# zqqqqz2000/MixGRPO

Hardware: AMD Instinct MI355X
Metric: GRPO train-step images/sec, FLUX.1-dev 1024^2 (higher is better)
Workload: dtype bf16

## Files before the change

### include/mixgrpo_hip.h

```cpp
#ifndef MIXGRPO_HIP_H
#define MIXGRPO_HIP_H
#include <stdint.h>
#ifdef __cplusplus
extern "C" {
#endif

int mgx_version(void);
const char* mgx_last_error(void);

typedef struct {
  float sigma_x0;
  float c_x;
  float c_v;
  float dt_mean;
  float sd_noise;
  float dt_det;
  float den;
  float log_sd;
  float log_c;
} mgx_flow_coeffs;

long mgx_logp_workspace_elems(int B, long n);

int mgx_flow_step_fwd(const float* x, const uint16_t* v, const uint16_t* noise, const float* prev_in,
// ... 7 lines not shown
  float ds_r;
  float s_r;
  float ds;
  float ds_b;
  float s_b;
  float one_m_s;
  float s_sq;
  float half_eta2;
  float sd;
  float den;
} mgx_dance_coeffs;

int mgx_dance_step_fwd(const float* x, const uint16_t* v, const float* noise, const float* prev_in,
                       float* prev_out, float* x0_out, float* logp, double* ws, int B, long n,
                       const mgx_dance_coeffs* k , int sde, void* stream);
int mgx_dance_step_bwd(const float* x, const uint16_t* v, const float* prev, const float* g_logp, uint16_t* dv,
                       int B, long n, const mgx_dance_coeffs* k , int sde, void* stream);

typedef struct {
  int order;
  int sde;
  float sigma_x0;
  float inv_r0;
  float inv_r1;
  float c_r;
  float inv_r01;
  float cm[4];
  float cx[4];
  float sd_noise;
  float den;
  float log_sd;
  float log_c;
} mgx_dpm_coeffs;

int mgx_dpm_step_fwd(const float* sample, const uint16_t* v, const float* m1, const float* m2, const float* noise,
                     float* x_out, float* x0_out, float* logp, double* ws, int B, long n,
                     const mgx_dpm_coeffs* k , void* stream);

int mgx_dpm_step_bwd(const float* sample, const uint16_t* v, const float* x_t, const float* g_logp, uint16_t* dv, int B,
                     long n, const mgx_dpm_coeffs* k , float sigma_b, void* stream);

int mgx_x0_pred(const float* sample, const uint16_t* v, float* x0_out, long total, float sigma_x0, void* stream);

int mgx_pack_latents(const void* in, void* out, int B, int C, int H, int W, int elem_size, void* stream);
int mgx_unpack_latents(const void* in, void* out, int B, int C, int H, int W, int elem_size, void* stream);

int mgx_group_advantage(const float* rewards, float* out, int n, int G, int trim, float weight, int accumulate,
                        void* stream);
int mgx_global_advantage(const float* rewards, const float* gathered, float* out, int n, int n_all, void* stream);

int mgx_grpo_loss(const float* new_logp, const float* old_logp, const float* adv, int B, float clip_range,
                  float adv_clip_max, float kl_coeff, float denom, float* loss, float* policy, float* kl,
                  float* clip_frac, float* g_logp, void* stream);

enum { MGX_EPI_BIAS = 0, MGX_EPI_BIAS_GELU = 1, MGX_EPI_BIAS_GATE_RES = 2, MGX_EPI_F32_ACC = 3, MGX_EPI_DGELU = 4 };

int mgx_gemm_bf16(const uint16_t* A, const uint16_t* W, const uint16_t* bias, void* C, const uint16_t* gate,
                  uint16_t* aux, long ldaux, int M, int N, int K, long lda, long a_rpb, long a_bstride, long ldw, long ldc,
                  long c_rpb, long c_bstride, long gate_ld, int epilogue, float beta, void* stream);
long mgx_gemm_sk_workspace_elems(void);
int mgx_gemm_bf16_sk(const uint16_t* A, const uint16_t* W, const uint16_t* bias, void* C, const uint16_t* gate,
                     uint16_t* aux, long ldaux, int M, int N, int K, long lda, long a_rpb, long a_bstride, long ldw, long ldc,
                     long c_rpb, long c_bstride, long gate_ld, int epilogue, float beta, float* sk_workspace,
                     long sk_workspace_elems, void* stream);
int mgx_linear_qk_norm_rope(const uint16_t* X, const uint16_t* Wqk, const uint16_t* bias, const float* wq, const float* wk,
                            const float* cos, const float* sin, const float* cos_sin_pairs ,
                            uint16_t* Q, uint16_t* K, int B, int H, int S, int rows_per_batch, int s0, int Kdim, long ldx,
                            long ldw, float q_scale, void* stream);

int mgx_linear_bf16_t(const uint16_t* X, const uint16_t* W, const uint16_t* bias, uint16_t* Ct, int tokens, int F, int K,
                      long ldx, long ldw, long ld_ct, long tok_rpb, long ct_bstride, float* sk_workspace,
                      long sk_workspace_elems, void* stream);

int mgx_gemm_plan(int M, int N, int K, int stream_k, int* out, int cap);
int mgx_gemm_plan_units(int M, int N, int K, int stream_k, int fixup, int index, int* out, int cap);

long mgx_transpose_partial_elems(int M, int N);
int mgx_transpose_bf16(const uint16_t* in, uint16_t* out, float* colsum_partial, float* colsum_out, float colsum_beta,
                       int M, int N, long ld_in, long in_rpb, long in_bstride, long ld_out, void* stream);

int mgx_ln_modulate_fwd(const uint16_t* x, long ldx, long x_rpb, long x_bstride, const uint16_t* shift,
                        const uint16_t* scale, long mod_ld, uint16_t* y, long ldy, float* stats, long M, int D,
                        void* stream);
long mgx_ln_modulate_bwd_workspace(long M, long rpb, int D);
int mgx_ln_modulate_bwd(const uint16_t* dy, long lddy, const uint16_t* x, long ldx, long x_rpb, long x_bstride,
                        const uint16_t* scale, long mod_ld, uint16_t* dx, long lddx, long dx_rpb, long dx_bstride,
                        int accumulate, uint16_t* dshift, uint16_t* dscale, float* ws, long M, int D, void* stream);

int mgx_qk_norm_rope_fwd(const uint16_t* qkv, long ld, const float* wq, const float* wk, const float* cos,
                         const float* sin, uint16_t* Q, uint16_t* K, uint16_t* Vt, uint16_t* V, uint16_t* Qt,
                         uint16_t* Kt, int B, int H, int S, int Sp, int rows_per_batch, int s0, void* stream);
int mgx_qk_norm_rope_fwd_qs(const uint16_t* qkv, long ld, const float* wq, const float* wk, const float* cos,
                            const float* sin, uint16_t* Q, uint16_t* K, uint16_t* Vt, uint16_t* V, uint16_t* Qt,
                            uint16_t* Kt, int B, int H, int S, int Sp, int rows_per_batch, int s0, float q_scale,
                            void* stream);
long mgx_qk_norm_rope_bwd_workspace(int B, int H, int rows_per_batch);
int mgx_qk_norm_rope_bwd(const uint16_t* qkv, long ld, const float* wq, const float* wk, const float* cos,
                         const float* sin, const uint16_t* dQ, const uint16_t* dK, const uint16_t* dV, uint16_t* dqkv,
                         long ld_dqkv , float* gwq, float* gwk, float* ws, int B,
                         int H, int S, int Sp, int rows_per_batch, int s0, void* stream);

int mgx_qk_norm_rope_bwd_qs(const uint16_t* qkv, long ld, const float* wq, const float* wk, const float* cos,
                            const float* sin, const uint16_t* dQ, const uint16_t* dK, const uint16_t* dV, uint16_t* dqkv,
                            long ld_dqkv, float* gwq, float* gwk, float* ws, int B, int H, int S, int Sp,
                            int rows_per_batch, int s0, float q_scale, void* stream);

int mgx_attn_fwd(const uint16_t* Q, const uint16_t* K, const uint16_t* Vt, uint16_t* O, float* lse, int B, int H, int S,
                 int Sp, long ldo, long o_bstride, float scale, void* stream);

int mgx_attn_fwd_log2(const uint16_t* Q2, const uint16_t* K, const uint16_t* Vt, uint16_t* O, float* lse, int B, int H,
                      int S, int Sp, long ldo, long o_bstride, void* stream);

int mgx_attn_fwd_path(int B, int H, int S, int Sp, long ldo, long o_bstride);
int mgx_attn_bwd_path(int B, int H, int S, int Sp, long ldo, long o_bstride);

int mgx_attn_fwd_log2_kv(const uint16_t* Q2, const uint16_t* K, const uint16_t* Vt, uint16_t* O, float* lse, int B, int H,
                         int Sa, int kv_len, long ldo, long o_bstride, void* stream);
int mgx_attn_fwd_kv_path(int B, int H, int Sa, int kv_len, long ldo, long o_bstride);

int mgx_attn_fp8_quantize(const uint16_t* Q, const uint16_t* K, const uint16_t* Vt, uint8_t* Q8, uint8_t* K8,
                          uint8_t* V8t, float* amax, int B, int H, int S, int Sp, void* stream);
int mgx_attn_fwd_fp8(const uint8_t* Q8, const uint8_t* K8, const uint8_t* V8t, const float* amax, uint16_t* O,
                     float* lse, int B, int H, int S, int Sp, long ldo, long o_bstride, float scale, void* stream);

int mgx_attn_bwd(const uint16_t* Q, const uint16_t* K, const uint16_t* V, const uint16_t* Qt, const uint16_t* Kt,
                 const uint16_t* O, const uint16_t* dO, const float* lse, float* delta, uint16_t* dOt, uint16_t* dQ,
                 uint16_t* dK, uint16_t* dV, int B, int H, int S, int Sp, long ldo, long o_bstride, float scale,
                 void* stream);

long mgx_attn_bwd_fp8_workspace(int B, int H, int S, int Sp);
int mgx_attn_bwd_fp8(const uint16_t* Q, const uint16_t* K, const uint16_t* V, const uint16_t* Qt, const uint16_t* Kt,
                     const uint16_t* O, const uint16_t* dO, const float* lse, float* delta, uint16_t* dOt, uint16_t* dQ,
                     uint16_t* dK, uint16_t* dV, uint8_t* ws, float* amax, int B, int H, int S, int Sp, long ldo,
                     long o_bstride, float scale, long ws_bytes, void* stream);

int mgx_attn_bwd_kv(const uint16_t* Q, const uint16_t* K, const uint16_t* V, const uint16_t* Qt, const uint16_t* Kt,
                    const uint16_t* O, const uint16_t* dO, const float* lse, float* delta, uint16_t* dOt, uint16_t* dQ,
                    uint16_t* dK, uint16_t* dV, int B, int H, int Sa, int kv_len, long ldo, long o_bstride, float scale,
                    void* stream);
int mgx_attn_bwd_kv_path(int B, int H, int Sa, int kv_len, long ldo, long o_bstride);

int mgx_attn_kv_operands(int stream, int kv_len, int block, int* out, int cap);

int mgx_skinny_linear(const uint16_t* x, long ldx, const uint16_t* W, long ldw, const uint16_t* bias, uint16_t* out,
                      long ldo, int Bn, int N, int K, void* stream);
int mgx_skinny_wgrad(const uint16_t* dout, long ldd, const uint16_t* x, long ldx, float* dW, long ldw, float* dbias,
                     int Bn, int N, int K, void* stream);
long mgx_skinny_dgrad_workspace(int Bn, int K);
int mgx_skinny_dgrad(const uint16_t* dout, long ldd, const uint16_t* W, long ldw, uint16_t* dx, long lddx, float* ws,
                     int Bn, int N, int K, int accumulate, void* stream);
int mgx_ew_bf16(const uint16_t* a, const uint16_t* b, uint16_t* y, long n, int op, void* stream);
int mgx_sincos_embed(const float* t, uint16_t* out, int Bn, void* stream);
int mgx_cast_f32_bf16(const float* x, uint16_t* y, long n, void* stream);
int mgx_cast_bf16_f32(const uint16_t* x, float* y, long n, float scale, void* stream);
int mgx_transpose_gelu_bf16(const uint16_t* in, uint16_t* out, int M, int N, long ld_in, long ld_out, void* stream);
int mgx_gelu_bf16(const uint16_t* x, long ldx, uint16_t* y, long ldy, long M, int N, void* stream);
long mgx_gate_bwd_workspace(long batches, long rows_per_batch, int D);
int mgx_gate_bwd(const uint16_t* dout, long ldd, long d_bstride, const uint16_t* y, long ldy, const uint16_t* gate,
                 long gate_ld, uint16_t* dy, long lddy, uint16_t* dgate, float* ws, int batches, long rows_per_batch,
                 int D, void* stream);

long mgx_sqnorm_workspace(void);
int mgx_sqnorm_f32(const float* g, long n, double* ws, float* out, float beta, void* stream);
int mgx_adamw_step(float* w, uint16_t* w16, const float* g, float* m, float* v, long n, double lr, double beta1,
                   double beta2, double eps, double weight_decay, int step, const float* gnorm_sq, float max_norm,
                   float grad_scale, void* stream);
int mgx_scale_f32(float* x, long n, float s, void* stream);


int mgx_conv3x3_nhwc(const uint16_t* x, const uint16_t* Wt, const uint16_t* bias, uint16_t* out, long ld_out,
                     const uint16_t* ones, int H, int W, int C, int Cout, int residual, void* stream);
long mgx_group_norm_workspace(long M, int C, int G);
int mgx_group_norm_nhwc(const uint16_t* x, long ld, const uint16_t* gamma, const uint16_t* beta, uint16_t* out, long out_row,
                        long out_px, float* ws, int H, int W, int C, int G, float eps, int silu, void* stream);
int mgx_upsample2x_pad_nhwc(const uint16_t* x, uint16_t* out, int H, int W, int C, void* stream);
int mgx_latents_to_pad_nhwc(const float* z, uint16_t* out, int Cin, int H, int W, int C, void* stream);
int mgx_nhwc_to_image(const uint16_t* x, long ld, uint16_t* img, int Cout, int H, int W, void* stream);
int mgx_softmax_rows_f32(const float* S, long lds, uint16_t* P, long ldp, int M, int n, float scale, void* stream);

int mgx_lora_proj(const uint16_t* in, const uint16_t* P, uint16_t* out, long M, int Kin, int r, long ld_in, long in_rpb,
                  long in_bstride, float scale, void* stream);
long mgx_lora_wgrad_workspace(long M, int Kin, int r);
int mgx_lora_wgrad(const uint16_t* small, const uint16_t* big, float* G, float* workspace, long workspace_elems, long M, int Kin,
                   int r, long ld_big, long big_rpb, long big_bstride, float beta, void* stream);
int mgx_lora_merge(const float* W0, const float* Bt, const float* A, uint16_t* W16, int N, int K, int r, float s, void* stream);

#ifdef __cplusplus
}
#endif
#endif
```

### mixgrpo_amd/_lib.py

```python
import ctypes as C
import os

import torch

_HERE = os.path.dirname(os.path.abspath(__file__))
LIB_PATH = os.path.join(_HERE, "csrc", "libmixgrpo_hip.so")


class MgxError(RuntimeError):
    pass


class FlowCoeffs(C.Structure):
    _fields_ = [(n, C.c_float) for n in ("sigma_x0", "c_x", "c_v", "dt_mean", "sd_noise", "dt_det", "den", "log_sd",
                                         "log_c")]


class DanceCoeffs(C.Structure):
    _fields_ = [(n, C.c_float) for n in ("ds_r", "s_r", "ds", "ds_b", "s_b", "one_m_s", "s_sq", "half_eta2", "sd", "den")]


class DpmCoeffs(C.Structure):
    _fields_ = [("order", C.c_int), ("sde", C.c_int), ("sigma_x0", C.c_float), ("inv_r0", C.c_float),
                ("inv_r1", C.c_float), ("c_r", C.c_float), ("inv_r01", C.c_float), ("cm", C.c_float * 4),
                ("cx", C.c_float * 4), ("sd_noise", C.c_float), ("den", C.c_float), ("log_sd", C.c_float),
                ("log_c", C.c_float)]


_P = C.c_void_p
_I = C.c_int
_L = C.c_long
_F = C.c_float
_D = C.c_double

SIGNATURES = {
    "mgx_version": (_I, []),
    "mgx_last_error": (C.c_char_p, []),
    "mgx_logp_workspace_elems": (_L, [_I, _L]),
    "mgx_flow_step_fwd": (_I, [_P] * 9 + [_I, _L, C.POINTER(FlowCoeffs), _I, _P]),
    "mgx_flow_step_bwd": (_I, [_P] * 5 + [_I, _L, C.POINTER(FlowCoeffs), _P]),
    "mgx_dance_step_fwd": (_I, [_P] * 8 + [_I, _L, C.POINTER(DanceCoeffs), _I, _P]),
    "mgx_dance_step_bwd": (_I, [_P] * 5 + [_I, _L, C.POINTER(DanceCoeffs), _I, _P]),
    "mgx_dpm_step_fwd": (_I, [_P] * 9 + [_I, _L, C.POINTER(DpmCoeffs), _P]),
    "mgx_dpm_step_bwd": (_I, [_P] * 5 + [_I, _L, C.POINTER(DpmCoeffs), _F, _P]),
    "mgx_x0_pred": (_I, [_P, _P, _P, _L, _F, _P]),
    "mgx_pack_latents": (_I, [_P, _P, _I, _I, _I, _I, _I, _P]),
    "mgx_unpack_latents": (_I, [_P, _P, _I, _I, _I, _I, _I, _P]),
    "mgx_group_advantage": (_I, [_P, _P, _I, _I, _I, _F, _I, _P]),
    "mgx_global_advantage": (_I, [_P, _P, _P, _I, _I, _P]),
    "mgx_grpo_loss": (_I, [_P, _P, _P, _I, _F, _F, _F, _F, _P, _P, _P, _P, _P, _P]),
    "mgx_gemm_bf16": (_I, [_P] * 6 + [_L, _I, _I, _I] + [_L] * 8 + [_I, _F, _P]),
    "mgx_gemm_sk_workspace_elems": (_L, []),
    "mgx_gemm_bf16_sk": (_I, [_P] * 6 + [_L, _I, _I, _I] + [_L] * 8 + [_I, _F, _P, _L, _P]),
    "mgx_linear_bf16_t": (_I, [_P] * 4 + [_I] * 3 + [_L] * 5 + [_P, _L, _P]),
    "mgx_linear_qk_norm_rope": (_I, [_P] * 10 + [_I] * 6 + [_L, _L, _F, _P]),
    "mgx_gemm_plan": (_I, [_I] * 4 + [C.POINTER(_I), _I]),
    "mgx_gemm_plan_units": (_I, [_I] * 6 + [C.POINTER(_I), _I]),
    "mgx_transpose_partial_elems": (_L, [_I, _I]),
    "mgx_transpose_bf16": (_I, [_P, _P, _P, _P, _F, _I, _I, _L, _L, _L, _L, _P]),
    "mgx_ln_modulate_fwd": (_I, [_P, _L, _L, _L, _P, _P, _L, _P, _L, _P, _L, _I, _P]),
    "mgx_ln_modulate_bwd_workspace": (_L, [_L, _L, _I]),
    "mgx_ln_modulate_bwd": (_I, [_P, _L, _P, _L, _L, _L, _P, _L, _P, _L, _L, _L, _I, _P, _P, _P, _L, _I, _P]),
    "mgx_qk_norm_rope_fwd": (_I, [_P, _L] + [_P] * 10 + [_I] * 6 + [_P]),
    "mgx_qk_norm_rope_fwd_qs": (_I, [_P, _L] + [_P] * 10 + [_I] * 6 + [_F, _P]),
    "mgx_qk_norm_rope_bwd_workspace": (_L, [_I, _I, _I]),
    "mgx_qk_norm_rope_bwd": (_I, [_P, _L] + [_P] * 8 + [_L] + [_P] * 3 + [_I] * 6 + [_P]),
    "mgx_qk_norm_rope_bwd_qs": (_I, [_P, _L] + [_P] * 8 + [_L] + [_P] * 3 + [_I] * 6 + [_F, _P]),
    "mgx_attn_fwd": (_I, [_P] * 5 + [_I] * 4 + [_L, _L, _F, _P]),
    "mgx_attn_fwd_log2": (_I, [_P] * 5 + [_I] * 4 + [_L, _L, _P]),
    "mgx_attn_fwd_path": (_I, [_I] * 4 + [_L, _L]),
    "mgx_attn_fwd_log2_kv": (_I, [_P] * 5 + [_I] * 4 + [_L, _L, _P]),
    "mgx_attn_fwd_kv_path": (_I, [_I] * 4 + [_L, _L]),
    "mgx_attn_bwd_path": (_I, [_I] * 4 + [_L, _L]),
    "mgx_attn_fp8_quantize": (_I, [_P] * 7 + [_I] * 4 + [_P]),
    "mgx_attn_fwd_fp8": (_I, [_P] * 6 + [_I] * 4 + [_L, _L, _F, _P]),
    "mgx_attn_bwd": (_I, [_P] * 13 + [_I] * 4 + [_L, _L, _F, _P]),
    "mgx_attn_bwd_fp8_workspace": (_L, [_I] * 4),
    "mgx_attn_bwd_fp8": (_I, [_P] * 15 + [_I] * 4 + [_L, _L, _F, _L, _P]),
    "mgx_attn_bwd_kv": (_I, [_P] * 13 + [_I] * 4 + [_L, _L, _F, _P]),
    "mgx_attn_bwd_kv_path": (_I, [_I] * 4 + [_L, _L]),
    "mgx_attn_kv_operands": (_I, [_I] * 3 + [C.POINTER(_I), _I]),
    "mgx_skinny_linear": (_I, [_P, _L, _P, _L, _P, _P, _L, _I, _I, _I, _P]),
    "mgx_skinny_wgrad": (_I, [_P, _L, _P, _L, _P, _L, _P, _I, _I, _I, _P]),
    "mgx_skinny_dgrad_workspace": (_L, [_I, _I]),
    "mgx_conv3x3_nhwc": (_I, [_P, _P, _P, _P, _L, _P, _I, _I, _I, _I, _I, _P]),
    "mgx_group_norm_workspace": (_L, [_L, _I, _I]),
    "mgx_group_norm_nhwc": (_I, [_P, _L, _P, _P, _P, _L, _L, _P, _I, _I, _I, _I, _F, _I, _P]),
    "mgx_upsample2x_pad_nhwc": (_I, [_P, _P, _I, _I, _I, _P]),
    "mgx_latents_to_pad_nhwc": (_I, [_P, _P, _I, _I, _I, _I, _P]),
    "mgx_nhwc_to_image": (_I, [_P, _L, _P, _I, _I, _I, _P]),
    "mgx_softmax_rows_f32": (_I, [_P, _L, _P, _L, _I, _I, _F, _P]),
    "mgx_skinny_dgrad": (_I, [_P, _L, _P, _L, _P, _L, _P, _I, _I, _I, _I, _P]),
    "mgx_ew_bf16": (_I, [_P, _P, _P, _L, _I, _P]),
    "mgx_sincos_embed": (_I, [_P, _P, _I, _P]),
    "mgx_cast_f32_bf16": (_I, [_P, _P, _L, _P]),
    "mgx_cast_bf16_f32": (_I, [_P, _P, _L, _F, _P]),
    "mgx_gelu_bf16": (_I, [_P, _L, _P, _L, _L, _I, _P]),
    "mgx_transpose_gelu_bf16": (_I, [_P, _P, _I, _I, _L, _L, _P]),
    "mgx_gate_bwd_workspace": (_L, [_L, _L, _I]),
    "mgx_gate_bwd": (_I, [_P, _L, _L, _P, _L, _P, _L, _P, _L, _P, _P, _I, _L, _I, _P]),
    "mgx_sqnorm_workspace": (_L, []),
    "mgx_sqnorm_f32": (_I, [_P, _L, _P, _P, _F, _P]),
    "mgx_adamw_step": (_I, [_P, _P, _P, _P, _P, _L, _D, _D, _D, _D, _D, _I, _P, _F, _F, _P]),
    "mgx_scale_f32": (_I, [_P, _L, _F, _P]),
    "mgx_lora_proj": (_I, [_P, _P, _P, _L, _I, _I, _L, _L, _L, _F, _P]),
    "mgx_lora_wgrad_workspace": (_L, [_L, _I, _I]),
    "mgx_lora_wgrad": (_I, [_P, _P, _P, _P, _L, _L, _I, _I, _L, _L, _L, _F, _P]),
    "mgx_lora_merge": (_I, [_P, _P, _P, _P, _I, _I, _I, _F, _P]),
}

_lib = None


def lib():
    global _lib
    if _lib is None:
        if not os.path.exists(LIB_PATH):
            raise MgxError(f"{LIB_PATH} is missing: run `python -m mixgrpo_amd.build` (hipcc, gfx950). "
                           "There is no CPU fallback for the product path.")
        h = C.CDLL(LIB_PATH)
        h.mgx_version.restype = _I
        v = h.mgx_version()
        if v < 0:
            raise MgxError(f"{LIB_PATH} is a DIAGNOSTIC build (mgx_version() = {v}, -DMGX_DIAGNOSTIC_BUILD): its timing-only "
                           "switches compute wrong results.  Rebuild with `python -m mixgrpo_amd.build --force`.")
        for name, (res, args) in SIGNATURES.items():
            fn = getattr(h, name)
            fn.restype = res
            fn.argtypes = args
        _lib = h
    return _lib


def check(code):
    if code != 0:
        raise MgxError(f"libmixgrpo_hip error {code}: {lib().mgx_last_error().decode()}")


def ptr(t):
    if t is None:
        return None
    if not t.is_cuda:
        raise MgxError("mixgrpo_amd HIP ops need device tensors (got a CPU tensor); there is no CPU path")
    if not t.is_contiguous():
        raise MgxError("mixgrpo_amd HIP ops need contiguous tensors")
    return t.data_ptr()


def stream():
    return torch.cuda.current_stream().cuda_stream


_ws_cache = {}


def logp_workspace(B, n, device):
    need = lib().mgx_logp_workspace_elems(B, n)
    key = (device, torch.cuda.current_stream().cuda_stream)
    w = _ws_cache.get(key)
    if w is None or w.numel() < need:
        w = torch.empty(max(need, 4096), dtype=torch.float64, device=device)
        _ws_cache[key] = w
    return w
```

### mixgrpo_amd/csrc/gemm.hip

```cpp
#include "../../include/mixgrpo_hip.h"
#include "common.h"
#include "gemm_plan.h"

#include <cmath>
#include <cstdlib>

namespace {

constexpr int BM = 128, BN = 128, BK = gemm_plan::BK;
constexpr int NT = 256;

struct RowMap {
  long ld;
  long rpb;
  long bstride;
};

__device__ __forceinline__ long row_off(const RowMap& r, long m) {
  const uint32_t rpb = (uint32_t)r.rpb;
  const uint32_t b = (uint32_t)m / rpb;
  return (long)b * r.bstride + (long)((uint32_t)m - b * rpb) * r.ld;
}

enum Epi { EPI_BIAS = 0, EPI_BIAS_GELU = 1, EPI_BIAS_GATE_RES = 2, EPI_F32_ACC = 3, EPI_BIAS_MULAUX = 4,
// ... 242 lines not shown
    if (m < M && n < N) v = in[row_off(im, m) + n];
    tile[r][tx] = v;
  }
  __syncthreads();
  for (int r = ty; r < 64; r += 4) {
    const int n = n0 + r;
    const long m = m0 + tx;
    if (n < N && m < ldo) out[(long)n * ldo + m] = (m < M) ? tile[tx][r] : (bf16_raw)0;
  }
  if (part && m0 < M) {
    if (ty == 0) {
      float s = 0.f;
      for (int r = 0; r < 64; ++r) s += bf2f(tile[r][tx]);
      if (n0 + tx < N) part[(long)blockIdx.y * N + n0 + tx] = s;
    }
  }
}

__device__ __forceinline__ uint32_t lo16(uint32_t a, uint32_t b) { return __builtin_amdgcn_perm(b, a, 0x05040100); }
__device__ __forceinline__ uint32_t hi16(uint32_t a, uint32_t b) { return __builtin_amdgcn_perm(b, a, 0x07060302); }
template <bool GELU>
__global__ void __launch_bounds__(256) transpose8_kernel(const bf16_raw* __restrict__ in, bf16_raw* __restrict__ out,
                                                         float* __restrict__ part, int M, int N, RowMap im, long ldo) {
  __shared__ float cs[16][129];
  const int tx = (threadIdx.x & 7) | (((threadIdx.x >> 6) & 1) << 3), ty = ((threadIdx.x >> 3) & 7) | ((threadIdx.x >> 7) << 3);
  const int n0 = blockIdx.x * 128 + tx * 8;
  const long m0 = (long)blockIdx.y * 128 + ty * 8;
  uint32_t r[8][4];
  float csum[8];
#pragma unroll
  for (int j = 0; j < 8; ++j) csum[j] = 0.f;
  const bool ncol_ok = n0 < N;
#pragma unroll
  for (int i = 0; i < 8; ++i) {
    const long m = m0 + i;
    uint4 v = make_uint4(0, 0, 0, 0);
    if (ncol_ok && m < M) v = *reinterpret_cast<const uint4*>(in + row_off(im, m) + n0);
    if (GELU && ncol_ok && m < M) {
      auto gl = [](uint32_t u) {
        return (uint32_t)f2bf(gelu_tanh_f(bf2f(u & 0xffff))) | ((uint32_t)f2bf(gelu_tanh_f(bf2f(u >> 16))) << 16);
      };
      v.x = gl(v.x); v.y = gl(v.y); v.z = gl(v.z); v.w = gl(v.w);
    }
    r[i][0] = v.x; r[i][1] = v.y; r[i][2] = v.z; r[i][3] = v.w;
    if (part) {
      csum[0] += bf2f(v.x & 0xffff); csum[1] += bf2f(v.x >> 16); csum[2] += bf2f(v.y & 0xffff); csum[3] += bf2f(v.y >> 16);
      csum[4] += bf2f(v.z & 0xffff); csum[5] += bf2f(v.z >> 16); csum[6] += bf2f(v.w & 0xffff); csum[7] += bf2f(v.w >> 16);
    }
  }
  if (ncol_ok && m0 < ldo) {
#pragma unroll
    for (int c2 = 0; c2 < 4; ++c2) {
      uint4 e, o;
      e.x = lo16(r[0][c2], r[1][c2]); e.y = lo16(r[2][c2], r[3][c2]); e.z = lo16(r[4][c2], r[5][c2]); e.w = lo16(r[6][c2], r[7][c2]);
      o.x = hi16(r[0][c2], r[1][c2]); o.y = hi16(r[2][c2], r[3][c2]); o.z = hi16(r[4][c2], r[5][c2]); o.w = hi16(r[6][c2], r[7][c2]);
      *reinterpret_cast<uint4*>(out + (long)(n0 + 2 * c2) * ldo + m0) = e;
      *reinterpret_cast<uint4*>(out + (long)(n0 + 2 * c2 + 1) * ldo + m0) = o;
    }
  }
  if (part) {
#pragma unroll
    for (int j = 0; j < 8; ++j) cs[ty][tx * 8 + j] = csum[j];
    __syncthreads();
    if (threadIdx.x < 128) {
      float t = 0.f;
#pragma unroll
      for (int k = 0; k < 16; ++k) t += cs[k][threadIdx.x];
      const int n = blockIdx.x * 128 + threadIdx.x;
      if (n < N && (long)blockIdx.y * 128 < M) part[(long)blockIdx.y * N + n] = t;
    }
  }
}

__global__ void __launch_bounds__(256) colsum_finish_kernel(const float* __restrict__ part, float* __restrict__ out, int nblk,
                                                            int N, float beta) {
  __shared__ float red[4][64];
  const int cx = threadIdx.x & 63, ky = threadIdx.x >> 6;
  const int n = blockIdx.x * 64 + cx;
  float s = 0.f;
  if (n < N)
    for (int b = ky; b < nblk; b += 4) s += part[(long)b * N + n];
  red[ky][cx] = s;
  __syncthreads();
  if (ky == 0 && n < N) out[n] = beta * out[n] + ((red[0][cx] + red[1][cx]) + (red[2][cx] + red[3][cx]));
}

__device__ __forceinline__ int wperm(int p) { return (p >> 5) * 32 + ((p & 15) >> 2) * 8 + ((p >> 4) & 1) * 4 + (p & 3); }
__device__ __forceinline__ int lane_feat(int fq, int t) { return (t >> 1) * 32 + fq * 8 + (t & 1) * 4; }

__device__ __forceinline__ void unpack8(const uint4& u, float* v) {
  v[0] = bf2f(u.x & 0xffff); v[1] = bf2f(u.x >> 16); v[2] = bf2f(u.y & 0xffff); v[3] = bf2f(u.y >> 16);
  v[4] = bf2f(u.z & 0xffff); v[5] = bf2f(u.z >> 16); v[6] = bf2f(u.w & 0xffff); v[7] = bf2f(u.w >> 16);
}
__device__ __forceinline__ uint4 pack8(const float* v) {
  uint4 o;
  o.x = (uint32_t)f2bf(v[0]) | ((uint32_t)f2bf(v[1]) << 16);
  o.y = (uint32_t)f2bf(v[2]) | ((uint32_t)f2bf(v[3]) << 16);
  o.z = (uint32_t)f2bf(v[4]) | ((uint32_t)f2bf(v[5]) << 16);
  o.w = (uint32_t)f2bf(v[6]) | ((uint32_t)f2bf(v[7]) << 16);
  return o;
}

__device__ __forceinline__ float vmul1(float a, float b) { float r; asm("v_mul_f32 %0, %1, %2" : "=v"(r) : "v"(a), "v"(b)); return r; }
__device__ __forceinline__ float vsub1(float a, float b) { float r; asm("v_sub_f32 %0, %1, %2" : "=v"(r) : "v"(a), "v"(b)); return r; }
__device__ __forceinline__ float vadd1(float a, float b) { float r; asm("v_add_f32 %0, %1, %2" : "=v"(r) : "v"(a), "v"(b)); return r; }

template <bool PAIRED>
__device__ __forceinline__ void qknorm_epilogue(const GemmArgs& g, f32x4 (&acc)[4][8], int wid, int lane, long m0, long n0,
                                                char* red) {
#pragma clang fp contract(off)
  constexpr int MT = 8;
  const int fr = lane & 15, fq = lane >> 4;
  const int wu = __builtin_amdgcn_readfirstlane(wid);
  const long nu = n0 + (wu & 3) * 64;
  long mu = m0 + (wu >> 2) * 128;
  const bool inside = mu < g.M;
  if (!inside) mu = g.M - 128;
  const int sec = nu >= g.qn_dmodel ? 1 : 0;
  const int hcol = (int)(nu - (long)sec * g.qn_dmodel);
  const int head = hcol >> 7, hb = hcol & 64;
  const uint32_t bu = (uint32_t)mu / (uint32_t)g.c.rpb;
  const int t0 = (int)((uint32_t)mu - bu * (uint32_t)g.c.rpb);
  const int f0 = lane_feat(fq, 0), f1 = lane_feat(fq, 2);
  uint4 bias0 = make_uint4(0, 0, 0, 0), bias1 = bias0;
  if (g.bias) {
    bias0 = *reinterpret_cast<const uint4*>(g.bias + nu + f0);
    bias1 = *reinterpret_cast<const uint4*>(g.bias + nu + f1);
  }
  const float* cbase = g.qn_cos + (long)(g.qn_s0 + t0 + fr) * 128 + hb;
  const float* sbase = g.qn_sin + (long)(g.qn_s0 + t0 + fr) * 128 + hb;
  constexpr int AHEAD = PAIRED ? 2 : 1, NSLOT = AHEAD + 1;
  float4 cs[NSLOT][PAIRED ? 4 : 8];
  const float* pbase = g.qn_cs2 + (long)(g.qn_s0 + t0 + fr) * 128 + hb;
  auto load_cs = [&](int slot, int j, uint32_t dep) {
    const long o = (long)(j * 16 + dep) * 128;
    if constexpr (PAIRED) {
      cs[slot][0] = *reinterpret_cast<const float4*>(pbase + o + f0);
      cs[slot][1] = *reinterpret_cast<const float4*>(pbase + o + f0 + 4);
      cs[slot][2] = *reinterpret_cast<const float4*>(pbase + o + f1);
      cs[slot][3] = *reinterpret_cast<const float4*>(pbase + o + f1 + 4);
      return;
    }
    cs[slot][0] = *reinterpret_cast<const float4*>(cbase + o + f0);
    cs[slot][1] = *reinterpret_cast<const float4*>(cbase + o + f0 + 4);
    cs[slot][2] = *reinterpret_cast<const float4*>(cbase + o + f1);
    cs[slot][3] = *reinterpret_cast<const float4*>(cbase + o + f1 + 4);
    cs[slot][4] = *reinterpret_cast<const float4*>(sbase + o + f0);
    cs[slot][5] = *reinterpret_cast<const float4*>(sbase + o + f0 + 4);
    cs[slot][6] = *reinterpret_cast<const float4*>(sbase + o + f1);
    cs[slot][7] = *reinterpret_cast<const float4*>(sbase + o + f1 + 4);
  };
  uint4 y[MT][2];
  {
    float bias[16];
    unpack8(bias0, bias);
    unpack8(bias1, bias + 8);
#pragma unroll
    for (int j = 0; j < MT; ++j) {
      float v[16];
#pragma unroll
      for (int t = 0; t < 4; ++t)
#pragma unroll
        for (int r = 0; r < 4; ++r) v[t * 4 + r] = acc[t][j][r] + bias[t * 4 + r];
      y[j][0] = pack8(v);
      y[j][1] = pack8(v + 8);
      __builtin_amdgcn_sched_barrier(0);
    }
// ... 837 lines not shown
```

### mixgrpo_amd/csrc/norm.hip

```cpp
#include "../../include/mixgrpo_hip.h"
#include "common.h"

namespace {

struct RowMap {
  long ld, rpb, bstride;
};
__device__ __forceinline__ long row_off(const RowMap& r, long m) {
  const long b = m / r.rpb;
  return b * r.bstride + (m - b * r.rpb) * r.ld;
}

constexpr int LN_MAXV = 8;

__device__ __forceinline__ void unpack8(const uint4& u, float* f) {
  f[0] = bf2f(u.x & 0xffff); f[1] = bf2f(u.x >> 16); f[2] = bf2f(u.y & 0xffff); f[3] = bf2f(u.y >> 16);
  f[4] = bf2f(u.z & 0xffff); f[5] = bf2f(u.z >> 16); f[6] = bf2f(u.w & 0xffff); f[7] = bf2f(u.w >> 16);
}
__device__ __forceinline__ uint4 pack8(const float* f) {
  uint4 u;
  u.x = (uint32_t)f2bf(f[0]) | ((uint32_t)f2bf(f[1]) << 16);
  u.y = (uint32_t)f2bf(f[2]) | ((uint32_t)f2bf(f[3]) << 16);
  u.z = (uint32_t)f2bf(f[4]) | ((uint32_t)f2bf(f[5]) << 16);
  u.w = (uint32_t)f2bf(f[6]) | ((uint32_t)f2bf(f[7]) << 16);
  return u;
}

template <int NV>
__global__ void __launch_bounds__(256) ln_mod_fwd_kernel(const bf16_raw* __restrict__ x, RowMap xm,
                                                         const bf16_raw* __restrict__ shift,
                                                         const bf16_raw* __restrict__ scale, long mod_ld,
                                                         bf16_raw* __restrict__ y, long ldy, float* __restrict__ stats,
                                                         long M) {
  const long m = (long)blockIdx.x * 4 + (threadIdx.x >> 6);
  if (m >= M) return;
  const int lane = threadIdx.x & 63;
  const long b = m / xm.rpb;
  const bf16_raw* xr = x + row_off(xm, m);
  float v[NV][8];
  float s = 0.f;
#pragma unroll
  for (int i = 0; i < NV; ++i) {
    unpack8(*reinterpret_cast<const uint4*>(xr + (i * 64 + lane) * 8), v[i]);
#pragma unroll
    for (int j = 0; j < 8; ++j) s += v[i][j];
  }
  const float D = (float)(NV * 512);
  const float mean = wave_sum(s) / D;
  float q = 0.f;
#pragma unroll
  for (int i = 0; i < NV; ++i)
#pragma unroll
    for (int j = 0; j < 8; ++j) {
      const float d = v[i][j] - mean;
      q += d * d;
    }
  const float rstd = rsqrtf(wave_sum(q) / D + 1e-6f);
  if (stats && lane == 0) {
    stats[2 * m] = mean;
    stats[2 * m + 1] = rstd;
  }
  const bf16_raw* sh = shift + b * mod_ld;
  const bf16_raw* sc = scale + b * mod_ld;
#pragma unroll
  for (int i = 0; i < NV; ++i) {
    const int c = (i * 64 + lane) * 8;
    float fs[8], fc[8], o[8];
    unpack8(*reinterpret_cast<const uint4*>(sh + c), fs);
    unpack8(*reinterpret_cast<const uint4*>(sc + c), fc);
#pragma unroll
    for (int j = 0; j < 8; ++j) o[j] = (v[i][j] - mean) * rstd * rbf(1.0f + fc[j]) + fs[j];
    *reinterpret_cast<uint4*>(y + m * ldy + c) = pack8(o);
  }
}

constexpr int LN_BWD_ROWS = 32;
template <int NV>
__global__ void __launch_bounds__(256) ln_mod_bwd_kernel(const bf16_raw* __restrict__ dy, long lddy,
                                                         const bf16_raw* __restrict__ x, RowMap xm,
                                                         const bf16_raw* __restrict__ scale, long mod_ld,
                                                         bf16_raw* __restrict__ dx, RowMap dxm, int accumulate,
                                                         float* __restrict__ part, long M, int blocks_per_batch) {
  extern __shared__ float red[];
  const int D = NV * 512;
  const int lane = threadIdx.x & 63, w = threadIdx.x >> 6;
  const long b = blockIdx.x / blocks_per_batch;
  const long r0 = (long)(blockIdx.x % blocks_per_batch) * LN_BWD_ROWS;
  const bf16_raw* sc = scale + b * mod_ld;
  float a_sh[NV][8], a_sc[NV][8];
#pragma unroll
  for (int i = 0; i < NV; ++i)
#pragma unroll
    for (int j = 0; j < 8; ++j) a_sh[i][j] = a_sc[i][j] = 0.f;

  auto row_ok = [&](int rr) { return rr < LN_BWD_ROWS && r0 + rr < xm.rpb && b * xm.rpb + r0 + rr < M; };
  uint4 nx[NV], ng[NV], nold[NV];
  auto fetch = [&](int rr) {
    const long m = b * xm.rpb + r0 + rr;
    const bf16_raw* xr = x + row_off(xm, m);
    const bf16_raw* dxr = dx + row_off(dxm, m);
#pragma unroll
    for (int i = 0; i < NV; ++i) {
      nx[i] = *reinterpret_cast<const uint4*>(xr + (i * 64 + lane) * 8);
      ng[i] = *reinterpret_cast<const uint4*>(dy + m * lddy + (i * 64 + lane) * 8);
      nold[i] = accumulate ? *reinterpret_cast<const uint4*>(dxr + (i * 64 + lane) * 8) : make_uint4(0, 0, 0, 0);
    }
  };
  if (row_ok(w)) fetch(w);
  for (int rr = w; row_ok(rr); rr += 4) {
    const long m = b * xm.rpb + r0 + rr;
    bf16_raw* dxr = dx + row_off(dxm, m);
    float v[NV][8], g[NV][8];
    uint4 oldp[NV];
    float s = 0.f;
#pragma unroll
    for (int i = 0; i < NV; ++i) {
      unpack8(nx[i], v[i]);
      unpack8(ng[i], g[i]);
      oldp[i] = nold[i];
#pragma unroll
      for (int j = 0; j < 8; ++j) s += v[i][j];
    }
    if (row_ok(rr + 4)) fetch(rr + 4);
    const float Df = (float)D;
    const float mean = wave_sum(s) / Df;
    float q = 0.f;
#pragma unroll
    for (int i = 0; i < NV; ++i)
#pragma unroll
      for (int j = 0; j < 8; ++j) {
        const float d = v[i][j] - mean;
        q += d * d;
      }
    const float rstd = rsqrtf(wave_sum(q) / Df + 1e-6f);
    float c1 = 0.f, c2 = 0.f;
#pragma unroll
    for (int i = 0; i < NV; ++i) {
      float fc[8];
      unpack8(*reinterpret_cast<const uint4*>(sc + (i * 64 + lane) * 8), fc);
#pragma unroll
      for (int j = 0; j < 8; ++j) {
        const float xh = (v[i][j] - mean) * rstd;
        const float gx = g[i][j] * rbf(1.0f + fc[j]);
        a_sh[i][j] += g[i][j];
        a_sc[i][j] += g[i][j] * xh;
        c1 += gx;
        c2 += gx * xh;
        v[i][j] = xh;
        g[i][j] = gx;
      }
    }
    c1 = wave_sum(c1) / Df;
    c2 = wave_sum(c2) / Df;
#pragma unroll
    for (int i = 0; i < NV; ++i) {
// ... 176 lines not shown
  long ldo;
  float* part;
  int H, S, Sp, rows_per_batch, s0;
  float q_scale;
};

__global__ void __launch_bounds__(256) qk_norm_rope_bwd_kernel(QkBwdArgs a) {
  __shared__ float red[4][2][128];
  const int lane = threadIdx.x & 63, w = threadIdx.x >> 6;
  const int hh = blockIdx.y, b = blockIdx.z;
  const int t0 = blockIdx.x * 64;
  const int HD = 128;
  const long dmodel = (long)a.H * HD;
  const float wq0 = a.wq[2 * lane], wq1 = a.wq[2 * lane + 1];
  const float wk0 = a.wk[2 * lane], wk1 = a.wk[2 * lane + 1];
  float gq0 = 0.f, gq1 = 0.f, gk0 = 0.f, gk1 = 0.f;
  constexpr int U = 4;
  for (int i0 = 0; i0 < 16; i0 += U) {
    uint32_t ux[U][2], ug[U][2], uv[U];
    float2 cc[U], ss[U];
    bool ok[U];
#pragma unroll
    for (int u = 0; u < U; ++u) {
      const int t = t0 + w * 16 + i0 + u;
      ok[u] = t < a.rows_per_batch;
      const int tc = ok[u] ? t : a.rows_per_batch - 1;
      const long row = (long)b * a.rows_per_batch + tc;
      const int s = a.s0 + tc;
      const bf16_raw* base = a.qkv + row * a.ld + hh * HD + 2 * lane;
      const long o = (((long)b * a.H + hh) * a.S + s) * HD + 2 * lane;
      ux[u][0] = *reinterpret_cast<const uint32_t*>(base);
      ux[u][1] = *reinterpret_cast<const uint32_t*>(base + dmodel);
      ug[u][0] = *reinterpret_cast<const uint32_t*>(a.dQ + o);
      ug[u][1] = *reinterpret_cast<const uint32_t*>(a.dK + o);
      uv[u] = *reinterpret_cast<const uint32_t*>(a.dV + o);
      cc[u] = *reinterpret_cast<const float2*>(a.cos + (long)s * HD + 2 * lane);
      ss[u] = *reinterpret_cast<const float2*>(a.sin + (long)s * HD + 2 * lane);
    }
#pragma unroll
    for (int u = 0; u < U; ++u) {
      if (!ok[u]) continue;
      const int t = t0 + w * 16 + i0 + u;
      const long row = (long)b * a.rows_per_batch + t;
      bf16_raw* obase = a.dqkv + row * a.ldo + hh * HD + 2 * lane;
      const float c0 = cc[u].x, c1 = cc[u].y, s0 = ss[u].x, s1 = ss[u].y;
#pragma unroll
      for (int which = 0; which < 2; ++which) {
        const float w0 = which ? wk0 : wq0, w1 = which ? wk1 : wq1;
        const float x0 = bf2f(ux[u][which] & 0xffff), x1 = bf2f(ux[u][which] >> 16);
        const float gs = which ? 1.f : a.q_scale;
        const float go0 = bf2f(ug[u][which] & 0xffff) * gs, go1 = bf2f(ug[u][which] >> 16) * gs;
        const float gy0 = go0 * c0 + go1 * s1;
        const float gy1 = -go0 * s0 + go1 * c1;
        const float r = rsqrtf(head_sum(x0 * x0 + x1 * x1) / 128.f + 1e-6f);
        if (which) { gk0 += gy0 * x0 * r; gk1 += gy1 * x1 * r; } else { gq0 += gy0 * x0 * r; gq1 += gy1 * x1 * r; }
        const float gz0 = gy0 * w0, gz1 = gy1 * w1;
        const float dot = wave_sum(gz0 * x0 + gz1 * x1) / 128.f;
        const float dx0 = r * gz0 - x0 * r * r * r * dot;
        const float dx1 = r * gz1 - x1 * r * r * r * dot;
        *reinterpret_cast<uint32_t*>(obase + which * dmodel) = (uint32_t)f2bf(dx0) | ((uint32_t)f2bf(dx1) << 16);
      }
      *reinterpret_cast<uint32_t*>(obase + 2 * dmodel) = uv[u];
    }
  }
  red[w][0][2 * lane] = gq0; red[w][0][2 * lane + 1] = gq1;
  red[w][1][2 * lane] = gk0; red[w][1][2 * lane + 1] = gk1;
  __syncthreads();
  const long blk = ((long)blockIdx.z * gridDim.y + blockIdx.y) * gridDim.x + blockIdx.x;
  {
    const int which = threadIdx.x >> 7, c = threadIdx.x & 127;
    a.part[(blk * 2 + which) * 128 + c] = red[0][which][c] + red[1][which][c] + red[2][which][c] + red[3][which][c];
  }
}

constexpr int QK_FIN_G = 128;
__global__ void __launch_bounds__(256) qk_bwd_partial_kernel(const float* __restrict__ part, float* __restrict__ mid,
                                                             long nblocks) {
  float s = 0.f;
  for (long k = blockIdx.x; k < nblocks; k += QK_FIN_G) s += part[k * 256 + threadIdx.x];
  mid[(long)blockIdx.x * 256 + threadIdx.x] = s;
}

__global__ void __launch_bounds__(256) qk_bwd_finish_kernel(const float* __restrict__ part, float* __restrict__ gq,
                                                            float* __restrict__ gk, long nblocks) {
  __shared__ float red[16][17];
  const int which = blockIdx.x >> 3, c0 = (blockIdx.x & 7) * 16;
  const int cx = threadIdx.x & 15, ry = threadIdx.x >> 4;
  float s = 0.f;
  for (long k = ry; k < nblocks; k += 16) s += part[(k * 2 + which) * 128 + c0 + cx];
  red[ry][cx] = s;
  __syncthreads();
  if (ry == 0) {
    float t = 0.f;
#pragma unroll
    for (int i = 0; i < 16; ++i) t += red[i][cx];
    float* dst = which ? gk : gq;
    dst[c0 + cx] += t;
  }
}

}

extern "C" int mgx_ln_modulate_fwd(const uint16_t* x, long ldx, long x_rpb, long x_bstride, const uint16_t* shift,
                                   const uint16_t* scale, long mod_ld, uint16_t* y, long ldy, float* stats, long M, int D,
                                   void* stream) {
  MGX_REQUIRE(x && shift && scale && y && M > 0, "bad argument");
  MGX_REQUIRE(D % 512 == 0 && D <= 4096, "feature size must be a multiple of 512 up to 4096");
  MGX_REQUIRE(ldx % 8 == 0 && ldy % 8 == 0 && mod_ld % 8 == 0 && x_bstride % 8 == 0, "16-byte row alignment");
  hipStream_t st = (hipStream_t)stream;
  const RowMap xm{ldx, x_rpb, x_bstride};
  const int grid = cdiv(M, 4);
  switch (D / 512) {
#define CASE(nv) case nv: ln_mod_fwd_kernel<nv><<<grid, 256, 0, st>>>(x, xm, shift, scale, mod_ld, y, ldy, stats, M); break;
    CASE(1) CASE(2) CASE(3) CASE(4) CASE(5) CASE(6) CASE(7) CASE(8)
#undef CASE
  }
  MGX_CHECK_LAUNCH();
  return MGX_OK;
}

extern "C" long mgx_ln_modulate_bwd_workspace(long M, long rpb, int D) {
  const long batches = (M + rpb - 1) / rpb;
  const long bpb = ((rpb < M ? rpb : M) + LN_BWD_ROWS - 1) / LN_BWD_ROWS;
  return batches * bpb * 2 * D;
}

extern "C" int mgx_ln_modulate_bwd(const uint16_t* dy, long lddy, const uint16_t* x, long ldx, long x_rpb, long x_bstride,
                                   const uint16_t* scale, long mod_ld, uint16_t* dx, long lddx, long dx_rpb,
                                   long dx_bstride, int accumulate, uint16_t* dshift, uint16_t* dscale, float* ws, long M,
                                   int D, void* stream) {
  MGX_REQUIRE(dy && x && scale && dx && dshift && dscale && ws && M > 0, "bad argument");
  MGX_REQUIRE(D % 512 == 0 && D <= 4096, "feature size must be a multiple of 512 up to 4096");
  MGX_REQUIRE(x_rpb == dx_rpb, "x and dx must be batched alike");
  hipStream_t st = (hipStream_t)stream;
  const long rpb = x_rpb < M ? x_rpb : M;
  const int batches = cdiv(M, rpb);
  const int bpb = cdiv(rpb, LN_BWD_ROWS);
  const RowMap xm{ldx, rpb, x_bstride}, dxm{lddx, rpb, dx_bstride};
  const size_t lds = (size_t)2 * D * sizeof(float);
  switch (D / 512) {
#define CASE(nv)                                                                                                  \
  case nv:                                                                                                        \
    ln_mod_bwd_kernel<nv><<<batches * bpb, 256, lds, st>>>(dy, lddy, x, xm, scale, mod_ld, dx, dxm, accumulate, ws, M, bpb); \
    break;
    CASE(1) CASE(2) CASE(3) CASE(4) CASE(5) CASE(6) CASE(7) CASE(8)
#undef CASE
  }
  ln_mod_bwd_finish_kernel<<<dim3(cdiv(D, 64), batches), 256, 0, st>>>(ws, dshift, dscale, mod_ld, D, bpb);
  MGX_CHECK_LAUNCH();
  return MGX_OK;
}

extern "C" int mgx_qk_norm_rope_fwd_qs(const uint16_t* qkv, long ld, const float* wq, const float* wk, const float* cos,
                                       const float* sin, uint16_t* Q, uint16_t* K, uint16_t* Vt, uint16_t* V, uint16_t* Qt,
                                       uint16_t* Kt, int B, int H, int S, int Sp, int rows_per_batch, int s0, float q_scale,
                                       void* stream) {
  MGX_REQUIRE(qkv && wq && wk && cos && sin && Q && K, "null argument");
  MGX_REQUIRE((V != nullptr) == (Qt != nullptr) && (V != nullptr) == (Kt != nullptr), "V, Qt, Kt come together");
  MGX_REQUIRE(Vt || !V, "Vt may only be left out (V^T written by mgx_linear_bf16_t) without the backward's extra layouts");
  MGX_REQUIRE(B > 0 && H > 0 && rows_per_batch > 0 && s0 >= 0 && s0 + rows_per_batch <= S && Sp >= S, "bad sizes");
  MGX_REQUIRE(ld == 3L * H * 128, "qkv rows must be [q | k | v] of H*128 each");
  MGX_REQUIRE(q_scale > 0.f, "q_scale must be positive");
  QkArgs a{qkv, ld, wq, wk, cos, sin, Q, K, Vt, V, Qt, Kt, H, S, Sp, rows_per_batch, s0, q_scale};
  dim3 grid(cdiv(rows_per_batch, 64), H, B);
  if (V) qk_norm_rope_fwd_kernel<true><<<grid, 256, 0, (hipStream_t)stream>>>(a);
  else qk_norm_rope_fwd_kernel<false><<<grid, 256, 0, (hipStream_t)stream>>>(a);
  MGX_CHECK_LAUNCH();
  return MGX_OK;
}

extern "C" int mgx_qk_norm_rope_fwd(const uint16_t* qkv, long ld, const float* wq, const float* wk, const float* cos,
                                    const float* sin, uint16_t* Q, uint16_t* K, uint16_t* Vt, uint16_t* V, uint16_t* Qt,
                                    uint16_t* Kt, int B, int H, int S, int Sp, int rows_per_batch, int s0, void* stream) {
  return mgx_qk_norm_rope_fwd_qs(qkv, ld, wq, wk, cos, sin, Q, K, Vt, V, Qt, Kt, B, H, S, Sp, rows_per_batch, s0, 1.0f, stream);
}

extern "C" long mgx_qk_norm_rope_bwd_workspace(int B, int H, int rows_per_batch) {
  return ((long)cdiv(rows_per_batch, 64) * H * B + QK_FIN_G) * 2 * 128;
}

extern "C" int mgx_qk_norm_rope_bwd_qs(const uint16_t* qkv, long ld, const float* wq, const float* wk, const float* cos,
                                       const float* sin, const uint16_t* dQ, const uint16_t* dK, const uint16_t* dV,
                                       uint16_t* dqkv, long ld_dqkv, float* gwq, float* gwk, float* ws, int B, int H, int S,
                                       int Sp, int rows_per_batch, int s0, float q_scale, void* stream) {
  MGX_REQUIRE(qkv && wq && wk && cos && sin && dQ && dK && dV && dqkv && gwq && gwk && ws, "null argument");
  MGX_REQUIRE(ld == 3L * H * 128, "qkv rows must be [q | k | v] of H*128 each");
  MGX_REQUIRE(ld_dqkv >= ld && ld_dqkv % 2 == 0, "dqkv rows must hold [dq | dk | dv] and keep 4-byte alignment");
  hipStream_t st = (hipStream_t)stream;
  QkBwdArgs a{qkv, ld, wq, wk, cos, sin, dQ, dK, dV, dqkv, ld_dqkv, ws, H, S, Sp, rows_per_batch, s0, q_scale};
  dim3 grid(cdiv(rows_per_batch, 64), H, B);
  qk_norm_rope_bwd_kernel<<<grid, 256, 0, st>>>(a);
  const long nblocks = (long)grid.x * grid.y * grid.z;
  float* mid = ws + nblocks * 256;
  qk_bwd_partial_kernel<<<QK_FIN_G, 256, 0, st>>>(ws, mid, nblocks);
  qk_bwd_finish_kernel<<<16, 256, 0, st>>>(mid, gwq, gwk, QK_FIN_G);
  MGX_CHECK_LAUNCH();
  return MGX_OK;
}

extern "C" int mgx_qk_norm_rope_bwd(const uint16_t* qkv, long ld, const float* wq, const float* wk, const float* cos,
                                    const float* sin, const uint16_t* dQ, const uint16_t* dK, const uint16_t* dV,
                                    uint16_t* dqkv, long ld_dqkv, float* gwq, float* gwk, float* ws, int B, int H, int S,
                                    int Sp, int rows_per_batch, int s0, void* stream) {
  return mgx_qk_norm_rope_bwd_qs(qkv, ld, wq, wk, cos, sin, dQ, dK, dV, dqkv, ld_dqkv, gwq, gwk, ws, B, H, S, Sp, rows_per_batch,
                                 s0, 1.0f, stream);
}
```

### mixgrpo_amd/csrc/small.hip

```cpp
#include "../../include/mixgrpo_hip.h"
#include "common.h"

namespace {

__global__ void __launch_bounds__(256) skinny_linear_kernel(const bf16_raw* __restrict__ x, long ldx,
                                                            const bf16_raw* __restrict__ W, long ldw,
                                                            const bf16_raw* __restrict__ bias,
                                                            bf16_raw* __restrict__ out, long ldo, int Bn, int N, int K) {
  __shared__ f32x4 red[3][64];
  const int lane = threadIdx.x & 63, w = threadIdx.x >> 6;
  const int n0 = blockIdx.x * 16;
  const int fr = lane & 15, fq = lane >> 4;
  int nrow = n0 + fr;
  if (nrow >= N) nrow = N - 1;
  int brow = fr < Bn ? fr : Bn - 1;
  const int kchunk = ((K / 32 + 3) / 4) * 32;
  const int kbeg = min(w * kchunk, K), kend = min(kbeg + kchunk, K);
  const bf16_raw* wp = W + (long)nrow * ldw + fq * 8;
  const bf16_raw* xp = x + (long)brow * ldx + fq * 8;
  f32x4 acc = {0.f, 0.f, 0.f, 0.f};
  int k = kbeg;
  for (; k + 128 <= kend; k += 128) {
    s16x8 a0 = *reinterpret_cast<const s16x8*>(wp + k), a1 = *reinterpret_cast<const s16x8*>(wp + k + 32);
    s16x8 a2 = *reinterpret_cast<const s16x8*>(wp + k + 64), a3 = *reinterpret_cast<const s16x8*>(wp + k + 96);
    s16x8 b0 = *reinterpret_cast<const s16x8*>(xp + k), b1 = *reinterpret_cast<const s16x8*>(xp + k + 32);
    s16x8 b2 = *reinterpret_cast<const s16x8*>(xp + k + 64), b3 = *reinterpret_cast<const s16x8*>(xp + k + 96);
    acc = __builtin_amdgcn_mfma_f32_16x16x32_bf16(a0, b0, acc, 0, 0, 0);
    acc = __builtin_amdgcn_mfma_f32_16x16x32_bf16(a1, b1, acc, 0, 0, 0);
    acc = __builtin_amdgcn_mfma_f32_16x16x32_bf16(a2, b2, acc, 0, 0, 0);
    acc = __builtin_amdgcn_mfma_f32_16x16x32_bf16(a3, b3, acc, 0, 0, 0);
  }
  for (; k < kend; k += 32) {
    s16x8 a0 = *reinterpret_cast<const s16x8*>(wp + k);
    s16x8 b0 = *reinterpret_cast<const s16x8*>(xp + k);
    acc = __builtin_amdgcn_mfma_f32_16x16x32_bf16(a0, b0, acc, 0, 0, 0);
  }
  if (w > 0) red[w - 1][lane] = acc;
  __syncthreads();
  if (w > 0) return;
#pragma unroll
  for (int i = 0; i < 3; ++i) {
    const f32x4 o = red[i][lane];
    acc[0] += o[0]; acc[1] += o[1]; acc[2] += o[2]; acc[3] += o[3];
  }
  if (fr < Bn) {
#pragma unroll
    for (int r = 0; r < 4; ++r) {
      const int n = n0 + 4 * fq + r;
      if (n < N) {
        float v = acc[r];
        if (bias) v += bf2f(bias[n]);
        out[(long)fr * ldo + n] = f2bf(v);
      }
    }
  }
}

__global__ void __launch_bounds__(256) skinny_wgrad_kernel(const bf16_raw* __restrict__ dout, long ldd,
                                                           const bf16_raw* __restrict__ x, long ldx,
                                                           float* __restrict__ dW, long ldw, float* __restrict__ dbias,
                                                           int Bn, int N, int K) {
  const int n = blockIdx.y;
  float dn[16];
  float sb = 0.f;
#pragma unroll
  for (int b = 0; b < 16; ++b) {
    dn[b] = b < Bn ? bf2f(dout[(long)b * ldd + n]) : 0.f;
    sb += dn[b];
  }
  if (dbias && blockIdx.x == 0 && threadIdx.x == 0) dbias[n] += sb;
  for (int k = (blockIdx.x * 256 + threadIdx.x) * 4; k < K; k += gridDim.x * 256 * 4) {
    float4 g = *reinterpret_cast<float4*>(dW + (long)n * ldw + k);
    for (int b = 0; b < Bn; ++b) {
      const uint2 u = *reinterpret_cast<const uint2*>(x + (long)b * ldx + k);
      g.x += dn[b] * bf2f(u.x & 0xffff); g.y += dn[b] * bf2f(u.x >> 16);
      g.z += dn[b] * bf2f(u.y & 0xffff); g.w += dn[b] * bf2f(u.y >> 16);
    }
    *reinterpret_cast<float4*>(dW + (long)n * ldw + k) = g;
  }
}

constexpr int SD_G = 128;
__global__ void __launch_bounds__(256) skinny_dgrad_kernel(const bf16_raw* __restrict__ dout, long ldd,
                                                           const bf16_raw* __restrict__ W, long ldw, float* __restrict__ part,
                                                           int Bn, int N, int K) {
  extern __shared__ float dsh[];
  const int g = blockIdx.y;
  const int nrows = (N - g + SD_G - 1) / SD_G;
  for (int id = threadIdx.x; id < nrows * 8; id += 256) {
    const int i = id >> 3, b = id & 7;
    dsh[id] = b < Bn ? bf2f(dout[(long)b * ldd + g + (long)i * SD_G]) : 0.f;
  }
  __syncthreads();
  const int c = (blockIdx.x * 256 + threadIdx.x) * 8;
  if (c >= K) return;
  float acc[8][8];
#pragma unroll
  for (int b = 0; b < 8; ++b)
#pragma unroll
    for (int e = 0; e < 8; ++e) acc[b][e] = 0.f;
  const bf16_raw* wp = W + (long)g * ldw + c;
  const long step = (long)SD_G * ldw;
  int i = 0;
  for (; i + 4 <= nrows; i += 4) {
    uint4 u[4];
#pragma unroll
    for (int q = 0; q < 4; ++q) u[q] = *reinterpret_cast<const uint4*>(wp + (i + q) * step);
#pragma unroll
    for (int q = 0; q < 4; ++q) {
      float wv[8];
      wv[0] = bf2f(u[q].x & 0xffff); wv[1] = bf2f(u[q].x >> 16); wv[2] = bf2f(u[q].y & 0xffff); wv[3] = bf2f(u[q].y >> 16);
      wv[4] = bf2f(u[q].z & 0xffff); wv[5] = bf2f(u[q].z >> 16); wv[6] = bf2f(u[q].w & 0xffff); wv[7] = bf2f(u[q].w >> 16);
      const float4 d0 = *reinterpret_cast<const float4*>(dsh + (i + q) * 8), d1 = *reinterpret_cast<const float4*>(dsh + (i + q) * 8 + 4);
      const float dv[8] = {d0.x, d0.y, d0.z, d0.w, d1.x, d1.y, d1.z, d1.w};
#pragma unroll
      for (int b = 0; b < 8; ++b)
#pragma unroll
        for (int e = 0; e < 8; ++e) acc[b][e] += dv[b] * wv[e];
    }
  }
  for (; i < nrows; ++i) {
    const uint4 u = *reinterpret_cast<const uint4*>(wp + i * step);
    float wv[8];
    wv[0] = bf2f(u.x & 0xffff); wv[1] = bf2f(u.x >> 16); wv[2] = bf2f(u.y & 0xffff); wv[3] = bf2f(u.y >> 16);
    wv[4] = bf2f(u.z & 0xffff); wv[5] = bf2f(u.z >> 16); wv[6] = bf2f(u.w & 0xffff); wv[7] = bf2f(u.w >> 16);
#pragma unroll
    for (int b = 0; b < 8; ++b)
#pragma unroll
      for (int e = 0; e < 8; ++e) acc[b][e] += dsh[i * 8 + b] * wv[e];
  }
  for (int b = 0; b < Bn; ++b) {
    float* pp = part + ((long)g * Bn + b) * K + c;
    *reinterpret_cast<float4*>(pp) = make_float4(acc[b][0], acc[b][1], acc[b][2], acc[b][3]);
    *reinterpret_cast<float4*>(pp + 4) = make_float4(acc[b][4], acc[b][5], acc[b][6], acc[b][7]);
  }
}

__global__ void __launch_bounds__(256) skinny_dgrad_finish_kernel(const float* __restrict__ part, bf16_raw* __restrict__ dx,
                                                                  long lddx, int Bn, int K, int accumulate) {
  const long id = (long)blockIdx.x * 256 + threadIdx.x;
  if (id >= (long)Bn * K) return;
  const int b = (int)(id / K), k = (int)(id - (long)b * K);
  float s = 0.f;
  for (int g = 0; g < SD_G; ++g) s += part[((long)g * Bn + b) * K + k];
  bf16_raw* o = dx + (long)b * lddx + k;
  const float r = rbf(s);
  *o = f2bf(accumulate ? bf2f(*o) + r : r);
}

__device__ __forceinline__ float silu_f(float x) { return x / (1.0f + expf(-x)); }

__global__ void ew_kernel(const bf16_raw* __restrict__ a, const bf16_raw* __restrict__ b, bf16_raw* __restrict__ y,
                          long n, int op) {
  for (long i = (long)blockIdx.x * blockDim.x + threadIdx.x; i < n; i += (long)gridDim.x * blockDim.x) {
    const float fa = bf2f(a[i]);
// ... 11 lines not shown
__global__ void sincos_embed_kernel(const float* __restrict__ t, bf16_raw* __restrict__ out, int Bn) {
  const int b = blockIdx.x, k = threadIdx.x;
  if (b >= Bn) return;
  const float f = expf(-logf(10000.0f) * (float)k / 128.0f);
  const float ang = t[b] * f;
  out[(long)b * 256 + k] = f2bf(cosf(ang));
  out[(long)b * 256 + 128 + k] = f2bf(sinf(ang));
}

__global__ void cast_f32_bf16_kernel(const float* __restrict__ x, bf16_raw* __restrict__ y, long n) {
  for (long i = ((long)blockIdx.x * blockDim.x + threadIdx.x) * 4; i < n; i += (long)gridDim.x * blockDim.x * 4) {
    const float4 v = *reinterpret_cast<const float4*>(x + i);
    uint2 o;
    o.x = (uint32_t)f2bf(v.x) | ((uint32_t)f2bf(v.y) << 16);
    o.y = (uint32_t)f2bf(v.z) | ((uint32_t)f2bf(v.w) << 16);
    *reinterpret_cast<uint2*>(y + i) = o;
  }
}

__global__ void cast_bf16_f32_kernel(const bf16_raw* __restrict__ x, float* __restrict__ y, long n, float scale) {
  for (long i = ((long)blockIdx.x * blockDim.x + threadIdx.x) * 8; i < n; i += (long)gridDim.x * blockDim.x * 8) {
    const uint4 u = *reinterpret_cast<const uint4*>(x + i);
    float4 a, b;
    a.x = bf2f(u.x & 0xffff) * scale; a.y = bf2f(u.x >> 16) * scale; a.z = bf2f(u.y & 0xffff) * scale; a.w = bf2f(u.y >> 16) * scale;
    b.x = bf2f(u.z & 0xffff) * scale; b.y = bf2f(u.z >> 16) * scale; b.z = bf2f(u.w & 0xffff) * scale; b.w = bf2f(u.w >> 16) * scale;
    *reinterpret_cast<float4*>(y + i) = a;
    *reinterpret_cast<float4*>(y + i + 4) = b;
  }
}

constexpr int GR_ROWS = 64;
__global__ void __launch_bounds__(256) gate_bwd_kernel(const bf16_raw* __restrict__ dout, long ldd, long d_rpb,
                                                       long d_bstride, const bf16_raw* __restrict__ y, long ldy,
                                                       const bf16_raw* __restrict__ gate, long gate_ld,
                                                       bf16_raw* __restrict__ dy, long lddy, float* __restrict__ part,
                                                       long rows_per_batch, int D, int blocks_per_batch) {
  const long b = blockIdx.y / blocks_per_batch;
  const long r0 = (long)(blockIdx.y % blocks_per_batch) * GR_ROWS;
  const int c = (blockIdx.x * 256 + threadIdx.x) * 2;
  if (c >= D) return;
  const uint32_t gu = *reinterpret_cast<const uint32_t*>(gate + b * gate_ld + c);
  const float g0 = bf2f(gu & 0xffff), g1 = bf2f(gu >> 16);
  float a0 = 0.f, a1 = 0.f;
  const long rend = min(r0 + (long)GR_ROWS, rows_per_batch);
  for (long r = r0; r < rend; ++r) {
    const long m = b * rows_per_batch + r;
    const uint32_t du = *reinterpret_cast<const uint32_t*>(dout + b * d_bstride + r * ldd + c);
    const uint32_t yu = *reinterpret_cast<const uint32_t*>(y + m * ldy + c);
    const float d0 = bf2f(du & 0xffff), d1 = bf2f(du >> 16);
    a0 += d0 * bf2f(yu & 0xffff);
    a1 += d1 * bf2f(yu >> 16);
    *reinterpret_cast<uint32_t*>(dy + m * lddy + c) = (uint32_t)f2bf(g0 * d0) | ((uint32_t)f2bf(g1 * d1) << 16);
  }
  part[(long)blockIdx.y * D + c] = a0;
  part[(long)blockIdx.y * D + c + 1] = a1;
}

__global__ void __launch_bounds__(256) gate_bwd_finish_kernel(const float* __restrict__ part, bf16_raw* __restrict__ dgate,
                                                              long gate_ld, int D, int blocks_per_batch) {
  __shared__ float red[4][64];
  const int b = blockIdx.y;
  const int cx = threadIdx.x & 63, ky = threadIdx.x >> 6;
  const int c = blockIdx.x * 64 + cx;
  float s = 0.f;
  if (c < D)
    for (int k = ky; k < blocks_per_batch; k += 4) s += part[((long)b * blocks_per_batch + k) * D + c];
  red[ky][cx] = s;
  __syncthreads();
  if (ky == 0 && c < D) dgate[(long)b * gate_ld + c] = f2bf((red[0][cx] + red[1][cx]) + (red[2][cx] + red[3][cx]));
}

}

extern "C" int mgx_skinny_linear(const uint16_t* x, long ldx, const uint16_t* W, long ldw, const uint16_t* bias,
                                 uint16_t* out, long ldo, int Bn, int N, int K, void* stream) {
  MGX_REQUIRE(x && W && out, "null operand");
  MGX_REQUIRE(Bn >= 1 && Bn <= 16, "skinny linear handles 1..16 rows");
  MGX_REQUIRE(K % 32 == 0 && ldx % 8 == 0 && ldw % 8 == 0, "K must be a multiple of 32 with 16-byte aligned rows");
  skinny_linear_kernel<<<cdiv(N, 16), 256, 0, (hipStream_t)stream>>>(x, ldx, W, ldw, bias, out, ldo, Bn, N, K);
  MGX_CHECK_LAUNCH();
  return MGX_OK;
}

extern "C" int mgx_skinny_wgrad(const uint16_t* dout, long ldd, const uint16_t* x, long ldx, float* dW, long ldw,
                                float* dbias, int Bn, int N, int K, void* stream) {
  MGX_REQUIRE(dout && x && dW, "null operand");
  MGX_REQUIRE(Bn >= 1 && Bn <= 16, "skinny wgrad handles 1..16 rows");
  MGX_REQUIRE(K % 4 == 0 && ldx % 4 == 0 && ldw % 4 == 0, "K must be a multiple of 4");
  int gx = cdiv(K, 1024);
  skinny_wgrad_kernel<<<dim3(gx, N), 256, 0, (hipStream_t)stream>>>(dout, ldd, x, ldx, dW, ldw, dbias, Bn, N, K);
  MGX_CHECK_LAUNCH();
  return MGX_OK;
}

extern "C" long mgx_skinny_dgrad_workspace(int Bn, int K) { return (long)SD_G * (Bn < 8 ? Bn : 8) * K; }

extern "C" int mgx_skinny_dgrad(const uint16_t* dout, long ldd, const uint16_t* W, long ldw, uint16_t* dx, long lddx,
                                float* ws, int Bn, int N, int K, int accumulate, void* stream) {
  MGX_REQUIRE(dout && W && dx && ws, "null operand");
  MGX_REQUIRE(Bn >= 1 && Bn <= 8, "skinny dgrad handles 1..8 rows per call");
  MGX_REQUIRE(N >= SD_G && K % 8 == 0 && ldw % 8 == 0 && ((uintptr_t)W % 16 == 0), "weight rows must be 16-byte addressable");
  hipStream_t st = (hipStream_t)stream;
  const size_t lds = (size_t)cdiv(N, SD_G) * 8 * sizeof(float);
  MGX_REQUIRE(lds <= 65536, "too many weight rows");
  skinny_dgrad_kernel<<<dim3(cdiv(K, 2048), SD_G), 256, lds, st>>>(dout, ldd, W, ldw, ws, Bn, N, K);
  skinny_dgrad_finish_kernel<<<cdiv((long)Bn * K, 256), 256, 0, st>>>(ws, dx, lddx, Bn, K, accumulate);
  MGX_CHECK_LAUNCH();
  return MGX_OK;
}

extern "C" int mgx_ew_bf16(const uint16_t* a, const uint16_t* b, uint16_t* y, long n, int op, void* stream) {
  MGX_REQUIRE(a && y && n > 0 && op >= 0 && op <= 3, "bad argument");
  MGX_REQUIRE(op == 0 || op == 3 || b, "binary op needs b");
  int nb = cdiv(n, 256);
  if (nb > 2048) nb = 2048;
  ew_kernel<<<nb, 256, 0, (hipStream_t)stream>>>(a, b, y, n, op);
  MGX_CHECK_LAUNCH();
  return MGX_OK;
}

extern "C" int mgx_sincos_embed(const float* t, uint16_t* out, int Bn, void* stream) {
  MGX_REQUIRE(t && out && Bn > 0, "bad argument");
  sincos_embed_kernel<<<Bn, 128, 0, (hipStream_t)stream>>>(t, out, Bn);
  MGX_CHECK_LAUNCH();
  return MGX_OK;
}

extern "C" int mgx_cast_f32_bf16(const float* x, uint16_t* y, long n, void* stream) {
  MGX_REQUIRE(x && y && n > 0 && n % 4 == 0, "bad argument");
  int nb = cdiv(n, 1024);
  if (nb > 4096) nb = 4096;
  cast_f32_bf16_kernel<<<nb, 256, 0, (hipStream_t)stream>>>(x, y, n);
  MGX_CHECK_LAUNCH();
  return MGX_OK;
}

extern "C" int mgx_cast_bf16_f32(const uint16_t* x, float* y, long n, float scale, void* stream) {
  MGX_REQUIRE(x && y && n > 0 && n % 8 == 0, "bad argument");
  MGX_REQUIRE(((uintptr_t)x % 16 == 0) && ((uintptr_t)y % 16 == 0), "operands must be 16-byte aligned");
  int nb = cdiv(n, 2048);
  if (nb > 4096) nb = 4096;
  cast_bf16_f32_kernel<<<nb, 256, 0, (hipStream_t)stream>>>(x, y, n, scale);
  MGX_CHECK_LAUNCH();
  return MGX_OK;
}

extern "C" long mgx_gate_bwd_workspace(long batches, long rows_per_batch, int D) {
  return batches * ((rows_per_batch + GR_ROWS - 1) / GR_ROWS) * D;
}

extern "C" int mgx_gate_bwd(const uint16_t* dout, long ldd, long d_bstride, const uint16_t* y, long ldy,
                            const uint16_t* gate, long gate_ld, uint16_t* dy, long lddy, uint16_t* dgate, float* ws,
                            int batches, long rows_per_batch, int D, void* stream) {
  MGX_REQUIRE(dout && y && gate && dy && dgate && ws, "null operand");
  MGX_REQUIRE(D % 2 == 0 && batches > 0 && rows_per_batch > 0, "bad sizes");
  const int bpb = cdiv(rows_per_batch, GR_ROWS);
  hipStream_t st = (hipStream_t)stream;
  gate_bwd_kernel<<<dim3(cdiv(D, 512), batches * bpb), 256, 0, st>>>(dout, ldd, rows_per_batch, d_bstride, y, ldy, gate,
                                                                      gate_ld, dy, lddy, ws, rows_per_batch, D, bpb);
  gate_bwd_finish_kernel<<<dim3(cdiv(D, 64), batches), 256, 0, st>>>(ws, dgate, gate_ld, D, bpb);
  MGX_CHECK_LAUNCH();
  return MGX_OK;
}
```

### mixgrpo_amd/flux.py

```python
import json
import math
import os
from dataclasses import asdict, dataclass
from typing import Dict, List, Tuple

import torch

from . import ops
from ._lib import MgxError
from .ops import BF16, F32, Rows, EPI_BIAS, EPI_BIAS_GELU, EPI_BIAS_GATE_RES


@dataclass
class FluxConfig:
    patch_size: int = 1
    in_channels: int = 64
    num_layers: int = 19
    num_single_layers: int = 38
    attention_head_dim: int = 128
    num_attention_heads: int = 24
    joint_attention_dim: int = 4096
    pooled_projection_dim: int = 768
    guidance_embeds: bool = True
    axes_dims_rope: Tuple[int, int, int] = (16, 56, 56)

    @property
    def dim(self):
        return self.attention_head_dim * self.num_attention_heads

    def to_dict(self):
        d = asdict(self)
        d["axes_dims_rope"] = list(self.axes_dims_rope)
        d["_class_name"] = "FluxTransformer2DModel"
        return d


def param_layout(cfg: FluxConfig) -> List[Tuple[str, Tuple[int, ...]]]:
    d, hd = cfg.dim, cfg.attention_head_dim
    out = []

    def lin(name, o, i):
        out.append((name + ".weight", (o, i)))
        out.append((name + ".bias", (o,)))

    def qkv(prefix, names):
        for n in names:
            out.append((f"{prefix}.{n}.weight", (d, d)))
        for n in names:
            out.append((f"{prefix}.{n}.bias", (d,)))

    lin("x_embedder", d, cfg.in_channels)
    lin("context_embedder", d, cfg.joint_attention_dim)
    embs = ["timestep_embedder"] + (["guidance_embedder"] if cfg.guidance_embeds else []) + ["text_embedder"]
    for e in embs:
        lin(f"time_text_embed.{e}.linear_1", d, cfg.pooled_projection_dim if e == "text_embedder" else 256)
        lin(f"time_text_embed.{e}.linear_2", d, d)
    for i in range(cfg.num_layers):
        p = f"transformer_blocks.{i}"
        lin(f"{p}.norm1.linear", 6 * d, d)
        lin(f"{p}.norm1_context.linear", 6 * d, d)
        qkv(f"{p}.attn", ("to_q", "to_k", "to_v"))
        qkv(f"{p}.attn", ("add_q_proj", "add_k_proj", "add_v_proj"))
        lin(f"{p}.attn.to_out.0", d, d)
        lin(f"{p}.attn.to_add_out", d, d)
        for n in ("norm_q", "norm_k", "norm_added_q", "norm_added_k"):
            out.append((f"{p}.attn.{n}.weight", (hd,)))
        for ff in ("ff", "ff_context"):
            lin(f"{p}.{ff}.net.0.proj", 4 * d, d)
            lin(f"{p}.{ff}.net.2", d, 4 * d)
    for i in range(cfg.num_single_layers):
        p = f"single_transformer_blocks.{i}"
        lin(f"{p}.norm.linear", 3 * d, d)
        for n in ("attn.to_q", "attn.to_k", "attn.to_v"):
            out.append((f"{p}.{n}.weight", (d, d)))
        out.append((f"{p}.proj_mlp.weight", (4 * d, d)))
        for n in ("attn.to_q", "attn.to_k", "attn.to_v"):
            out.append((f"{p}.{n}.bias", (d,)))
        out.append((f"{p}.proj_mlp.bias", (4 * d,)))
        lin(f"{p}.proj_out", d, 5 * d)
        for n in ("norm_q", "norm_k"):
            out.append((f"{p}.attn.{n}.weight", (hd,)))
    lin("norm_out.linear", 2 * d, d)
    lin("proj_out", cfg.patch_size * cfg.patch_size * cfg.in_channels, d)
    return out


class ParamStore:

    ALIGN = 64

    def __init__(self, cfg: FluxConfig, device):
        self.cfg = cfg
        self.device = torch.device(device)
        self.index: Dict[str, Tuple[int, Tuple[int, ...]]] = {}
        off = 0
        for name, shape in param_layout(cfg):
            self.index[name] = (off, shape)
            n = 1
            for s in shape:
                n *= s
            off += (n + self.ALIGN - 1) // self.ALIGN * self.ALIGN
        self.numel = off
        self.w32 = torch.zeros(off, dtype=F32, device=self.device)
        self.w16 = torch.zeros(off, dtype=BF16, device=self.device)
        self.g32 = None

    def view(self, buf, name):
        off, shape = self.index[name]
        n = 1
        for s in shape:
            n *= s
        return buf[off:off + n].view(shape)

    def fused(self, buf, first, rows_total):
        off, shape = self.index[first]
        if len(shape) == 1:
            return buf[off:off + rows_total]
        return buf[off:off + rows_total * shape[1]].view(rows_total, shape[1])

    def block_ranges(self):
        names = list(self.index)
        key = lambda n: ".".join(n.split(".")[:2]) if n.startswith(("transformer_blocks.", "single_transformer_blocks.")) \
            else ("head" if self.index[n][0] < self.index["norm_out.linear.weight"][0] else "tail")
        out, cur, lo = {}, None, 0
        for n in names:
            k = key(n)
            if k != cur:
                if cur is not None:
                    out[cur] = (lo, self.index[n][0])
                cur, lo = k, self.index[n][0]
        out[cur] = (lo, self.numel)
        return out

    def sync_bf16(self):
        self.w16.copy_(self.w32)

    def ensure_grad(self):
        if self.g32 is None:
            self.g32 = torch.zeros(self.numel, dtype=F32, device=self.device)
        return self.g32

    def init_synthetic(self, seed=0, std=0.02, bias_std=0.0):
        g = torch.Generator(device=self.device).manual_seed(seed)
        for name, (off, shape) in self.index.items():
            v = self.view(self.w32, name)
            if name.endswith(".bias"):
                if bias_std > 0:
                    v.normal_(0.0, bias_std, generator=g)
                else:
                    v.zero_()
            elif len(shape) == 1:
                v.fill_(1.0)
                if bias_std > 0:
                    v.add_(torch.randn(shape, generator=g, device=self.device) * bias_std)
            else:
                v.normal_(0.0, std, generator=g)
        self.sync_bf16()


def rope_tables(ids, axes_dims, theta=10000.0):
    cos, sin = [], []
    pos = ids.float()
    for a, dim in enumerate(axes_dims):
        fr = 1.0 / (theta ** (torch.arange(0, dim, 2, dtype=torch.float64, device=ids.device) / dim))
        ang = torch.outer(pos[:, a].double(), fr)
        cos.append(ang.cos().repeat_interleave(2, dim=1).float())
        sin.append(ang.sin().repeat_interleave(2, dim=1).float())
    return torch.cat(cos, -1).contiguous(), torch.cat(sin, -1).contiguous()


class _Work:

    kv_len = None

    def __init__(self, cfg, B, L, N, device):
        d, H, hd = cfg.dim, cfg.num_attention_heads, cfg.attention_head_dim
        S = L + N
        self.B, self.L, self.N, self.S = B, L, N, S
        self.Sp = (S + 63) // 64 * 64
        e = lambda *shape, dtype=BF16: torch.empty(*shape, dtype=dtype, device=device)
        self.X = e(B, S, d)
        self.nrm = e(B * S, d)
        self.qkv = e(B * S, 3 * d)
        self.Q = e(B, H, S, hd)
        self.K = e(B, H, S, hd)
        self.Vt = torch.zeros(B, H, hd, self.Sp, dtype=BF16, device=device)
        self.O = e(B, S, d)
        self.hid = e(B * S, 4 * d)
# ... 90 lines not shown
        lo = LoraStore(self.cfg, self.store.device, rank, rank if alpha is None else alpha, target_modules)
        lo.init_adapters(seed)
        self._attach_lora(lo)
        return self

    def _attach_lora(self, lo):
        self.lora = lo
        self.lora_param = torch.nn.Parameter(lo.w32, requires_grad=True)
        self.flat_param.requires_grad_(False)
        self.flat_param.grad = None
        self.store.g32 = None
        self.config.update(lora_rank=lo.rank, lora_alpha=lo.alpha, lora_target_modules=list(lo.target_modules))
        lo.merge(self.store)

    def merge_lora(self):
        self.lora.merge(self.store)

    def unload_lora(self):
        if self.lora is None:
            return self
        self.lora.unmerge(self.store)
        self.lora = None
        del self.lora_param
        for k in ("lora_rank", "lora_alpha", "lora_target_modules"):
            self.config.pop(k, None)
        self.flat_param.requires_grad_(True)
        return self

    def lora_state_dict(self):
        if self.lora is None:
            raise MgxError("lora_state_dict: no adapters attached")
        return self.lora.state_dict()

    def save_lora(self, save_dir, step=0):
        from safetensors.torch import save_file

        from .lora import WEIGHTS_NAME, write_lora_config
        os.makedirs(save_dir, exist_ok=True)
        sd = {k: v.detach().cpu().contiguous() for k, v in self.lora_state_dict().items()}
        tmp = os.path.join(save_dir, WEIGHTS_NAME + ".tmp")
        save_file(sd, tmp)
        os.replace(tmp, os.path.join(save_dir, WEIGHTS_NAME))
        write_lora_config(save_dir, self.lora.config(step))

    def load_lora(self, load_dir):
        from safetensors.torch import load_file

        from .lora import WEIGHTS_NAME, LoraStore, read_lora_config
        rank, alpha, targets, _ = read_lora_config(load_dir)
        self.unload_lora()
        lo = LoraStore(self.cfg, self.store.device, rank, alpha, targets)
        lo.load_state_dict(load_file(os.path.join(load_dir, WEIGHTS_NAME)))
        self._attach_lora(lo)
        return self

    def state_dict(self, *args, **kwargs):
        return {k: self.store.view(self.store.w32, k) for k in self.store.index}

    def load_state_dict(self, sd, strict=True):
        missing = [k for k in self.store.index if k not in sd]
        unexpected = [k for k in sd if k not in self.store.index]
        if strict and (missing or unexpected):
            raise RuntimeError(f"load_state_dict: missing {missing[:5]} unexpected {unexpected[:5]}")
        with torch.no_grad():
            for k, v in sd.items():
                if k in self.store.index:
                    self.store.view(self.store.w32, k).copy_(v.to(F32))
        self.store.sync_bf16()
        if self.lora is not None:
            self.lora.merge(self.store)
        return missing, unexpected

    def init_synthetic(self, seed=0, std=0.02, bias_std=0.0):
        self.store.init_synthetic(seed, std, bias_std)
        return self

    def W(self, name):
        return self.store.view(self.store.w16, name)

    def W32(self, name):
        return self.store.view(self.store.w32, name)

    def clip_grad_norm_(self, max_norm):
        g = self.trainable_store.ensure_grad()
        nsq = torch.zeros(1, dtype=F32, device=g.device)
        ops.sqnorm(g, nsq)
        total = nsq.sqrt()
        coef = torch.clamp(max_norm / (total + 1e-6), max=1.0)
        g.mul_(coef)
        return total.squeeze(0)

    def grow_ff_keep(self, reserve_gib=None):
        from . import flux_backward as FB
        if not FB.KEEP_ACTS or (FB.KEEP_FF != "auto" and FB.KEEP_QKV != "auto"):
            return self.ff_blocks_kept()
        reserve = (FB.KEEP_FF_RESERVE_GIB if reserve_gib is None else reserve_gib) * 2.0 ** 30
        for base in self._work.values():
            tr = base.train
            if tr is None or tr.keep is None:
                continue
            free, _total = torch.cuda.mem_get_info(self.store.device)
            tr.grow_auto(int(free - reserve))
        return self.ff_blocks_kept()

    def ff_blocks_kept(self):
        return sum(b.train.ff_kept() for b in self._work.values() if b.train is not None and b.train.keep is not None)

    def qkv_blocks_kept(self):
        return sum(b.train.qkv_kept() for b in self._work.values() if b.train is not None and b.train.keep is not None)

    def _workspace(self, B, L, N, kv_len=None):
        key = (L, N)
        base = self._work.get(key)
        if base is None or base.B < B:
            if base is not None:
                self._work.pop(key)
                del base
            elif len(self._work) >= 2:
                self._work.pop(next(iter(self._work)))
            torch.cuda.empty_cache()
            base = _Work(self.cfg, B, L, N, self.store.device)
            self._work[key] = base
        return base.view(B, kv_len)

    def _attn(self, w, O, lse, ldo, o_bstride):
        H = self.cfg.num_attention_heads
        scale = self.attn_scale()
        if self.attention_dtype == "fp8":
            q8, k8, v8t, amax = w.fp8_operands()
            ops.attn_fp8_quantize(w.Q, w.K, w.Vt, q8, k8, v8t, amax, w.B, H, w.S, w.Sp)
            ops.attn_fwd_fp8(q8, k8, v8t, amax, O, lse, w.B, H, w.S, w.Sp, ldo, o_bstride, scale)
        elif ops.Q_PRESCALE and w.kv_len is not None:
            if not ops.attn_fwd_log2_kv(w.Q, w.K, w.Vt, O, lse, w.B, H, w.S, w.kv_len, ldo, o_bstride):
                raise MgxError(f"mgx_attn_fwd_log2_kv refused B {w.B} H {H} Sa {w.S} kv_len {w.kv_len} after its path query took it")
        elif ops.Q_PRESCALE:
            ops.attn_fwd_log2(w.Q, w.K, w.Vt, O, lse, w.B, H, w.S, w.Sp, ldo, o_bstride)
        else:
            ops.attn_fwd(w.Q, w.K, w.Vt, O, lse, w.B, H, w.S, w.Sp, ldo, o_bstride, scale)

    def _qkv_nograd(self, nrm, first, qkv, w, rows, s0, wq, wk, cos, sin):
        d, H = self.cfg.dim, self.cfg.num_attention_heads
        Wf = self.store.fused(self.store.w16, f"{first}.weight", 3 * d)
        bf = self.store.fused(self.store.w16, f"{first}.bias", 3 * d)
        tokens = nrm.numel() // d
        B = tokens // rows
        vt = ops.LINEAR_VT and ops.linear_t(nrm, Wf[2 * d:], bf[2 * d:], w.Vt.view(-1)[s0:], tokens, d, d, w.Sp, rows, d * w.Sp)
        if vt and ops.LINEAR_QKNORM and H * 128 == d and ops.linear_qk_norm_rope(
                nrm, Wf[:2 * d], bf[:2 * d], wq, wk, cos, sin, w.Q, w.K, B, H, w.S, rows, s0, d, q_scale=self.q_scale(),
                pairs=self._rope_pairs(cos, sin)):
            return
        if vt:
            ops.gemm(Rows.of(nrm), Wf[:2 * d], bf[:2 * d], Rows(qkv, tokens, 3 * d), 2 * d, d)
        else:
            ops.gemm(Rows.of(nrm), Wf, bf, Rows.of(qkv), 3 * d, d)
        ops.qk_norm_rope(qkv, wq, wk, cos, sin, w.Q, w.K, None if vt else w.Vt, B, H, w.S, w.Sp, rows, s0, q_scale=self.q_scale())

    def q_scale(self):
        return ops.LOG2E / math.sqrt(self.cfg.attention_head_dim) if ops.Q_PRESCALE else 1.0

    def attn_scale(self):
        return ops.LN2 if ops.Q_PRESCALE else 1.0 / math.sqrt(self.cfg.attention_head_dim)

    def _rope(self, txt_ids, img_ids):
        key = (id(txt_ids), txt_ids._version, tuple(txt_ids.shape), id(img_ids), img_ids._version, tuple(img_ids.shape))
        hit = self._rope_cache.get("k")
        if hit is not None and hit[0] == key:
            return hit[1], hit[2]
        ids = torch.cat([txt_ids.float(), img_ids.float()], dim=0)
        cos, sin = rope_tables(ids, self.cfg.axes_dims_rope)
        self._rope_cache["k"] = (key, cos, sin, txt_ids, img_ids)
        return cos, sin

    def _rope_pairs(self, cos, sin):
        if not ops.ROPE_PAIR_TABLE:
            return None
        hit = self._rope_cache.get("pairs")
        if hit is None or hit[0] is not cos:
            hit = (cos, ops.rope_pair_table(cos, sin))
            self._rope_cache["pairs"] = hit
        return hit[1]

    def _temb(self, B, timestep, guidance, pooled, keep=None):
        d = self.cfg.dim
        dev = self.store.device
        t = (timestep.to(BF16) * 1000).float().contiguous()
        gd = guidance.to(dev)
        gd = (gd.to(BF16) * 1000).float()
        gd = gd.expand(B).contiguous() if gd.numel() == 1 else gd.contiguous()

        def mlp(name, x, K):
            h1 = torch.empty(B, d, dtype=BF16, device=dev)
            ops.skinny_linear(x, self.W(f"time_text_embed.{name}.linear_1.weight"),
                              self.W(f"time_text_embed.{name}.linear_1.bias"), h1, d, K)
            a1 = torch.empty_like(h1)
            ops.ew(h1, None, a1, 0)
            h2 = torch.empty_like(h1)
            ops.skinny_linear(a1, self.W(f"time_text_embed.{name}.linear_2.weight"),
                              self.W(f"time_text_embed.{name}.linear_2.bias"), h2, d, d)
            if keep is not None:
                keep[name] = (x, h1, a1)
            return h2

        te = torch.empty(B, 256, dtype=BF16, device=dev)
        ops.sincos_embed(t, te)
        temb = mlp("timestep_embedder", te, 256)
        if self.cfg.guidance_embeds:
            ge = torch.empty(B, 256, dtype=BF16, device=dev)
            ops.sincos_embed(gd, ge)
            gemb = mlp("guidance_embedder", ge, 256)
            t2 = torch.empty_like(temb)
            ops.ew(temb, gemb, t2, 2)
            temb = t2
        pe = mlp("text_embedder", pooled.to(BF16).contiguous(), self.cfg.pooled_projection_dim)
        t3 = torch.empty_like(temb)
        ops.ew(temb, pe, t3, 2)
        st = torch.empty_like(t3)
        ops.ew(t3, None, st, 0)
        return t3, st

    def _stream_rows(self, t, w, which, width):
        if which == "txt":
            return Rows(t, w.B * w.L, width, w.L, w.S * width)
        return Rows(t[0, w.L:], w.B * w.N, width, w.N, w.S * width)

    def _streams(self, w):
        streams = (("txt", "norm1_context", ("add_q_proj", "add_k_proj", "add_v_proj"), "norm_added_q", "norm_added_k",
                    "to_add_out", "ff_context", w.L, 0),
                   ("img", "norm1", ("to_q", "to_k", "to_v"), "norm_q", "norm_k", "to_out.0", "ff", w.N, w.L))
        return streams, {"txt": slice(0, w.B * w.L), "img": slice(w.B * w.L, w.B * w.S)}

    def _double_block(self, i, w, st, cos, sin, pl, mods_in=None):
        cfg, d, H = self.cfg, self.cfg.dim, self.cfg.num_attention_heads
        p = f"transformer_blocks.{i}"
        B = w.B
        dev = self.store.device
        mods = {}
        streams, sl = self._streams(w)
        W16, fused = self.W, self.store.fused
        if pl.restore is not None:
            w.X.copy_(pl.restore)
        for name, norm, qkvn, nq, nk, outn, ffn, rows, s0 in streams:
            if mods_in is not None:
                m = mods_in[name]
            else:
                m = torch.empty(B, 6 * d, dtype=BF16, device=dev)
                ops.skinny_linear(st, W16(f"{p}.{norm}.linear.weight"), W16(f"{p}.{norm}.linear.bias"), m, 6 * d, d)
            mods[name] = m
            ops.ln_modulate(self._stream_rows(pl.x_in, w, name, d), m[:, 0:d], m[:, d:2 * d], 6 * d, pl.nrm1[sl[name]], d)
        if pl.fused_qkv:
            for name, _, qkvn, nq, nk, _, _, rows, s0 in streams:
                self._qkv_nograd(pl.nrm1[sl[name]], f"{p}.attn.{qkvn[0]}", pl.qkv[sl[name]], w, rows, s0,
                                 self.W32(f"{p}.attn.{nq}.weight"), self.W32(f"{p}.attn.{nk}.weight"), cos, sin)
        else:
            for name, _, qkvn, *_ in (streams if pl.run_qkv else ()):
                ops.gemm(Rows.of(pl.nrm1[sl[name]]), fused(self.store.w16, f"{p}.attn.{qkvn[0]}.weight", 3 * d),
                         fused(self.store.w16, f"{p}.attn.{qkvn[0]}.bias", 3 * d), Rows.of(pl.qkv[sl[name]]), 3 * d, d)
            for name, norm, qkvn, nq, nk, outn, ffn, rows, s0 in streams:
                ops.qk_norm_rope(pl.qkv[sl[name]], self.W32(f"{p}.attn.{nq}.weight"), self.W32(f"{p}.attn.{nk}.weight"), cos, sin,
                                 w.Q, w.K, w.Vt, B, H, w.S, w.Sp, rows, s0, V=pl.V, Qt=pl.Qt, Kt=pl.Kt, q_scale=self.q_scale())
        if pl.run_attn:
            self._attn(w, pl.O, pl.lse, d, w.S * d)
        part = lambda t, name: None if t is None else t[sl[name]]
        if pl.run_out:
            for name, _, _, _, _, outn, *_ in streams:
                ops.gemm(self._stream_rows(pl.O, w, name, d), W16(f"{p}.attn.{outn}.weight"), W16(f"{p}.attn.{outn}.bias"),
                         self._stream_rows(w.X, w, name, d), d, d, EPI_BIAS_GATE_RES, gate=mods[name][:, 2 * d:3 * d],
                         gate_ld=6 * d, aux=part(pl.y_attn, name))
            if pl.x_mid is not None:
                pl.x_mid.copy_(w.X)
        x_mid = w.X if pl.run_out else pl.x_mid
        for name in ("txt", "img"):
            m = mods[name]
            ops.ln_modulate(self._stream_rows(x_mid, w, name, d), m[:, 3 * d:4 * d], m[:, 4 * d:5 * d], 6 * d, pl.nrm2[sl[name]], d)
        for name, _, _, _, _, _, ffn, *_ in (streams if pl.run_ff else ()):
            ops.gemm(Rows.of(pl.nrm2[sl[name]]), W16(f"{p}.{ffn}.net.0.proj.weight"), W16(f"{p}.{ffn}.net.0.proj.bias"),
                     Rows.of(w.hid[sl[name]]), 4 * d, d, EPI_BIAS_GELU, aux=part(pl.hid_pre, name))
        for name, _, _, _, _, _, ffn, *_ in (streams if pl.run_out else ()):
            ops.gemm(Rows.of(w.hid[sl[name]]), W16(f"{p}.{ffn}.net.2.weight"), W16(f"{p}.{ffn}.net.2.bias"),
                     self._stream_rows(w.X, w, name, d), d, 4 * d, EPI_BIAS_GATE_RES, gate=mods[name][:, 5 * d:6 * d],
                     gate_ld=6 * d, aux=part(pl.y_ff, name))
        return mods

    def _single_block(self, i, w, st, cos, sin, pl, mod_in=None):
        cfg, d, H = self.cfg, self.cfg.dim, self.cfg.num_attention_heads
        p = f"single_transformer_blocks.{i}"
        B, S = w.B, w.S
        M = B * S
        if pl.restore is not None:
            w.X.copy_(pl.restore)
        if mod_in is not None:
            m = mod_in
        else:
            m = torch.empty(B, 3 * d, dtype=BF16, device=self.store.device)
            ops.skinny_linear(st, self.W(f"{p}.norm.linear.weight"), self.W(f"{p}.norm.linear.bias"), m, 3 * d, d)
        Xa = Rows(pl.x_in, M, d, S, S * d)
        ops.ln_modulate(Xa, m[:, 0:d], m[:, d:2 * d], 3 * d, pl.nrm1, d)
        wq, wk = self.W32(f"{p}.attn.norm_q.weight"), self.W32(f"{p}.attn.norm_k.weight")
        if pl.fused_qkv:
            self._qkv_nograd(pl.nrm1, f"{p}.attn.to_q", pl.qkv, w, S, 0, wq, wk, cos, sin)
        elif pl.run_qkv:
            ops.gemm(Rows.of(pl.nrm1), self.store.fused(self.store.w16, f"{p}.attn.to_q.weight", 3 * d),
                     self.store.fused(self.store.w16, f"{p}.attn.to_q.bias", 3 * d), Rows.of(pl.qkv), 3 * d, d)
        cat2 = w.cat.view(M, 5 * d)
        if pl.run_ff:
            ops.gemm(Rows.of(pl.nrm1), self.W(f"{p}.proj_mlp.weight"), self.W(f"{p}.proj_mlp.bias"),
                     Rows(cat2[0, d:], M, 5 * d), 4 * d, d, EPI_BIAS_GELU, aux=pl.hid_pre)
        if not pl.fused_qkv:
            ops.qk_norm_rope(pl.qkv, wq, wk, cos, sin, w.Q, w.K, w.Vt, B, H, S, w.Sp, S, 0, V=pl.V, Qt=pl.Qt, Kt=pl.Kt,
                             q_scale=self.q_scale())
        if pl.run_attn:
            self._attn(w, pl.O, pl.lse, pl.ldo, S * pl.ldo)
            if pl.O_keep is not None:
                pl.O_keep.copy_(w.cat[:, :, :d])
        elif not pl.lean:
            w.cat[:, :, :d].copy_(pl.O_keep)
        if pl.run_out:
            ops.gemm(Rows.of(cat2), self.W(f"{p}.proj_out.weight"), self.W(f"{p}.proj_out.bias"), Xa, d, 5 * d,
                     EPI_BIAS_GATE_RES, gate=m[:, 2 * d:3 * d], gate_ld=3 * d, aux=pl.y_attn)
        return m

    def _embed(self, w, hidden_states, encoder_hidden_states):
        d = self.cfg.dim
        B, N, L = w.B, w.N, w.L
        hs = hidden_states.detach()
        if hs.dtype == BF16:
            w.in16.copy_(hs.reshape(B * N, -1))
        else:
            ops.cast_bf16(hs.to(F32).contiguous().view(-1), w.in16.view(-1))
        ops.gemm(Rows.of(w.in16), self.W("x_embedder.weight"), self.W("x_embedder.bias"),
                 self._stream_rows(w.X, w, "img", d), d, self.cfg.in_channels)
        ehs = encoder_hidden_states.detach().to(BF16).contiguous()
        ops.gemm(Rows.of(ehs.view(B * L, -1)), self.W("context_embedder.weight"), self.W("context_embedder.bias"),
                 self._stream_rows(w.X, w, "txt", d), d, self.cfg.joint_attention_dim)
        return ehs

    def _head(self, w, st):
        d = self.cfg.dim
        B, N = w.B, w.N
        e = torch.empty(B, 2 * d, dtype=BF16, device=self.store.device)
        ops.skinny_linear(st, self.W("norm_out.linear.weight"), self.W("norm_out.linear.bias"), e, 2 * d, d)
        nrm = w.nrm[:B * N]
        ops.ln_modulate(self._stream_rows(w.X, w, "img", d), e[:, d:2 * d], e[:, 0:d], 2 * d, nrm, d)
        cout = self.cfg.patch_size * self.cfg.patch_size * self.cfg.in_channels
        out = torch.empty(B, N, cout, dtype=BF16, device=self.store.device)
        ops.gemm(Rows.of(nrm), self.W("proj_out.weight"), self.W("proj_out.bias"), Rows.of(out.view(B * N, cout)), cout, d)
        return out, e

    def forward(self, hidden_states, encoder_hidden_states, timestep, guidance, txt_ids, pooled_projections, img_ids,
                joint_attention_kwargs=None, return_dict=False):
        if torch.is_grad_enabled() and self.training and self.trainable_param.requires_grad:
            from .flux_backward import FluxFunction
            out = FluxFunction.apply(self.trainable_param, self, hidden_states, encoder_hidden_states, timestep, guidance,
                                     txt_ids, pooled_projections, img_ids)
            return (out,)
        with torch.no_grad():
            out = self._forward_nograd(hidden_states, encoder_hidden_states, timestep, guidance, txt_ids,
                                       pooled_projections, img_ids)
        return (out,)

    def _pad_kv_rows(self, B, L, N):
        S = L + N
        if not ops.ATTN_PAD_KV or S % 256 == 0 or not ops.Q_PRESCALE or self.attention_dtype != "bf16":
            return None
        d, H = self.cfg.dim, self.cfg.num_attention_heads
        Sa = (S + 255) // 256 * 256
        if not all(ops.attn_fwd_kv_path(B, H, Sa, S, ld, Sa * ld) == 1 for ld in (d, 5 * d)):
            return None
        return Sa - L

    def _pad_kv_rows_train(self, B, L, N):
        N_pad = self._pad_kv_rows(B, L, N)
        if N_pad is None:
            return None
        d, H = self.cfg.dim, self.cfg.num_attention_heads
        Sa = L + N_pad
        if not all(ops.attn_bwd_kv_path(B, H, Sa, L + N, ld, Sa * ld) == 1 for ld in (d, 5 * d)):
            return None
        return N_pad

# ... 82 lines not shown
```

### mixgrpo_amd/flux_backward.py

```python
import math

import torch

from . import ops
from .ops import BF16, F32, Rows, EPI_BIAS, EPI_BIAS_GATE_RES, EPI_DGELU, EPI_F32_ACC


import os

KEEP_ACTS = os.environ.get("MGX_KEEP_ACTS", "1") != "0"
KEEP_FF = os.environ.get("MGX_KEEP_FF_BLOCKS", "auto")
KEEP_FF_RESERVE_GIB = float(os.environ.get("MGX_KEEP_FF_RESERVE_GIB", "12"))
KEEP_QKV = os.environ.get("MGX_KEEP_QKV_BLOCKS", "auto")


def _pad64(n):
    return (n + 63) // 64 * 64


class _Train:

    def __init__(self, cfg, w, device):
        d, H, hd = cfg.dim, cfg.num_attention_heads, cfg.attention_head_dim
        B, S, Sp = w.B, w.S, w.Sp
        self.B, self.S = B, S
        M = B * S
        e = lambda *shape, dtype=BF16: torch.empty(*shape, dtype=dtype, device=device)
        z = lambda *shape, dtype=BF16: torch.zeros(*shape, dtype=dtype, device=device)
        nblk = cfg.num_layers + cfg.num_single_layers
        self.block_in = e(nblk, B, S, d)
        self.x_final = e(B, S, d)
        self.keep = None
        if KEEP_ACTS:
            self.keep = []
            for b in range(nblk):
                k = dict(O=e(B, S, d), lse=e(B, H, S, dtype=F32), y_attn=e(M, d))
                if b < cfg.num_layers:
                    k.update(y_ff=e(M, d), x_mid=e(B, S, d))
                self.keep.append(k)
            self._ff_shape, self._ff_device = (M, 4 * d), device
            self._qkv_shape = (M, 3 * d)
            if KEEP_FF != "auto":
                self.grow_ff(int(KEEP_FF))
            if KEEP_QKV != "auto":
                self.grow_qkv(int(KEEP_QKV))
        self.save = dict(nrm1=e(M, d), nrm2=e(M, d), y_attn=e(M, d), y_ff=e(M, d), hid_pre=e(M, 4 * d),
                         x_mid=e(B, S, d), V=e(B, H, S, hd), Qt=z(B, H, hd, Sp), Kt=z(B, H, hd, Sp))
        self.dX = e(B, S, d)
        self.dO = e(B, S, 5 * d)
        self.dQ, self.dK, self.dV = e(B, H, S, hd), e(B, H, S, hd), e(B, H, S, hd)
        self.dOt = z(B, H, hd, Sp)
        self.delta = e(B, H, S, dtype=F32)
        self.dy = e(M, d)
        self.dbig = e(M, 7 * d)
        self.dnrm = e(M, d)
        Mp = _pad64(M)
        self.dCt = e(7 * d * Mp)
        self.At = e(5 * d * Mp)
        self.Wt = e(7 * d * max(d, 64) + 5 * d * d)
        self.ones = torch.ones(1, 5 * d, dtype=BF16, device=device)

    def view(self, B):
        return self if B == self.B else _TrainView(self, B)

    def ff_block_bytes(self):
        return self._ff_shape[0] * self._ff_shape[1] * 2

    def ff_kept(self):
        return sum(1 for k in (self.keep or []) if "hid_pre" in k)

    def qkv_block_bytes(self):
        return self._qkv_shape[0] * self._qkv_shape[1] * 2

    def qkv_kept(self):
        return sum(1 for k in (self.keep or []) if "qkv" in k)

    def grow_ff(self, n_total):
        if self.keep is None:
            return 0
        for k in self.keep[:max(0, n_total)]:
            if "hid_pre" not in k:
                k["hid_pre"] = torch.empty(*self._ff_shape, dtype=BF16, device=self._ff_device)
        return self.ff_kept()

    def grow_qkv(self, n_total):
        if self.keep is None:
            return 0
        for k in self.keep[:max(0, n_total)]:
            if "qkv" not in k:
                k["qkv"] = torch.empty(*self._qkv_shape, dtype=BF16, device=self._ff_device)
        return self.qkv_kept()

    def grow_auto(self, budget_bytes):
        if self.keep is None:
            return budget_bytes
        for i, k in enumerate(self.keep):
            for name, auto, size, grow in (("hid_pre", KEEP_FF == "auto", self.ff_block_bytes(), self.grow_ff),
                                           ("qkv", KEEP_QKV == "auto", self.qkv_block_bytes(), self.grow_qkv)):
                if name in k or not auto:
                    continue
                if budget_bytes < size:
                    return budget_bytes
                k[name] = torch.empty(*(self._ff_shape if name == "hid_pre" else self._qkv_shape), dtype=BF16,
                                      device=self._ff_device)
                budget_bytes -= size
        return budget_bytes


class _TrainView:

    def __init__(self, base, B):
        assert B <= base.B
        M = B * base.S
        self.B, self.S = B, base.S
        self.block_in = [base.block_in[i, :B] for i in range(base.block_in.shape[0])]
        self.x_final = base.x_final[:B]
        rows = ("nrm1", "nrm2", "y_attn", "y_ff", "hid_pre")
        self.save = {k: (v[:M] if k in rows else v[:B]) for k, v in base.save.items()}
        self.keep = None
        if base.keep is not None:
            self.keep = [{k: (v[:M] if k in ("y_attn", "y_ff", "hid_pre", "qkv") else v[:B]) for k, v in kb.items()}
                         for kb in base.keep]
        self.dX, self.dO, self.dQ, self.dK, self.dV, self.dOt, self.delta = (
            t[:B] for t in (base.dX, base.dO, base.dQ, base.dK, base.dV, base.dOt, base.delta))
        self.dy, self.dbig, self.dnrm = base.dy[:M], base.dbig[:M], base.dnrm[:M]
        self.dCt, self.At, self.Wt, self.ones = base.dCt, base.At, base.Wt, base.ones


class _BlockPlan:

    def __init__(self, w, double, tr=None, blk=None, recompute=False):
        k = tr.keep[blk] if tr is not None and tr.keep else None
        s = tr.save if recompute else {}
        replay = recompute and k is not None
        has = lambda name: k is not None and name in k
        pick = lambda name, scratch=None: k[name] if has(name) else s.get(name, scratch)
        d = w.X.shape[-1]
        self.fused_qkv = k is None and not recompute
        self.run_qkv = not (replay and has("qkv"))
        self.run_attn = self.run_out = not replay
        self.run_ff = not (replay and has("hid_pre"))
        self.lean = not double and not self.run_ff
        self.restore = tr.block_in[blk] if recompute and not replay else None
        self.x_in = tr.block_in[blk] if replay else w.X
        self.nrm1, self.nrm2 = s.get("nrm1", w.nrm), s.get("nrm2", w.nrm)
        self.qkv = pick("qkv", w.qkv)
        self.V, self.Qt, self.Kt = s.get("V"), s.get("Qt"), s.get("Kt")
        self.lse = pick("lse", w.lse if recompute else None)
        self.y_attn, self.hid_pre = pick("y_attn"), pick("hid_pre")
        if double:
            self.O, self.ldo = pick("O", w.O), d
            self.y_ff, self.x_mid = pick("y_ff"), pick("x_mid")
        else:
            self.O_keep = pick("O")
            self.O, self.ldo = (self.O_keep, d) if self.lean else (w.cat, 5 * d)


def _train_buffers(cfg, w, device):
    base = w.train
    if base is None or base.B < w.B:
        w.train = None
        del base
        torch.cuda.empty_cache()
        base = _Train(cfg, w, device)
        w.train = base
    return base.view(w.B)


class FluxFunction(torch.autograd.Function):
    @staticmethod
    def forward(ctx, flat_param, model, hidden_states, encoder_hidden_states, timestep, guidance, txt_ids,
                pooled_projections, img_ids):
        cfg = model.cfg
        B, N, _ = hidden_states.shape
        L = encoder_hidden_states.shape[1]
        N_pad = model._pad_kv_rows_train(B, L, N)
        kv_len = None
        if N_pad is not None:
            hidden_states, img_ids = model._padded_inputs(hidden_states, img_ids, N_pad)
            kv_len = L + N
        w = model._workspace(B, L, N if N_pad is None else N_pad, kv_len=kv_len)
        tr = _train_buffers(cfg, w, model.store.device)
        ehs = model._embed(w, hidden_states, encoder_hidden_states)
        keep = {}
        temb, st = model._temb(B, timestep.to(model.store.device), guidance, pooled_projections, keep=keep)
        cos, sin = model._rope(txt_ids, img_ids)
        mods = []
        for blk in range(cfg.num_layers + cfg.num_single_layers):
            tr.block_in[blk].copy_(w.X)
            if blk < cfg.num_layers:
                mods.append(model._double_block(blk, w, st, cos, sin, _BlockPlan(w, True, tr, blk)))
            else:
                mods.append(model._single_block(blk - cfg.num_layers, w, st, cos, sin, _BlockPlan(w, False, tr, blk)))
        tr.x_final.copy_(w.X)
        out, e = model._head(w, st)
        model.last_train_route = "plain" if kv_len is None else "padded_kv"
        model.padded_kv_train_calls += int(kv_len is not None)
        w.train.generation = getattr(w.train, "generation", 0) + 1
        ctx.generation = w.train.generation
        ctx.model, ctx.w, ctx.tr = model, w, tr
        ctx.rows = N
        ctx.saved = dict(ehs=ehs, in16=w.in16.clone(), temb=temb, st=st, keep=keep, cos=cos, sin=sin, mods=mods, e=e)
        return out if kv_len is None else out[:, :N].contiguous()

    @staticmethod
    def backward(ctx, dout):
        if getattr(ctx.w.train, "generation", None) != ctx.generation:
            from ._lib import MgxError
            raise MgxError("FluxTransformer2DModel: the activations of this forward pass were overwritten by a later "
                           "grad-enabled forward of the same model (one pending backward per model; call backward() "
                           "before the next training forward)")
        dout = dout.contiguous().to(BF16)
        if ctx.w.kv_len is not None:
            dout, valid = dout.new_zeros(dout.shape[0], ctx.w.N, dout.shape[2]), dout
            dout[:, :ctx.rows] = valid
        _backward(ctx.model, ctx.w, ctx.tr, ctx.saved, dout)
        return (None,) * 9


def _wgrad(model, tr, A, K, dC: Rows, N, wname, bname, rows=None):
    if model.lora is not None:
        return _lora_wgrad(model, A, K, dC, wname, N if rows else None)
    st = model.store
    g = st.ensure_grad()
    parts = A if isinstance(A, list) else [(A, K, False)]
    M = parts[0][0].M
    Mp = _pad64(M)
    dCt = tr.dCt[:N * Mp].view(N, Mp)
    At = tr.At[:K * Mp].view(K, Mp)
    gb = None
    if bname is not None:
        gb = st.fused(g, bname, N) if rows else st.view(g, bname)
    ops.transpose(dC, N, dCt, Mp, colsum_out=gb, colsum_beta=1.0)
    k0 = 0
    for a_rows, width, gelu in parts:
        ops.transpose(a_rows, width, At[k0:k0 + width], Mp, gelu=gelu)
        k0 += width
    assert k0 == K
    gw = st.fused(g, wname, N) if rows else st.view(g, wname)
    ops.gemm(Rows.of(dCt), At, None, Rows(gw, N, K), K, Mp, EPI_F32_ACC, beta=1.0, ldw=Mp)


def _lora_wgrad(model, X, K, dC: Rows, wname, rows_total):
    lo = model.lora
    members = lo.members(wname, rows_total)
    if not members:
        return
    assert isinstance(X, Rows), "adapter targets take their input as one row-batched matrix"
    g = lo.ensure_grad()
    r, M = lo.rank, dC.M
    dev = lo.device
    T = ops.scratch("lora_T", M * r, BF16, dev)
    dT = ops.scratch("lora_dT", M * r, BF16, dev)
    flat = dC.t.reshape(-1)
    for module, col, n in members:
        A16, Bt16 = lo.view(lo.w16, f"{module}.lora_A"), lo.view(lo.w16, f"{module}.lora_Bt")
        dCm = Rows(flat[col:], M, dC.ld, dC.rpb, dC.bstride)
        ops.lora_proj(X, A16, T, K, r, lo.scale)
        ops.lora_proj(dCm, Bt16, dT, n, r, lo.scale)
        ops.lora_wgrad(T, dCm, lo.view(g, f"{module}.lora_Bt"), n, r, beta=1.0)
        ops.lora_wgrad(dT, X, lo.view(g, f"{module}.lora_A"), K, r, beta=1.0)


def _dgrad(model, tr, dC: Rows, N, K, wname, out: Rows, rows=None, epi=EPI_BIAS, aux=None, ldaux=None, row_lo=0,
           row_hi=None, gate=None):
    st = model.store
    W = st.fused(st.w16, wname, N) if rows else st.view(st.w16, wname)
    Wt = tr.Wt[:K * N].view(K, N)
    ops.transpose(Rows.of(W), K, Wt, N)
    row_hi = K if row_hi is None else row_hi
    ops.gemm(dC, Wt[row_lo:row_hi], None, out, row_hi - row_lo, N, epi, aux=aux, ldaux=ldaux, gate=gate, gate_ld=0)


def _attn_bwd(model, w, Q, K, V, Qt, Kt, O, dO, lse, tr, B, H, S, Sp, ldo, o_bstride, scale):
    if ops.ATTN_FP8_BWD and model.attention_dtype == "fp8":
        ws, amax = w.fp8_bwd_workspace()
        ops.attn_bwd_fp8(Q, K, V, Qt, Kt, O, dO, lse, tr.delta, tr.dOt, tr.dQ, tr.dK, tr.dV, ws, amax, B, H, S, Sp, ldo, o_bstride,
                         scale)
        return
    if w.kv_len is None:
        ops.attn_bwd(Q, K, V, Qt, Kt, O, dO, lse, tr.delta, tr.dOt, tr.dQ, tr.dK, tr.dV, B, H, S, Sp, ldo, o_bstride, scale)
    elif not ops.attn_bwd_kv(Q, K, V, Qt, Kt, O, dO, lse, tr.delta, tr.dOt, tr.dQ, tr.dK, tr.dV, B, H, S, w.kv_len, ldo, o_bstride,
                             scale):
        from ._lib import MgxError
        raise MgxError(f"mgx_attn_bwd_kv refused B {B} H {H} Sa {S} kv_len {w.kv_len} after its path query took it")


def _skinny_bwd(model, tr, dmod, x, wname, bname, N, K, dx_acc):
    st = model.store
    if model.lora is None:
        g = st.ensure_grad()
        ops.skinny_wgrad(dmod, x, st.view(g, wname), st.view(g, bname), N, K)
    if dx_acc is not None:
        ops.skinny_dgrad(dmod, st.view(st.w16, wname), dx_acc, N, K)


def _backward(model, w, tr, sv, dout):
    cfg = model.cfg
    d, H = cfg.dim, cfg.num_attention_heads
    B, L, N, S, Sp = w.B, w.L, w.N, w.S, w.Sp
    M = B * S
    dev = model.store.device
    st_, cos, sin = sv["st"], sv["cos"], sv["sin"]
    scale, q_scale = model.attn_scale(), model.q_scale()
    store = model.store
    if model.lora is None:
        g32 = store.ensure_grad()
        gnorm = lambda name: store.view(g32, name)
    else:
        sink = torch.zeros(cfg.attention_head_dim, dtype=F32, device=dev)
        gnorm = lambda name: sink
    dst = torch.zeros(B, d, dtype=BF16, device=dev)

    def srows(t, which, width):
        return model._stream_rows(t, w, which, width)

    cout = cfg.patch_size * cfg.patch_size * cfg.in_channels
    e = sv["e"]
    nrm = tr.save["nrm1"][:B * N]
    ops.ln_modulate(srows(tr.x_final, "img", d), e[:, d:2 * d], e[:, 0:d], 2 * d, nrm, d)
    dC = Rows.of(dout.view(B * N, cout))
    _wgrad(model, tr, Rows.of(nrm), d, dC, cout, "proj_out.weight", "proj_out.bias")
    dn = tr.dnrm[:B * N]
    _dgrad(model, tr, dC, cout, d, "proj_out.weight", Rows.of(dn))
    tr.dX.zero_()
    de = torch.zeros(B, 2 * d, dtype=BF16, device=dev)
    ops.ln_modulate_bwd(dn, srows(tr.x_final, "img", d), e[:, 0:d], 2 * d, srows(tr.dX, "img", d), False,
                        de[:, d:2 * d], de[:, 0:d], d)
    _skinny_bwd(model, tr, de, st_, "norm_out.linear.weight", "norm_out.linear.bias", 2 * d, d, dst)

    grad_ready = getattr(model, "_grad_ready", None) or (lambda prefix: None)
    grad_ready("tail")
    nblk = cfg.num_layers + cfg.num_single_layers
    for i in reversed(range(cfg.num_single_layers)):
        blk = cfg.num_layers + i
        p = f"single_transformer_blocks.{i}"
        m = sv["mods"][blk]
        pl = _BlockPlan(w, False, tr, blk, recompute=True)
        model._single_block(i, w, st_, cos, sin, pl, mod_in=m)
        dmod = torch.empty(B, 3 * d, dtype=BF16, device=dev)
        x_in = Rows(tr.block_in[blk], M, d, S, S * d)
        dXr = Rows(tr.dX, M, d, S, S * d)
        ops.gate_bwd(dXr, pl.y_attn, m[:, 2 * d:3 * d], 3 * d, tr.dy, dmod[:, 2 * d:3 * d], B, S, d)
        dyr = Rows.of(tr.dy)
        a_op = [(Rows.of(pl.O.view(M, d)), d, False), (Rows.of(pl.hid_pre), 4 * d, True)] if pl.lean else Rows.of(pl.O.view(M, 5 * d))
        _wgrad(model, tr, a_op, 5 * d, dyr, d, f"{p}.proj_out.weight", f"{p}.proj_out.bias")
        dO = tr.dO.view(-1)[:M * pl.ldo].view(B, S, pl.ldo)
        dbig = tr.dbig
        stW = store.view(store.w16, f"{p}.proj_out.weight")
        Wt = tr.Wt[:5 * d * d].view(5 * d, d)
        ops.transpose(Rows.of(stW), 5 * d, Wt, d)
        ops.gemm(dyr, Wt[0:d], None, Rows.of(dO.view(M, pl.ldo)), d, d, EPI_BIAS)
        ops.gemm(dyr, Wt[d:5 * d], None, Rows(dbig[0, 3 * d:], M, 7 * d), 4 * d, d, EPI_DGELU, aux=pl.hid_pre, ldaux=4 * d)
        _attn_bwd(model, w, w.Q, w.K, pl.V, pl.Qt, pl.Kt, pl.O, dO, pl.lse, tr, B, H, S, Sp, pl.ldo, S * pl.ldo, scale)
        ops.qk_norm_rope_bwd(pl.qkv, model.W32(f"{p}.attn.norm_q.weight"), model.W32(f"{p}.attn.norm_k.weight"), cos, sin,
                             tr.dQ, tr.dK, tr.dV, dbig, gnorm(f"{p}.attn.norm_q.weight"),
                             gnorm(f"{p}.attn.norm_k.weight"), B, H, S, Sp, S, 0, ld_dqkv=7 * d, q_scale=q_scale)
        dbr = Rows.of(dbig)
        _wgrad(model, tr, Rows.of(pl.nrm1), d, dbr, 7 * d, f"{p}.attn.to_q.weight", f"{p}.attn.to_q.bias", rows=True)
        _dgrad(model, tr, dbr, 7 * d, d, f"{p}.attn.to_q.weight", Rows.of(tr.dnrm), rows=True)
        ops.ln_modulate_bwd(tr.dnrm, x_in, m[:, d:2 * d], 3 * d, dXr, True, dmod[:, 0:d], dmod[:, d:2 * d], d)
        _skinny_bwd(model, tr, dmod, st_, f"{p}.norm.linear.weight", f"{p}.norm.linear.bias", 3 * d, d, dst)
        grad_ready(p)

    streams, sl = model._streams(w)
    dO3 = tr.dO.view(-1)[:B * S * d].view(B, S, d)
    dh_all = tr.dbig.view(-1)[:M * 4 * d].view(M, 4 * d)
    dqkv_all = tr.dbig.view(-1)[:M * 3 * d].view(M, 3 * d)
    for i in reversed(range(cfg.num_layers)):
        p = f"transformer_blocks.{i}"
        mods = sv["mods"][i]
        pl = _BlockPlan(w, True, tr, i, recompute=True)
        model._double_block(i, w, st_, cos, sin, pl, mods_in=mods)
        dmods = {k: torch.empty(B, 6 * d, dtype=BF16, device=dev) for k in ("img", "txt")}
        for name, norm, qkvn, nq, nk, outn, ffn, rows, s0 in streams:
            m, dm = mods[name], dmods[name]
            ops.gate_bwd(srows(tr.dX, name, d), pl.y_ff[sl[name]], m[:, 5 * d:6 * d], 6 * d, tr.dy[sl[name]],
                         dm[:, 5 * d:6 * d], B, rows, d)
            a_op = Rows.of(w.hid[sl[name]]) if pl.run_ff else [(Rows.of(pl.hid_pre[sl[name]]), 4 * d, True)]
            _wgrad(model, tr, a_op, 4 * d, Rows.of(tr.dy[sl[name]]), d, f"{p}.{ffn}.net.2.weight", f"{p}.{ffn}.net.2.bias")
        for name, norm, qkvn, nq, nk, outn, ffn, rows, s0 in streams:
            _dgrad(model, tr, Rows.of(tr.dy[sl[name]]), d, 4 * d, f"{p}.{ffn}.net.2.weight", Rows.of(dh_all[sl[name]]),
                   epi=EPI_DGELU, aux=pl.hid_pre[sl[name]], ldaux=4 * d)
        for name, norm, qkvn, nq, nk, outn, ffn, rows, s0 in streams:
            _wgrad(model, tr, Rows.of(pl.nrm2[sl[name]]), d, Rows.of(dh_all[sl[name]]), 4 * d, f"{p}.{ffn}.net.0.proj.weight",
                   f"{p}.{ffn}.net.0.proj.bias")
        for name, norm, qkvn, nq, nk, outn, ffn, rows, s0 in streams:
            _dgrad(model, tr, Rows.of(dh_all[sl[name]]), 4 * d, d, f"{p}.{ffn}.net.0.proj.weight", Rows.of(tr.dnrm[sl[name]]))
        for name, norm, qkvn, nq, nk, outn, ffn, rows, s0 in streams:
            m, dm = mods[name], dmods[name]
            dXs = srows(tr.dX, name, d)
            ops.ln_modulate_bwd(tr.dnrm[sl[name]], srows(pl.x_mid, name, d), m[:, 4 * d:5 * d], 6 * d, dXs, True,
                                dm[:, 3 * d:4 * d], dm[:, 4 * d:5 * d], d)
            ops.gate_bwd(dXs, pl.y_attn[sl[name]], m[:, 2 * d:3 * d], 6 * d, tr.dy[sl[name]], dm[:, 2 * d:3 * d], B, rows, d)
            _wgrad(model, tr, srows(pl.O, name, d), d, Rows.of(tr.dy[sl[name]]), d, f"{p}.attn.{outn}.weight",
                   f"{p}.attn.{outn}.bias")
        for name, norm, qkvn, nq, nk, outn, ffn, rows, s0 in streams:
            _dgrad(model, tr, Rows.of(tr.dy[sl[name]]), d, d, f"{p}.attn.{outn}.weight", srows(dO3, name, d))
        _attn_bwd(model, w, w.Q, w.K, pl.V, pl.Qt, pl.Kt, pl.O, dO3, pl.lse, tr, B, H, S, Sp, d, S * d, scale)
        for name, norm, qkvn, nq, nk, outn, ffn, rows, s0 in streams:
            ops.qk_norm_rope_bwd(pl.qkv[sl[name]], model.W32(f"{p}.attn.{nq}.weight"), model.W32(f"{p}.attn.{nk}.weight"), cos,
                                 sin, tr.dQ, tr.dK, tr.dV, dqkv_all[sl[name]], gnorm(f"{p}.attn.{nq}.weight"),
                                 gnorm(f"{p}.attn.{nk}.weight"), B, H, S, Sp, rows, s0, q_scale=q_scale)
            _wgrad(model, tr, Rows.of(pl.nrm1[sl[name]]), d, Rows.of(dqkv_all[sl[name]]), 3 * d, f"{p}.attn.{qkvn[0]}.weight",
                   f"{p}.attn.{qkvn[0]}.bias", rows=True)
        for name, norm, qkvn, nq, nk, outn, ffn, rows, s0 in streams:
            _dgrad(model, tr, Rows.of(dqkv_all[sl[name]]), 3 * d, d, f"{p}.attn.{qkvn[0]}.weight", Rows.of(tr.dnrm[sl[name]]),
                   rows=True)
        for name, norm, qkvn, nq, nk, outn, ffn, rows, s0 in streams:
            m, dm = mods[name], dmods[name]
            ops.ln_modulate_bwd(tr.dnrm[sl[name]], srows(tr.block_in[i], name, d), m[:, d:2 * d], 6 * d, srows(tr.dX, name, d),
                                True, dm[:, 0:d], dm[:, d:2 * d], d)
            _skinny_bwd(model, tr, dm, st_, f"{p}.{norm}.linear.weight", f"{p}.{norm}.linear.bias", 6 * d, d, dst)
        grad_ready(p)

    _wgrad(model, tr, Rows.of(sv["in16"]), cfg.in_channels, srows(tr.dX, "img", d), d, "x_embedder.weight",
           "x_embedder.bias")
    _wgrad(model, tr, Rows.of(sv["ehs"].view(B * L, -1)), cfg.joint_attention_dim, srows(tr.dX, "txt", d), d,
           "context_embedder.weight", "context_embedder.bias")

    dtemb = torch.empty(B, d, dtype=BF16, device=dev)
    ops.ew(sv["temb"], dst, dtemb, 1)
    for name, (x, h1, a1) in sv["keep"].items():
        K = x.shape[1]
        da1 = torch.zeros(B, d, dtype=BF16, device=dev)
        _skinny_bwd(model, tr, dtemb, a1, f"time_text_embed.{name}.linear_2.weight",
                    f"time_text_embed.{name}.linear_2.bias", d, d, da1)
        dh1 = torch.empty(B, d, dtype=BF16, device=dev)
        ops.ew(h1, da1, dh1, 1)
        _skinny_bwd(model, tr, dh1, x, f"time_text_embed.{name}.linear_1.weight",
                    f"time_text_embed.{name}.linear_1.bias", d, K, None)
    if model.lora is not None:
        if model.lora_param.grad is None:
            model.lora_param.grad = model.lora.ensure_grad()
    elif model.flat_param.grad is None:
        model.flat_param.grad = g32
```

### mixgrpo_amd/lora.py

```python
import json
import math
import os
from typing import Dict, List, Tuple

import torch

from . import ops
from .ops import BF16, F32

SUPPORTED_TARGETS = ("to_q", "to_k", "to_v", "add_q_proj", "add_k_proj", "add_v_proj", "to_out.0", "to_add_out",
                     "ff.net.0.proj", "ff_context.net.0.proj", "proj_mlp")
DEFAULT_TARGETS = ("to_q", "to_k", "to_v", "add_q_proj", "add_k_proj", "add_v_proj", "to_out.0", "to_add_out")
WEIGHTS_NAME = "pytorch_lora_weights.safetensors"
CONFIG_NAME = "lora_config.json"
KEY_PREFIX = "transformer."


def parse_target_modules(spec):
    if spec is None or spec == "" or spec == ():
        return DEFAULT_TARGETS
    names = [s.strip() for s in spec.split(",")] if isinstance(spec, str) else list(spec)
    names = [n for n in names if n]
    for n in names:
        if n not in SUPPORTED_TARGETS:
            raise ValueError(f"LoRA target module {n!r} is not supported; choose from {', '.join(SUPPORTED_TARGETS)}")
    if not names:
        return DEFAULT_TARGETS
    return tuple(dict.fromkeys(names))


def resolve_targets(layout, target_modules) -> List[Tuple[str, int, int]]:
    targets = parse_target_modules(target_modules)
    out = []
    for name, shape in layout:
        if not name.endswith(".weight") or len(shape) != 2:
            continue
        module = name[:-len(".weight")]
        if any(module == t or module.endswith("." + t) for t in targets):
            out.append((module, shape[0], shape[1]))
    return out


def check_rank(rank):
    if rank not in ops.LORA_RANKS:
        raise ValueError(f"LoRA rank {rank} is not supported; choose from {ops.LORA_RANKS}")


class LoraStore:

    ALIGN = 64

    def __init__(self, cfg, device, rank, alpha, target_modules=None, layout=None, allocate=True):
        from .flux import param_layout
        check_rank(rank)
        self.cfg = cfg
        self.device = torch.device(device)
        self.rank, self.alpha = int(rank), float(alpha)
        self.scale = self.alpha / self.rank
        self.target_modules = parse_target_modules(target_modules)
        self.layout = param_layout(cfg) if layout is None else layout
        self.targets = resolve_targets(self.layout, self.target_modules)
        if not self.targets:
            raise ValueError(f"LoRA target modules {self.target_modules} select no Linear of this model")
        for module, N, K in self.targets:
            if K % 64 or N % 64:
                raise ValueError(f"LoRA target {module}: [{N}, {K}] is not a multiple of 64 in both dimensions")
        self.index: Dict[str, Tuple[int, Tuple[int, ...]]] = {}
        self.by_module = {m: (N, K) for m, N, K in self.targets}
        off = 0
        for module, N, K in self.targets:
            for key, width in ((f"{module}.lora_A", K), (f"{module}.lora_Bt", N)):
                self.index[key] = (off, (self.rank, width))
                off += (self.rank * width + self.ALIGN - 1) // self.ALIGN * self.ALIGN
        self.numel = off
        self.g32 = None
        self._members = {}
        self._order = [n for n, _ in self.layout]
        self._shape = dict(self.layout)
        if allocate:
            self.w32 = torch.zeros(off, dtype=F32, device=self.device)
            self.w16 = torch.zeros(off, dtype=BF16, device=self.device)

    def view(self, buf, name):
        off, shape = self.index[name]
        return buf[off:off + shape[0] * shape[1]].view(shape)

    def sync_bf16(self):
        self.w16.copy_(self.w32)

    def ensure_grad(self):
        if self.g32 is None:
            self.g32 = torch.zeros(self.numel, dtype=F32, device=self.device)
        return self.g32

    def block_ranges(self):
        cfg = self.cfg
        prefixes = [f"transformer_blocks.{i}" for i in range(cfg.num_layers)] + \
                   [f"single_transformer_blocks.{i}" for i in range(cfg.num_single_layers)]
        out, pos = {"head": (0, 0)}, 0
        keys = list(self.index)
        k = 0
        for p in prefixes:
            lo = pos
            while k < len(keys) and keys[k].startswith(p + "."):
                k += 1
                pos = self.index[keys[k]][0] if k < len(keys) else self.numel
            out[p] = (lo, pos)
        out["tail"] = (self.numel, self.numel)
        return out

    def init_adapters(self, seed=0):
        g = torch.Generator(device=self.device).manual_seed(seed)
        self.w32.zero_()
        for module, N, K in self.targets:
            bound = math.sqrt(6.0 / ((1.0 + 5.0) * K))
            self.view(self.w32, f"{module}.lora_A").uniform_(-bound, bound, generator=g)
        self.sync_bf16()

    def members(self, wname, rows_total=None):
        key = (wname, rows_total)
        hit = self._members.get(key)
        if hit is None:
            hit, i, col = [], self._order.index(wname), 0
            total = self._shape[wname][0] if rows_total is None else rows_total
            while col < total:
                name = self._order[i]
                module = name[:-len(".weight")]
                if module in self.by_module:
                    hit.append((module, col, self._shape[name][0]))
                col += self._shape[name][0]
                i += 1
            assert col == total, (wname, rows_total)
            self._members[key] = hit
        return hit

    def merge(self, store):
        for module, N, K in self.targets:
            ops.lora_merge(store.view(store.w32, f"{module}.weight"), self.view(self.w32, f"{module}.lora_Bt"),
                           self.view(self.w32, f"{module}.lora_A"), store.view(store.w16, f"{module}.weight"), N, K, self.rank,
                           self.scale)

    def unmerge(self, store):
        for module, N, K in self.targets:
            store.view(store.w16, f"{module}.weight").copy_(store.view(store.w32, f"{module}.weight"))

    def key_shapes(self):
        out = {}
        for module, N, K in self.targets:
            out[f"{KEY_PREFIX}{module}.lora_A.weight"] = (self.rank, K)
            out[f"{KEY_PREFIX}{module}.lora_B.weight"] = (N, self.rank)
        return out

    def state_dict(self):
        out = {}
        for module, N, K in self.targets:
            out[f"{KEY_PREFIX}{module}.lora_A.weight"] = self.view(self.w32, f"{module}.lora_A")
            out[f"{KEY_PREFIX}{module}.lora_B.weight"] = self.view(self.w32, f"{module}.lora_Bt").t()
        return out
# ... 44 lines not shown
```

### mixgrpo_amd/ops.py

```python
import os
from dataclasses import dataclass

import torch

from ._lib import check, lib, ptr, stream

EPI_BIAS, EPI_BIAS_GELU, EPI_BIAS_GATE_RES, EPI_F32_ACC, EPI_DGELU = 0, 1, 2, 3, 4
BF16 = torch.bfloat16
F32 = torch.float32


@dataclass
class Rows:
    t: torch.Tensor
    M: int
    ld: int
    rpb: int = 1 << 40
    bstride: int = 0

    @staticmethod
    def of(t):
        cols = t.shape[-1]
        return Rows(t, t.numel() // cols, cols)

# ... 9 lines not shown
def _profiled(launch, args, flops, shape):
    if GEMM_PROFILE is None:
        return launch(*args)
    e0, e1 = torch.cuda.Event(enable_timing=True), torch.cuda.Event(enable_timing=True)
    e0.record()
    took = launch(*args)
    if took is not False:
        e1.record()
        GEMM_PROFILE.append((e0, e1, flops, shape))
    return took


def _try(entry, *args):
    rc = entry(*args)
    if rc == 1:
        return False
    check(rc)
    return True

LINEAR_VT = os.environ.get("MGX_LINEAR_VT", "1") != "0"
LINEAR_QKNORM = os.environ.get("MGX_LINEAR_QKNORM", "1") != "0"
ROPE_PAIR_TABLE = os.environ.get("MGX_ROPE_PAIR_TABLE", "1") != "0"


def linear_t(X, W, bias, Ct, tokens, F, K, ld_ct, tok_rpb, ct_bstride):
    ws = _sk_workspace(X.device) if GEMM_STREAM_K else None
    return _profiled(_try, (lib().mgx_linear_bf16_t, ptr(X), ptr(W), ptr(bias), Ct.data_ptr(), tokens, F, K, K, K, ld_ct, tok_rpb,
                            ct_bstride, None if ws is None else ws.data_ptr(), 0 if ws is None else ws.numel(), stream()),
                     2.0 * tokens * F * K, (F, tokens, K, EPI_BIAS))


def _gemm_launch(A, W, bias, C, N, K, epi, gate, gate_ld, aux, beta, ldw, ldaux):
    ws = _sk_workspace(C.t.device) if GEMM_STREAM_K else None
    check(lib().mgx_gemm_bf16_sk(ptr(A.t), ptr(W), ptr(bias), ptr(C.t), None if gate is None else gate.data_ptr(),
                                 None if aux is None else aux.data_ptr(), (N if ldaux is None else ldaux), A.M, N, K, A.ld,
                                 A.rpb, A.bstride, K if ldw is None else ldw, C.ld, C.rpb, C.bstride, gate_ld, epi, beta,
                                 None if ws is None else ws.data_ptr(), 0 if ws is None else ws.numel(), stream()))




GEMM_STREAM_K = os.environ.get("MGX_GEMM_STREAM_K", "1") != "0"
_sk_ws = {}


def _sk_workspace(device):
    key = (device, torch.cuda.current_stream().cuda_stream)
    w = _sk_ws.get(key)
    if w is None:
        w = torch.empty(lib().mgx_gemm_sk_workspace_elems(), dtype=F32, device=device)
        _sk_ws[key] = w
    return w


_scratch = {}


def scratch(name, numel, dtype, device):
    key = (name, dtype, device)
    t = _scratch.get(key)
    if t is None or t.numel() < numel:
        t = torch.empty(int(numel), dtype=dtype, device=device)
        _scratch[key] = t
    return t[:numel]


def transpose(inp: Rows, N, out, ld_out, colsum_out=None, colsum_beta=1.0, gelu=False):
    if gelu:
        assert colsum_out is None and inp.rpb >= inp.M
        check(lib().mgx_transpose_gelu_bf16(ptr(inp.t), ptr(out), inp.M, N, inp.ld, ld_out, stream()))
        return
    part = None
    if colsum_out is not None:
        part = scratch("colsum_partial", lib().mgx_transpose_partial_elems(inp.M, N), F32, out.device)
    check(lib().mgx_transpose_bf16(ptr(inp.t), ptr(out), ptr(part), ptr(colsum_out), colsum_beta, inp.M, N, inp.ld,
                                   inp.rpb, inp.bstride, ld_out, stream()))


def ln_modulate(x: Rows, shift, scale, mod_ld, y, D, stats=None):
    check(lib().mgx_ln_modulate_fwd(ptr(x.t), x.ld, x.rpb, x.bstride, shift.data_ptr(), scale.data_ptr(), mod_ld, ptr(y),
                                    D, ptr(stats), x.M, D, stream()))


def ln_modulate_bwd(dy, x: Rows, scale, mod_ld, dx: Rows, accumulate, dshift, dscale, D):
    ws = scratch("ln_bwd", lib().mgx_ln_modulate_bwd_workspace(x.M, min(x.rpb, x.M), D), F32, dy.device)
    check(lib().mgx_ln_modulate_bwd(ptr(dy), D, ptr(x.t), x.ld, min(x.rpb, x.M), x.bstride, scale.data_ptr(), mod_ld,
                                    ptr(dx.t), dx.ld, min(dx.rpb, dx.M), dx.bstride, int(accumulate), dshift.data_ptr(),
                                    dscale.data_ptr(), ptr(ws), x.M, D, stream()))


LN2, LOG2E = 0.6931471805599453, 1.4426950408889634
Q_PRESCALE = os.environ.get("MGX_ATTN_Q_PRESCALE", "1") != "0"


def qk_norm_rope(qkv, wq, wk, cos, sin, Q, K, Vt, B, H, S, Sp, rows_per_batch, s0, V=None, Qt=None, Kt=None, q_scale=1.0):
    check(lib().mgx_qk_norm_rope_fwd_qs(ptr(qkv), qkv.shape[-1], ptr(wq), ptr(wk), ptr(cos), ptr(sin), ptr(Q), ptr(K),
                                        ptr(Vt), ptr(V), ptr(Qt), ptr(Kt), B, H, S, Sp, rows_per_batch, s0, float(q_scale),
                                        stream()))


def qk_norm_rope_bwd(qkv, wq, wk, cos, sin, dQ, dK, dV, dqkv, gwq, gwk, B, H, S, Sp, rows_per_batch, s0, ld_dqkv=None,
                     q_scale=1.0):
    ws = scratch("qk_bwd", lib().mgx_qk_norm_rope_bwd_workspace(B, H, rows_per_batch), F32, qkv.device)
    check(lib().mgx_qk_norm_rope_bwd_qs(ptr(qkv), qkv.shape[-1], ptr(wq), ptr(wk), ptr(cos), ptr(sin), ptr(dQ), ptr(dK),
                                        ptr(dV), dqkv.data_ptr(), qkv.shape[-1] if ld_dqkv is None else ld_dqkv, ptr(gwq),
                                        ptr(gwk), ptr(ws), B, H, S, Sp, rows_per_batch, s0, float(q_scale), stream()))


def linear_qk_norm_rope(X, Wqk, bias, wq, wk, cos, sin, Q, K, B, H, S, rows_per_batch, s0, Kdim, q_scale=1.0, pairs=None):
    return _profiled(_try, (lib().mgx_linear_qk_norm_rope, ptr(X), ptr(Wqk), ptr(bias), ptr(wq), ptr(wk), ptr(cos), ptr(sin), ptr(pairs),
                            ptr(Q), ptr(K), B, H, S, rows_per_batch, s0, Kdim, Kdim, Kdim, float(q_scale), stream()),
                     2.0 * B * rows_per_batch * 2 * H * 128 * Kdim, (B * rows_per_batch, 2 * H * 128, Kdim, 5))


def rope_pair_table(cos, sin):
    if not (torch.equal(cos[:, 0::2], cos[:, 1::2]) and torch.equal(sin[:, 0::2], sin[:, 1::2])):
        return None
    return torch.stack([cos[:, 0::2], sin[:, 0::2]], dim=-1).contiguous()


def attn_fwd(Q, K, Vt, O_ptr_tensor, lse, B, H, S, Sp, ldo, o_bstride, scale):
    check(lib().mgx_attn_fwd(ptr(Q), ptr(K), ptr(Vt), O_ptr_tensor.data_ptr(), ptr(lse), B, H, S, Sp, ldo, o_bstride,
                             scale, stream()))


def attn_fwd_log2(Q2, K, Vt, O_ptr_tensor, lse, B, H, S, Sp, ldo, o_bstride):
    check(lib().mgx_attn_fwd_log2(ptr(Q2), ptr(K), ptr(Vt), O_ptr_tensor.data_ptr(), ptr(lse), B, H, S, Sp, ldo, o_bstride,
                                  stream()))


def attn_fwd_path(B, H, S, Sp, ldo, o_bstride):
    r = lib().mgx_attn_fwd_path(B, H, S, Sp, ldo, o_bstride)
    check(min(r, 0))
    return r


ATTN_PAD_KV = os.environ.get("MGX_ATTN_PAD_KV", "0") != "0"


def attn_fwd_log2_kv(Q2, K, Vt, O_ptr_tensor, lse, B, H, Sa, kv_len, ldo, o_bstride):
    return _try(lib().mgx_attn_fwd_log2_kv, ptr(Q2), ptr(K), ptr(Vt), O_ptr_tensor.data_ptr(), ptr(lse), B, H, Sa, kv_len, ldo, o_bstride,
                stream())


def attn_fwd_kv_path(B, H, Sa, kv_len, ldo, o_bstride):
    return lib().mgx_attn_fwd_kv_path(B, H, Sa, kv_len, ldo, o_bstride)


def attn_bwd_path(B, H, S, Sp, ldo, o_bstride):
    r = lib().mgx_attn_bwd_path(B, H, S, Sp, ldo, o_bstride)
    check(min(r, 0))
    return r


def attn_fp8_quantize(Q, K, Vt, Q8, K8, V8t, amax, B, H, S, Sp):
    check(lib().mgx_attn_fp8_quantize(ptr(Q), ptr(K), ptr(Vt), ptr(Q8), ptr(K8), ptr(V8t), ptr(amax), B, H, S, Sp,
                                      stream()))


def attn_fwd_fp8(Q8, K8, V8t, amax, O_ptr_tensor, lse, B, H, S, Sp, ldo, o_bstride, scale):
    check(lib().mgx_attn_fwd_fp8(ptr(Q8), ptr(K8), ptr(V8t), ptr(amax), O_ptr_tensor.data_ptr(), ptr(lse), B, H, S, Sp,
                                 ldo, o_bstride, scale, stream()))


ATTN_FP8_BWD = os.environ.get("MGX_ATTN_FP8_BWD", "0") != "0"


def attn_bwd_fp8_workspace(B, H, S, Sp):
    n = lib().mgx_attn_bwd_fp8_workspace(B, H, S, Sp)
    if n < 0:
        raise ValueError(f"attn_bwd_fp8_workspace: bad sizes B {B} H {H} S {S} Sp {Sp}")
    return n


def attn_bwd_fp8_layout(B, H, S, Sp):
    rb, tb = (B * H * S * 128 + 255) // 256 * 256, B * H * 128 * Sp
    out = {n: (i * rb, (B, H, S, 128)) for i, n in enumerate(("Q8", "K8", "V8", "dO8"))}
    out.update({n: (4 * rb + i * tb, (B, H, 128, Sp)) for i, n in enumerate(("Q8t", "K8t", "dO8t"))})
    return out


def attn_bwd_fp8(Q, K, V, Qt, Kt, O, dO, lse, delta, dOt, dQ, dK, dV, ws, amax, B, H, S, Sp, ldo, o_bstride, scale):
    check(lib().mgx_attn_bwd_fp8(ptr(Q), ptr(K), ptr(V), ptr(Qt), ptr(Kt), O.data_ptr(), dO.data_ptr(), ptr(lse), ptr(delta),
                                 ptr(dOt), ptr(dQ), ptr(dK), ptr(dV), ptr(ws), ptr(amax), B, H, S, Sp, ldo, o_bstride, scale,
                                 ws.numel(), stream()))


def skinny_linear(x, W, bias, out, N, K):
    Bn = x.shape[0]
    for b0 in range(0, Bn, 16):
        nb = min(16, Bn - b0)
        check(lib().mgx_skinny_linear(x[b0:].data_ptr(), x.stride(0), ptr(W), K, ptr(bias), out[b0:].data_ptr(),
                                      out.stride(0), nb, N, K, stream()))


def skinny_wgrad(dout, x, dW, dbias, N, K):
    Bn = x.shape[0]
    for b0 in range(0, Bn, 16):
        nb = min(16, Bn - b0)
        check(lib().mgx_skinny_wgrad(dout[b0:].data_ptr(), dout.stride(0), x[b0:].data_ptr(), x.stride(0), ptr(dW), K,
                                     ptr(dbias), nb, N, K, stream()))


def skinny_dgrad(dout, W, dx, N, K, accumulate=True):
    Bn = dout.shape[0]
    for b0 in range(0, Bn, 8):
        nb = min(8, Bn - b0)
        ws = scratch("skinny_dgrad", lib().mgx_skinny_dgrad_workspace(nb, K), F32, dout.device)
        check(lib().mgx_skinny_dgrad(dout[b0:].data_ptr(), dout.stride(0), ptr(W), K, dx[b0:].data_ptr(), dx.stride(0),
                                     ptr(ws), nb, N, K, 1 if accumulate else 0, stream()))


def ew(a, b, y, op):
    check(lib().mgx_ew_bf16(ptr(a), ptr(b), ptr(y), a.numel(), op, stream()))


def sincos_embed(t, out):
    check(lib().mgx_sincos_embed(ptr(t), ptr(out), t.numel(), stream()))


def cast_bf16(x, y):
    check(lib().mgx_cast_f32_bf16(ptr(x), ptr(y), x.numel(), stream()))


def gelu_rows(x, ldx, y, ldy, M, N):
    check(lib().mgx_gelu_bf16(ptr(x), ldx, ptr(y), ldy, M, N, stream()))


def cast_f32(x, y, scale=1.0):
    check(lib().mgx_cast_bf16_f32(ptr(x), ptr(y), x.numel(), float(scale), stream()))


def gate_bwd(dout: Rows, y, gate, gate_ld, dy, dgate, batches, rows_per_batch, D):
    ws = scratch("gate_bwd", lib().mgx_gate_bwd_workspace(batches, rows_per_batch, D), F32, y.device)
    check(lib().mgx_gate_bwd(ptr(dout.t), dout.ld, dout.bstride, ptr(y), D, gate.data_ptr(), gate_ld, ptr(dy), D,
                             dgate.data_ptr(), ptr(ws), batches, rows_per_batch, D, stream()))


def sqnorm(g, out, beta=0.0):
    ws = scratch("sqnorm", lib().mgx_sqnorm_workspace(), torch.float64, g.device)
    check(lib().mgx_sqnorm_f32(ptr(g), g.numel(), ptr(ws), ptr(out), beta, stream()))


def adamw_step(w, w16, g, m, v, lr, beta1, beta2, eps, wd, step, gnorm_sq, max_norm, grad_scale=1.0):
    check(lib().mgx_adamw_step(ptr(w), ptr(w16), ptr(g), ptr(m), ptr(v), w.numel(), lr, beta1, beta2, eps, wd, step,
                               ptr(gnorm_sq), max_norm, grad_scale, stream()))


def attn_bwd(Q, K, V, Qt, Kt, O, dO, lse, delta, dOt, dQ, dK, dV, B, H, S, Sp, ldo, o_bstride, scale):
    check(lib().mgx_attn_bwd(ptr(Q), ptr(K), ptr(V), ptr(Qt), ptr(Kt), O.data_ptr(), dO.data_ptr(), ptr(lse), ptr(delta),
                             ptr(dOt), ptr(dQ), ptr(dK), ptr(dV), B, H, S, Sp, ldo, o_bstride, scale, stream()))


def attn_bwd_kv(Q, K, V, Qt, Kt, O, dO, lse, delta, dOt, dQ, dK, dV, B, H, Sa, kv_len, ldo, o_bstride, scale):
    return _try(lib().mgx_attn_bwd_kv, ptr(Q), ptr(K), ptr(V), ptr(Qt), ptr(Kt), O.data_ptr(), dO.data_ptr(), ptr(lse), ptr(delta),
                ptr(dOt), ptr(dQ), ptr(dK), ptr(dV), B, H, Sa, kv_len, ldo, o_bstride, scale, stream())


def attn_bwd_kv_path(B, H, Sa, kv_len, ldo, o_bstride):
    return lib().mgx_attn_bwd_kv_path(B, H, Sa, kv_len, ldo, o_bstride)


LORA_RANKS = (16, 32, 64, 128)


def lora_proj(inp: Rows, P, out, Kin, r, scale):
    check(lib().mgx_lora_proj(ptr(inp.t), ptr(P), ptr(out), inp.M, Kin, r, inp.ld, min(inp.rpb, 1 << 40), inp.bstride, float(scale),
                              stream()))


def lora_wgrad_workspace(M, Kin, r):
    n = lib().mgx_lora_wgrad_workspace(M, Kin, r)
    if n < 0:
        raise ValueError(f"lora_wgrad_workspace: unsupported sizes M {M} Kin {Kin} r {r} (r in {LORA_RANKS}, Kin % 64 == 0, M >= 1)")
    return n


def lora_wgrad(small, big: Rows, G, Kin, r, beta=1.0):
    ws = scratch("lora_wgrad", lora_wgrad_workspace(big.M, Kin, r), F32, G.device)
    check(lib().mgx_lora_wgrad(ptr(small), ptr(big.t), ptr(G), ptr(ws), ws.numel(), big.M, Kin, r, big.ld, min(big.rpb, 1 << 40),
                               big.bstride, float(beta), stream()))


def lora_merge(W0, Bt, A, W16, N, K, r, s):
# ... 33 lines not shown
```

### mixgrpo_amd/optim.py

```python
import math

import torch

from . import ops


class FusedAdamW:
    def __init__(self, model, lr=1e-5, betas=(0.9, 0.999), weight_decay=1e-4, eps=1e-8, store=None):
        self.model = model
        self.store = store if store is not None else getattr(model, "trainable_store", model.store)
        self.lr = float(lr)
        self.base_lr = float(lr)
        self.betas = betas
        self.weight_decay = float(weight_decay)
        self.eps = float(eps)
        self.step_count = 0
        dev = self.store.device
        self.m = torch.zeros(self.store.numel, dtype=torch.float32, device=dev)
        self.v = torch.zeros(self.store.numel, dtype=torch.float32, device=dev)
        self.gnorm_sq = torch.zeros(1, dtype=torch.float32, device=dev)
        self.param_groups = [{"lr": self.lr}]

    def zero_grad(self, set_to_none=False):
        g = self.store.g32
        if g is not None:
            g.zero_()

    def grad_sqnorm(self):
        ops.sqnorm(self.store.ensure_grad(), self.gnorm_sq)
        return self.gnorm_sq

    def step(self, max_grad_norm=None, grad_scale=1.0, gnorm_sq=None):
        self.step_count += 1
        lr = self.param_groups[0]["lr"]
        nsq = None
        if max_grad_norm is not None:
            nsq = gnorm_sq if gnorm_sq is not None else self.grad_sqnorm()
        ops.adamw_step(self.store.w32, self.store.w16, self.store.ensure_grad(), self.m, self.v, lr, self.betas[0],
                       self.betas[1], self.eps, self.weight_decay, self.step_count, nsq,
                       0.0 if max_grad_norm is None else float(max_grad_norm), grad_scale)

    def state_dict(self):
        return {"step": self.step_count, "m": self.m, "v": self.v, "lr": self.param_groups[0]["lr"]}

    def load_state_dict(self, sd):
        self.step_count = int(sd["step"])
        self.m.copy_(sd["m"])
        self.v.copy_(sd["v"])
        self.param_groups[0]["lr"] = float(sd["lr"])


SCHEDULER_NAMES = ("linear", "cosine", "cosine_with_restarts", "polynomial", "constant", "constant_with_warmup")


class LambdaSchedule:

    def __init__(self, optimizer, name="constant", num_warmup_steps=0, num_training_steps=1000000, num_cycles=1, power=1.0):
        if name not in SCHEDULER_NAMES:
            raise ValueError(f"lr_scheduler {name!r} is not supported; choose one of {', '.join(SCHEDULER_NAMES)} "
                             "(piecewise_constant needs step_rules, which the reference's get_scheduler call never passes)")
        self.opt = optimizer
        self.name = name
        self.warmup = int(num_warmup_steps) if name != "constant" else 0
        self.total = int(num_training_steps)
        self.num_cycles = num_cycles
        self.power = power
        self.base = [g["lr"] for g in optimizer.param_groups]
        self.n = 0
        self._apply()

    def _factor(self, lr_init=None):
        n, w, T = self.n, self.warmup, self.total
        if self.name == "constant":
            return 1.0
        if n < w:
            return float(n) / float(max(1.0 if self.name == "constant_with_warmup" else 1, w))
        if self.name == "constant_with_warmup":
            return 1.0
        if self.name == "linear":
            return max(0.0, float(T - n) / float(max(1, T - w)))
        progress = float(n - w) / float(max(1, T - w))
        if self.name == "cosine":
            return max(0.0, 0.5 * (1.0 + math.cos(math.pi * 0.5 * 2.0 * progress)))
        if self.name == "cosine_with_restarts":
            if progress >= 1.0:
                return 0.0
            return max(0.0, 0.5 * (1.0 + math.cos(math.pi * ((float(self.num_cycles) * progress) % 1.0))))
        lr_end = 1e-7
        if n > T:
            return lr_end / lr_init
        pct_remaining = 1 - (n - w) / (T - w)
        return ((lr_init - lr_end) * pct_remaining ** self.power + lr_end) / lr_init

    def _apply(self):
        for g, b in zip(self.opt.param_groups, self.base):
            g["lr"] = b * self._factor(b)

    def step(self):
        self.n += 1
        self._apply()

    def get_last_lr(self):
        return [g["lr"] for g in self.opt.param_groups]


def get_scheduler(name, optimizer, num_warmup_steps=0, num_training_steps=1000000, num_cycles=1, power=1.0, last_epoch=-1):
    return LambdaSchedule(optimizer, name, num_warmup_steps, num_training_steps, num_cycles, power)


class ConstantWithWarmup(LambdaSchedule):

    def __init__(self, optimizer, num_warmup_steps=0, last_epoch=-1):
        super().__init__(optimizer, "constant_with_warmup", num_warmup_steps)
```

### mixgrpo_amd/train_grpo_flux.py

```python
import random
from argparse import Namespace

import numpy as np
import torch
import torch.distributed as dist

from . import ops
from . import sampling_utils as SU
from ._lib import check, lib, ptr, stream
from .dist_utils import GradReducer, allreduce_mean_vec_, gather_tensor, is_dist, main_print, rank, world_size
from .latents import pack_latents, prepare_latent_image_ids, unpack_latents

F32, BF16 = torch.float32, torch.bfloat16


def default_args(**kw):
    a = dict(h=1024, w=1024, t=1, sampling_steps=25, shift=3.0, eta=0.7, init_same_noise=True, use_group=True,
             num_generations=8, training_strategy="part", flow_grpo_sampling=True, drop_last_sample=False,
             clip_range=1e-4, adv_clip_max=5.0, kl_coeff=0.0, gradient_accumulation_steps=3, max_grad_norm=1.0,
             multi_reward_mix="advantage_aggr", trimmed_ratio=0.0, advantage_rerange_strategy="null",
             timestep_fraction=0.6, frozen_init_timesteps=-1, dpm_algorithm_type="null", dpm_apply_strategy="post",
             dpm_post_compress_ratio=0.4, dpm_solver_order=2, dpm_solver_type="midpoint",
             sample_strategy="progressive", output_dir="data/outputs", experiment_name="exp", reward_model="synthetic",
             rollout_batch=0, train_microbatch=0, skip_dead_backward=False)
    a.update(kw)
    return Namespace(**a)


def balance_pos_neg(samples, use_random=False):
    if use_random:
        return random.sample(samples, len(samples))
    pos = [s for s in samples if s["advantages"].item() > 0]
    neg = [s for s in samples if s["advantages"].item() < 0]
    pos = random.sample(pos, len(pos))
    neg = random.sample(neg, len(neg))
    small, large = (pos, neg) if len(pos) < len(neg) else (neg, pos)
    out = []
    for a, b in zip(small, large):
        out += [a, b]
    return out + large[len(small):]


def _timestep_tensor(values, device):
    v = np.asarray(values, dtype=np.float32) / np.float32(1000)
    return torch.from_numpy(v).to(device)


def grpo_one_step(args, latents, pre_latents, encoder_hidden_states, pooled_prompt_embeds, text_ids, image_ids,
                  transformer, timesteps, i, sigma_schedule):
    dev = latents.device
    transformer.train()
    ts = timesteps
    if ts.dtype in (torch.long, torch.int32, torch.int64):
        ts = _timestep_tensor(ts.detach().cpu().numpy(), dev)
    with torch.autocast("cuda", torch.bfloat16):
        pred = transformer(hidden_states=latents, encoder_hidden_states=encoder_hidden_states, timestep=ts,
                           guidance=torch.tensor([3.5], device=dev, dtype=BF16),
                           txt_ids=text_ids.repeat(encoder_hidden_states.shape[1], 1),
                           pooled_projections=pooled_prompt_embeds,
                           img_ids=image_ids.squeeze(0) if image_ids.dim() == 3 else image_ids,
                           joint_attention_kwargs=None, return_dict=False)[0]
    if args.dpm_algorithm_type == "null" or ("dpmsolver" in args.dpm_algorithm_type
                                             and args.dpm_apply_strategy == "post"):
        if args.flow_grpo_sampling:
            return SU.flow_grpo_step(pred, latents.to(F32), args.eta, sigma_schedule, i, pre_latents.to(F32),
                                     determistic=False, want_x0=False, want_mean=False)[2]
        return SU.dance_grpo_step(pred, latents.to(F32), args.eta, sigma_schedule, i, pre_latents.to(F32), True, True)[2]
    return SU.dpm_step(args, pred, latents.to(F32), i, sigma_schedule[:-1], sigma_schedule, dpm_state=None,
                       generator=torch.Generator(device=dev), sde_solver=True)[2]


def _as_tensor(x, device):
    if torch.is_tensor(x):
        return x.to(device=device, dtype=F32).reshape(-1)
    return torch.tensor(list(x), device=device, dtype=F32)


def sample_reference_model(args, device, transformer, vae, encoder_hidden_states, pooled_prompt_embeds, text_ids,
                           reward_function, caption, timesteps_train, global_step, reward_weights):
    w, h = args.w, args.h
    T = args.sampling_steps
    sigma_schedule = SU.sd3_time_shift(args.shift, torch.linspace(1, 0, T + 1))
    assert len(sigma_schedule) == T + 1, "sigma_schedule must have length sample_steps + 1"
    B = encoder_hidden_states.shape[0]
    lw, lh = w // 8, h // 8
    inj = getattr(args, "injected_noise", None)
    if args.init_same_noise:
        x_T = inj["x_T"].to(device) if inj else torch.randn((1, 16, lh, lw), device=device, dtype=BF16)
    if args.training_strategy == "part":
        det = [True] * T
        for i in timesteps_train:
            det[i] = False
    elif args.training_strategy == "all":
        det = [False] * T
    else:
        raise ValueError(f"training_strategy {args.training_strategy} is not supported.")
    image_ids = prepare_latent_image_ids(1, lh // 2, lw // 2, device, BF16)
    rb = args.rollout_batch if getattr(args, "rollout_batch", 0) else B
    shared = bool(args.init_same_noise and getattr(args, "use_group", False) and B == args.num_generations
                  and getattr(args, "share_rollout_prefix", True))
    lat_chunks, lp_chunks, final_chunks = [], [], []
    for b0 in range(0, B, rb):
        nb = min(rb, B - b0)
        x0 = x_T.expand(nb, -1, -1, -1).contiguous() if args.init_same_noise else \
            torch.randn((nb, 16, lh, lw), device=device, dtype=BF16)
        z0 = pack_latents(x0, nb, 16, lh, lw)
        with torch.no_grad():
            _, latents, bl, blp = SU.run_sample_step(args, z0, range(T), sigma_schedule, transformer,
                                                     encoder_hidden_states[b0:b0 + nb],
                                                     pooled_prompt_embeds[b0:b0 + nb], text_ids[b0:b0 + 1], image_ids,
                                                     True, det,
                                                     noises=[n[b0:b0 + nb].to(device) for n in inj["steps"]] if inj else None,
                                                     shared_rows=shared)
        lat_chunks.append(bl)
        lp_chunks.append(blp)
        final_chunks.append(latents)
    all_latents = lat_chunks[0] if len(lat_chunks) == 1 else torch.cat(lat_chunks, 0)
    all_log_probs = lp_chunks[0] if len(lp_chunks) == 1 else torch.cat(lp_chunks, 0)
    final = final_chunks[0] if len(final_chunks) == 1 else torch.cat(final_chunks, 0)
    total, heads = reward_function(final, caption)
    if args.multi_reward_mix == "reward_aggr":
        rewards = _as_tensor(total, device)
    elif args.multi_reward_mix == "advantage_aggr":
        rewards = {k: _as_tensor(v, device) for k, v in heads.items()}
    else:
        raise ValueError(f"multi_reward_mix {args.multi_reward_mix} is not supported.")
    all_image_ids = image_ids.unsqueeze(0).expand(B, -1, -1)
    return rewards, all_latents, all_log_probs, sigma_schedule, all_image_ids


def trim_count(G, trimmed_ratio):
    if not trimmed_ratio > 0:
        return -1
    return min(int(G * trimmed_ratio), G - 1)


def compute_advantages(args, rewards, reward_weights, gathered):
    G = args.num_generations
    trim = trim_count(G, args.trimmed_ratio)
    if args.use_group:
        if args.multi_reward_mix == "advantage_aggr":
            first = next(iter(rewards.values()))
            adv = torch.zeros_like(first)
            for k, r in rewards.items():
                check(lib().mgx_group_advantage(ptr(r.contiguous()), ptr(adv), r.numel(), G, trim,
                                                float(reward_weights[k]), 1, stream()))
            return adv
        r = rewards.contiguous()
        adv = torch.zeros_like(r)
        check(lib().mgx_group_advantage(ptr(r), ptr(adv), r.numel(), G, trim, 1.0, 0, stream()))
        return adv
    if args.multi_reward_mix == "advantage_aggr":
        raise ValueError("multi_reward_mix 'advantage_aggr' is not supported when use_group is False.")
    r = rewards.contiguous()
    adv = torch.empty_like(r)
    ga = gathered.contiguous()
    check(lib().mgx_global_advantage(ptr(r), ptr(ga), ptr(adv), r.numel(), ga.numel(), stream()))
    return adv


def _trainable_store(transformer):
    return getattr(transformer, "trainable_store", None) or getattr(transformer, "store", None)


def _grad_reducer(transformer):
    g = _trainable_store(transformer).ensure_grad()
    r = getattr(transformer, "_mgx_grad_reducer", None)
    if r is None or r.flat.data_ptr() != g.data_ptr():
        r = GradReducer(g, mode=getattr(transformer, "dp_grad_dtype", None), overlap=getattr(transformer, "dp_overlap", None))
        transformer._mgx_grad_reducer = r
    return r


def _fused_step(transformer, optimizer, max_grad_norm):
    ws = world_size()
    store = _trainable_store(transformer)
    if store is not None and hasattr(optimizer, "grad_sqnorm"):
        if getattr(optimizer, "store", store) is not store:
            from ._lib import MgxError
            raise MgxError("the optimizer was built over another store than the model trains (build FusedAdamW after "
                           "add_lora / load_lora / unload_lora)")
        _grad_reducer(transformer).finish()
        nsq = optimizer.grad_sqnorm()
        optimizer.step(max_grad_norm=max_grad_norm, grad_scale=1.0 / ws, gnorm_sq=nsq)
        if getattr(transformer, "lora", None) is not None:
            transformer.merge_lora()
        return nsq.sqrt().squeeze(0) / ws
    if ws > 1:
        for prm in transformer.parameters():
            if prm.grad is not None:
                dist.all_reduce(prm.grad, op=dist.ReduceOp.SUM)
                prm.grad.div_(ws)
    gn = transformer.clip_grad_norm_(max_grad_norm)
    optimizer.step()
    return gn


def train_one_step(args, device, transformer, vae, reward_function, optimizer, lr_scheduler, loader, noise_scheduler,
                   max_grad_norm, timesteps_train, global_step, reward_weights, trace=None):
    optimizer.zero_grad()
    steps_done = getattr(transformer, "_mgx_train_steps", 0)
    if steps_done == 1 and hasattr(transformer, "grow_ff_keep"):
        transformer.grow_ff_keep()
    encoder_hidden_states, pooled_prompt_embeds, text_ids, caption = next(loader)
    encoder_hidden_states = encoder_hidden_states.to(device)
    pooled_prompt_embeds = pooled_prompt_embeds.to(device)
    text_ids = text_ids.to(device)
    G = args.num_generations
    if args.use_group:
        encoder_hidden_states = torch.repeat_interleave(encoder_hidden_states, G, dim=0)
        pooled_prompt_embeds = torch.repeat_interleave(pooled_prompt_embeds, G, dim=0)
        text_ids = torch.repeat_interleave(text_ids, G, dim=0)
        if isinstance(caption, str):
            caption = [caption] * G
        elif isinstance(caption, (list, tuple)):
            caption = [c for c in caption for _ in range(G)]
        else:
            raise ValueError(f"Unsupported caption type: {type(caption)}")

    reward, all_latents, all_log_probs, sigma_schedule, all_image_ids = sample_reference_model(
        args, device, transformer, vae, encoder_hidden_states, pooled_prompt_embeds, text_ids, reward_function, caption,
        timesteps_train, global_step, reward_weights)
    B = all_latents.shape[0]
    T = args.sampling_steps
    sig_host = sigma_schedule
    timestep_value = [int(s * 1000) for s in sig_host][:T]

    if args.multi_reward_mix == "advantage_aggr":
        gathered = {k: gather_tensor(v) for k, v in reward.items()}
    else:
        gathered = gather_tensor(reward)
    adv = compute_advantages(args, reward, reward_weights, gathered)
    if trace is not None:
        trace["advantages"] = adv.clone()
        trace["log_probs"] = all_log_probs.clone()

    n_trans = all_log_probs.shape[1] - 1
    order = list(range(B))
    perms = None
    if args.training_strategy == "all":
        perms = torch.stack([torch.randperm(n_trans) for _ in range(B)])
        nt = args.frozen_init_timesteps if args.frozen_init_timesteps > 0 else int(n_trans * args.timestep_fraction)
        if args.frozen_init_timesteps > 0:
            assert args.frozen_init_timesteps <= n_trans
        steps_of = lambda i: [int(perms[i][k]) for k in range(nt)]
    else:
        steps_of = lambda i: list(timesteps_train)
        nt = len(list(timesteps_train))
        if args.advantage_rerange_strategy != "null":
# ... 419 lines not shown
```

Before: 0.4472.

## Fold LN-modulate into wgrad transpose and write grads on first accumulation

Adds a fused transpose+layernorm-modulate kernel so weight-gradient GEMMs can recompute the normalized activations from the block input and saved stats, instead of reading stored normalized tensors. Separately, zero_grad now marks the gradient buffer stale rather than zeroing it, and the wgrad, skinny-wgrad and qk-norm backward kernels take a beta so the first write overwrites instead of accumulating. This removes a full-buffer memset and some activation storage or traffic per step. In exchange it adds bookkeeping: any path that reads gradients must call settled_grad, or it will see stale data.

```diff
diff --git a/include/mixgrpo_hip.h b/include/mixgrpo_hip.h
--- a/include/mixgrpo_hip.h
+++ b/include/mixgrpo_hip.h
@@ -113,6 +113,9 @@
 int mgx_ln_modulate_fwd(const uint16_t* x, long ldx, long x_rpb, long x_bstride, const uint16_t* shift,
                         const uint16_t* scale, long mod_ld, uint16_t* y, long ldy, float* stats, long M, int D,
                         void* stream);
+int mgx_transpose_lnmod_bf16(const uint16_t* x, long ldx, long x_rpb, long x_bstride, const float* stats,
+                             const uint16_t* shift, const uint16_t* scale, long mod_ld, uint16_t* out, long ld_out, long M,
+                             int D, void* stream);
 long mgx_ln_modulate_bwd_workspace(long M, long rpb, int D);
 int mgx_ln_modulate_bwd(const uint16_t* dy, long lddy, const uint16_t* x, long ldx, long x_rpb, long x_bstride,
                         const uint16_t* scale, long mod_ld, uint16_t* dx, long lddx, long dx_rpb, long dx_bstride,
@@ -135,6 +138,10 @@
                             const float* sin, const uint16_t* dQ, const uint16_t* dK, const uint16_t* dV, uint16_t* dqkv,
                             long ld_dqkv, float* gwq, float* gwk, float* ws, int B, int H, int S, int Sp,
                             int rows_per_batch, int s0, float q_scale, void* stream);
+int mgx_qk_norm_rope_bwd_qs_beta(const uint16_t* qkv, long ld, const float* wq, const float* wk, const float* cos,
+                                 const float* sin, const uint16_t* dQ, const uint16_t* dK, const uint16_t* dV, uint16_t* dqkv,
+                                 long ld_dqkv, float* gwq, float* gwk, float* ws, int B, int H, int S, int Sp,
+                                 int rows_per_batch, int s0, float q_scale, float beta, void* stream);
 
 int mgx_attn_fwd(const uint16_t* Q, const uint16_t* K, const uint16_t* Vt, uint16_t* O, float* lse, int B, int H, int S,
                  int Sp, long ldo, long o_bstride, float scale, void* stream);
@@ -177,6 +184,8 @@
                       long ldo, int Bn, int N, int K, void* stream);
 int mgx_skinny_wgrad(const uint16_t* dout, long ldd, const uint16_t* x, long ldx, float* dW, long ldw, float* dbias,
                      int Bn, int N, int K, void* stream);
+int mgx_skinny_wgrad_beta(const uint16_t* dout, long ldd, const uint16_t* x, long ldx, float* dW, long ldw, float* dbias,
+                          int Bn, int N, int K, float beta, void* stream);
 long mgx_skinny_dgrad_workspace(int Bn, int K);
 int mgx_skinny_dgrad(const uint16_t* dout, long ldd, const uint16_t* W, long ldw, uint16_t* dx, long lddx, float* ws,
                      int Bn, int N, int K, int accumulate, void* stream);
diff --git a/mixgrpo_amd/_lib.py b/mixgrpo_amd/_lib.py
--- a/mixgrpo_amd/_lib.py
+++ b/mixgrpo_amd/_lib.py
@@ -59,6 +59,7 @@
     "mgx_transpose_partial_elems": (_L, [_I, _I]),
     "mgx_transpose_bf16": (_I, [_P, _P, _P, _P, _F, _I, _I, _L, _L, _L, _L, _P]),
     "mgx_ln_modulate_fwd": (_I, [_P, _L, _L, _L, _P, _P, _L, _P, _L, _P, _L, _I, _P]),
+    "mgx_transpose_lnmod_bf16": (_I, [_P, _L, _L, _L, _P, _P, _P, _L, _P, _L, _L, _I, _P]),
     "mgx_ln_modulate_bwd_workspace": (_L, [_L, _L, _I]),
     "mgx_ln_modulate_bwd": (_I, [_P, _L, _P, _L, _L, _L, _P, _L, _P, _L, _L, _L, _I, _P, _P, _P, _L, _I, _P]),
     "mgx_qk_norm_rope_fwd": (_I, [_P, _L] + [_P] * 10 + [_I] * 6 + [_P]),
@@ -66,6 +67,7 @@
     "mgx_qk_norm_rope_bwd_workspace": (_L, [_I, _I, _I]),
     "mgx_qk_norm_rope_bwd": (_I, [_P, _L] + [_P] * 8 + [_L] + [_P] * 3 + [_I] * 6 + [_P]),
     "mgx_qk_norm_rope_bwd_qs": (_I, [_P, _L] + [_P] * 8 + [_L] + [_P] * 3 + [_I] * 6 + [_F, _P]),
+    "mgx_qk_norm_rope_bwd_qs_beta": (_I, [_P, _L] + [_P] * 8 + [_L] + [_P] * 3 + [_I] * 6 + [_F, _F, _P]),
     "mgx_attn_fwd": (_I, [_P] * 5 + [_I] * 4 + [_L, _L, _F, _P]),
     "mgx_attn_fwd_log2": (_I, [_P] * 5 + [_I] * 4 + [_L, _L, _P]),
     "mgx_attn_fwd_path": (_I, [_I] * 4 + [_L, _L]),
@@ -82,6 +84,7 @@
     "mgx_attn_kv_operands": (_I, [_I] * 3 + [C.POINTER(_I), _I]),
     "mgx_skinny_linear": (_I, [_P, _L, _P, _L, _P, _P, _L, _I, _I, _I, _P]),
     "mgx_skinny_wgrad": (_I, [_P, _L, _P, _L, _P, _L, _P, _I, _I, _I, _P]),
+    "mgx_skinny_wgrad_beta": (_I, [_P, _L, _P, _L, _P, _L, _P, _I, _I, _I, _F, _P]),
     "mgx_skinny_dgrad_workspace": (_L, [_I, _I]),
     "mgx_conv3x3_nhwc": (_I, [_P, _P, _P, _P, _L, _P, _I, _I, _I, _I, _I, _P]),
     "mgx_group_norm_workspace": (_L, [_L, _I, _I]),
diff --git a/mixgrpo_amd/csrc/gemm.hip b/mixgrpo_amd/csrc/gemm.hip
--- a/mixgrpo_amd/csrc/gemm.hip
+++ b/mixgrpo_amd/csrc/gemm.hip
@@ -348,7 +348,10 @@
     for (int b = ky; b < nblk; b += 4) s += part[(long)b * N + n];
   red[ky][cx] = s;
   __syncthreads();
-  if (ky == 0 && n < N) out[n] = beta * out[n] + ((red[0][cx] + red[1][cx]) + (red[2][cx] + red[3][cx]));
+  if (ky == 0 && n < N) {
+    const float s = (red[0][cx] + red[1][cx]) + (red[2][cx] + red[3][cx]);
+    out[n] = beta != 0.f ? beta * out[n] + s : s;
+  }
 }
 
 __device__ __forceinline__ int wperm(int p) { return (p >> 5) * 32 + ((p & 15) >> 2) * 8 + ((p >> 4) & 1) * 4 + (p & 3); }
diff --git a/mixgrpo_amd/csrc/norm.hip b/mixgrpo_amd/csrc/norm.hip
--- a/mixgrpo_amd/csrc/norm.hip
+++ b/mixgrpo_amd/csrc/norm.hip
@@ -24,6 +24,10 @@
   u.z = (uint32_t)f2bf(f[4]) | ((uint32_t)f2bf(f[5]) << 16);
   u.w = (uint32_t)f2bf(f[6]) | ((uint32_t)f2bf(f[7]) << 16);
   return u;
+}
+
+__device__ __forceinline__ float ln_mod_elem(float v, float mean, float rstd, float scale, float shift) {
+  return (v - mean) * rstd * rbf(1.0f + scale) + shift;
 }
 
 template <int NV>
@@ -69,8 +73,54 @@
     unpack8(*reinterpret_cast<const uint4*>(sh + c), fs);
     unpack8(*reinterpret_cast<const uint4*>(sc + c), fc);
 #pragma unroll
-    for (int j = 0; j < 8; ++j) o[j] = (v[i][j] - mean) * rstd * rbf(1.0f + fc[j]) + fs[j];
+    for (int j = 0; j < 8; ++j) o[j] = ln_mod_elem(v[i][j], mean, rstd, fc[j], fs[j]);
     *reinterpret_cast<uint4*>(y + m * ldy + c) = pack8(o);
+  }
+}
+
+__device__ __forceinline__ uint32_t perm_lo16(uint32_t a, uint32_t b) { return __builtin_amdgcn_perm(b, a, 0x05040100); }
+__device__ __forceinline__ uint32_t perm_hi16(uint32_t a, uint32_t b) { return __builtin_amdgcn_perm(b, a, 0x07060302); }
+__global__ void __launch_bounds__(256) transpose_lnmod_kernel(const bf16_raw* __restrict__ x, RowMap xm,
+                                                              const float* __restrict__ stats,
+                                                              const bf16_raw* __restrict__ shift,
+                                                              const bf16_raw* __restrict__ scale, long mod_ld,
+                                                              bf16_raw* __restrict__ out, long M, int D, long ldo) {
+  const int tx = (threadIdx.x & 7) | (((threadIdx.x >> 6) & 1) << 3), ty = ((threadIdx.x >> 3) & 7) | ((threadIdx.x >> 7) << 3);
+  const int n0 = blockIdx.x * 128 + tx * 8;
+  const long m0 = (long)blockIdx.y * 128 + ty * 8;
+  if (n0 >= D || m0 >= ldo) return;
+  uint32_t r[8][4];
+  long bcur = -1;
+  float fs[8], fc[8];
+#pragma unroll
+  for (int i = 0; i < 8; ++i) {
+    const long m = m0 + i;
+    uint4 v = make_uint4(0, 0, 0, 0);
+    if (m < M) {
+      const long b = m / xm.rpb;
+      if (b != bcur) {
+        unpack8(*reinterpret_cast<const uint4*>(shift + b * mod_ld + n0), fs);
+        unpack8(*reinterpret_cast<const uint4*>(scale + b * mod_ld + n0), fc);
+        bcur = b;
+      }
+      const float mean = stats[2 * m], rstd = stats[2 * m + 1];
+      float f[8], o[8];
+      unpack8(*reinterpret_cast<const uint4*>(x + b * xm.bstride + (m - b * xm.rpb) * xm.ld + n0), f);
+#pragma unroll
+      for (int j = 0; j < 8; ++j) o[j] = ln_mod_elem(f[j], mean, rstd, fc[j], fs[j]);
+      v = pack8(o);
+    }
+    r[i][0] = v.x; r[i][1] = v.y; r[i][2] = v.z; r[i][3] = v.w;
+  }
+#pragma unroll
+  for (int c2 = 0; c2 < 4; ++c2) {
+    uint4 e, o;
+    e.x = perm_lo16(r[0][c2], r[1][c2]); e.y = perm_lo16(r[2][c2], r[3][c2]);
+    e.z = perm_lo16(r[4][c2], r[5][c2]); e.w = perm_lo16(r[6][c2], r[7][c2]);
+    o.x = perm_hi16(r[0][c2], r[1][c2]); o.y = perm_hi16(r[2][c2], r[3][c2]);
+    o.z = perm_hi16(r[4][c2], r[5][c2]); o.w = perm_hi16(r[6][c2], r[7][c2]);
+    *reinterpret_cast<uint4*>(out + (long)(n0 + 2 * c2) * ldo + m0) = e;
+    *reinterpret_cast<uint4*>(out + (long)(n0 + 2 * c2 + 1) * ldo + m0) = o;
   }
 }
 
@@ -413,7 +463,7 @@
 }
 
 __global__ void __launch_bounds__(256) qk_bwd_finish_kernel(const float* __restrict__ part, float* __restrict__ gq,
-                                                            float* __restrict__ gk, long nblocks) {
+                                                            float* __restrict__ gk, long nblocks, float beta) {
   __shared__ float red[16][17];
   const int which = blockIdx.x >> 3, c0 = (blockIdx.x & 7) * 16;
   const int cx = threadIdx.x & 15, ry = threadIdx.x >> 4;
@@ -426,7 +476,7 @@
 #pragma unroll
     for (int i = 0; i < 16; ++i) t += red[i][cx];
     float* dst = which ? gk : gq;
-    dst[c0 + cx] += t;
+    dst[c0 + cx] = (beta != 0.f ? beta * dst[c0 + cx] : 0.f) + t;
   }
 }
 
@@ -446,6 +496,22 @@
     CASE(1) CASE(2) CASE(3) CASE(4) CASE(5) CASE(6) CASE(7) CASE(8)
 #undef CASE
   }
+  MGX_CHECK_LAUNCH();
+  return MGX_OK;
+}
+
+extern "C" int mgx_transpose_lnmod_bf16(const uint16_t* x, long ldx, long x_rpb, long x_bstride, const float* stats,
+                                        const uint16_t* shift, const uint16_t* scale, long mod_ld, uint16_t* out,
+                                        long ld_out, long M, int D, void* stream) {
+  MGX_REQUIRE(x && stats && shift && scale && out && M > 0 && x_rpb > 0, "bad argument");
+  MGX_REQUIRE(D % 512 == 0 && D <= 4096, "feature size must be a multiple of 512 up to 4096");
+  MGX_REQUIRE(ld_out >= M && ld_out % 8 == 0, "output leading dimension must cover M in 16-byte steps");
+  MGX_REQUIRE(ldx % 8 == 0 && mod_ld % 8 == 0 && x_bstride % 8 == 0, "16-byte row alignment");
+  MGX_REQUIRE(((uintptr_t)x % 16 == 0) && ((uintptr_t)out % 16 == 0) && ((uintptr_t)shift % 16 == 0) &&
+              ((uintptr_t)scale % 16 == 0), "operands must be 16-byte aligned");
+  dim3 grid(cdiv(D, 128), (unsigned)cdiv(ld_out, 128));
+  transpose_lnmod_kernel<<<grid, 256, 0, (hipStream_t)stream>>>(x, RowMap{ldx, x_rpb, x_bstride}, stats, shift, scale, mod_ld,
+                                                                out, M, D, ld_out);
   MGX_CHECK_LAUNCH();
   return MGX_OK;
 }
@@ -510,10 +576,11 @@
   return ((long)cdiv(rows_per_batch, 64) * H * B + QK_FIN_G) * 2 * 128;
 }
 
-extern "C" int mgx_qk_norm_rope_bwd_qs(const uint16_t* qkv, long ld, const float* wq, const float* wk, const float* cos,
-                                       const float* sin, const uint16_t* dQ, const uint16_t* dK, const uint16_t* dV,
-                                       uint16_t* dqkv, long ld_dqkv, float* gwq, float* gwk, float* ws, int B, int H, int S,
-                                       int Sp, int rows_per_batch, int s0, float q_scale, void* stream) {
+extern "C" int mgx_qk_norm_rope_bwd_qs_beta(const uint16_t* qkv, long ld, const float* wq, const float* wk, const float* cos,
+                                            const float* sin, const uint16_t* dQ, const uint16_t* dK, const uint16_t* dV,
+                                            uint16_t* dqkv, long ld_dqkv, float* gwq, float* gwk, float* ws, int B, int H,
+                                            int S, int Sp, int rows_per_batch, int s0, float q_scale, float beta,
+                                            void* stream) {
   MGX_REQUIRE(qkv && wq && wk && cos && sin && dQ && dK && dV && dqkv && gwq && gwk && ws, "null argument");
   MGX_REQUIRE(ld == 3L * H * 128, "qkv rows must be [q | k | v] of H*128 each");
   MGX_REQUIRE(ld_dqkv >= ld && ld_dqkv % 2 == 0, "dqkv rows must hold [dq | dk | dv] and keep 4-byte alignment");
@@ -524,9 +591,17 @@
   const long nblocks = (long)grid.x * grid.y * grid.z;
   float* mid = ws + nblocks * 256;
   qk_bwd_partial_kernel<<<QK_FIN_G, 256, 0, st>>>(ws, mid, nblocks);
-  qk_bwd_finish_kernel<<<16, 256, 0, st>>>(mid, gwq, gwk, QK_FIN_G);
+  qk_bwd_finish_kernel<<<16, 256, 0, st>>>(mid, gwq, gwk, QK_FIN_G, beta);
   MGX_CHECK_LAUNCH();
   return MGX_OK;
+}
+
+extern "C" int mgx_qk_norm_rope_bwd_qs(const uint16_t* qkv, long ld, const float* wq, const float* wk, const float* cos,
+                                       const float* sin, const uint16_t* dQ, const uint16_t* dK, const uint16_t* dV,
+                                       uint16_t* dqkv, long ld_dqkv, float* gwq, float* gwk, float* ws, int B, int H, int S,
+                                       int Sp, int rows_per_batch, int s0, float q_scale, void* stream) {
+  return mgx_qk_norm_rope_bwd_qs_beta(qkv, ld, wq, wk, cos, sin, dQ, dK, dV, dqkv, ld_dqkv, gwq, gwk, ws, B, H, S, Sp,
+                                      rows_per_batch, s0, q_scale, 1.0f, stream);
 }
 
 extern "C" int mgx_qk_norm_rope_bwd(const uint16_t* qkv, long ld, const float* wq, const float* wk, const float* cos,
diff --git a/mixgrpo_amd/csrc/small.hip b/mixgrpo_amd/csrc/small.hip
--- a/mixgrpo_amd/csrc/small.hip
+++ b/mixgrpo_amd/csrc/small.hip
@@ -59,7 +59,7 @@
 __global__ void __launch_bounds__(256) skinny_wgrad_kernel(const bf16_raw* __restrict__ dout, long ldd,
                                                            const bf16_raw* __restrict__ x, long ldx,
                                                            float* __restrict__ dW, long ldw, float* __restrict__ dbias,
-                                                           int Bn, int N, int K) {
+                                                           int Bn, int N, int K, float beta) {
   const int n = blockIdx.y;
   float dn[16];
   float sb = 0.f;
@@ -68,9 +68,13 @@
     dn[b] = b < Bn ? bf2f(dout[(long)b * ldd + n]) : 0.f;
     sb += dn[b];
   }
-  if (dbias && blockIdx.x == 0 && threadIdx.x == 0) dbias[n] += sb;
+  if (dbias && blockIdx.x == 0 && threadIdx.x == 0) dbias[n] = (beta != 0.f ? beta * dbias[n] : 0.f) + sb;
   for (int k = (blockIdx.x * 256 + threadIdx.x) * 4; k < K; k += gridDim.x * 256 * 4) {
-    float4 g = *reinterpret_cast<float4*>(dW + (long)n * ldw + k);
+    float4 g = make_float4(0.f, 0.f, 0.f, 0.f);
+    if (beta != 0.f) {
+      g = *reinterpret_cast<float4*>(dW + (long)n * ldw + k);
+      g.x *= beta; g.y *= beta; g.z *= beta; g.w *= beta;
+    }
     for (int b = 0; b < Bn; ++b) {
       const uint2 u = *reinterpret_cast<const uint2*>(x + (long)b * ldx + k);
       g.x += dn[b] * bf2f(u.x & 0xffff); g.y += dn[b] * bf2f(u.x >> 16);
@@ -248,15 +252,20 @@
   return MGX_OK;
 }
 
-extern "C" int mgx_skinny_wgrad(const uint16_t* dout, long ldd, const uint16_t* x, long ldx, float* dW, long ldw,
-                                float* dbias, int Bn, int N, int K, void* stream) {
+extern "C" int mgx_skinny_wgrad_beta(const uint16_t* dout, long ldd, const uint16_t* x, long ldx, float* dW, long ldw,
+                                     float* dbias, int Bn, int N, int K, float beta, void* stream) {
   MGX_REQUIRE(dout && x && dW, "null operand");
   MGX_REQUIRE(Bn >= 1 && Bn <= 16, "skinny wgrad handles 1..16 rows");
   MGX_REQUIRE(K % 4 == 0 && ldx % 4 == 0 && ldw % 4 == 0, "K must be a multiple of 4");
   int gx = cdiv(K, 1024);
-  skinny_wgrad_kernel<<<dim3(gx, N), 256, 0, (hipStream_t)stream>>>(dout, ldd, x, ldx, dW, ldw, dbias, Bn, N, K);
-  MGX_CHECK_LAUNCH();
-  return MGX_OK;
+  skinny_wgrad_kernel<<<dim3(gx, N), 256, 0, (hipStream_t)stream>>>(dout, ldd, x, ldx, dW, ldw, dbias, Bn, N, K, beta);
+  MGX_CHECK_LAUNCH();
+  return MGX_OK;
+}
+
+extern "C" int mgx_skinny_wgrad(const uint16_t* dout, long ldd, const uint16_t* x, long ldx, float* dW, long ldw,
+                                float* dbias, int Bn, int N, int K, void* stream) {
+  return mgx_skinny_wgrad_beta(dout, ldd, x, ldx, dW, ldw, dbias, Bn, N, K, 1.0f, stream);
 }
 
 extern "C" long mgx_skinny_dgrad_workspace(int Bn, int K) { return (long)SD_G * (Bn < 8 ? Bn : 8) * K; }
diff --git a/mixgrpo_amd/flux.py b/mixgrpo_amd/flux.py
--- a/mixgrpo_amd/flux.py
+++ b/mixgrpo_amd/flux.py
@@ -104,6 +104,7 @@
         self.w32 = torch.zeros(off, dtype=F32, device=self.device)
         self.w16 = torch.zeros(off, dtype=BF16, device=self.device)
         self.g32 = None
+        self.grad_stale = False
 
     def view(self, buf, name):
         off, shape = self.index[name]
@@ -360,7 +361,8 @@
         return self.store.view(self.store.w32, name)
 
     def clip_grad_norm_(self, max_norm):
-        g = self.trainable_store.ensure_grad()
+        from .optim import settled_grad
+        g = settled_grad(self.trainable_store)
         nsq = torch.zeros(1, dtype=F32, device=g.device)
         ops.sqnorm(g, nsq)
         total = nsq.sqrt()
@@ -515,6 +517,7 @@
         mods = {}
         streams, sl = self._streams(w)
         W16, fused = self.W, self.store.fused
+        part = lambda t, name: None if t is None else t[sl[name]]
         if pl.restore is not None:
             w.X.copy_(pl.restore)
         for name, norm, qkvn, nq, nk, outn, ffn, rows, s0 in streams:
@@ -524,7 +527,9 @@
                 m = torch.empty(B, 6 * d, dtype=BF16, device=dev)
                 ops.skinny_linear(st, W16(f"{p}.{norm}.linear.weight"), W16(f"{p}.{norm}.linear.bias"), m, 6 * d, d)
             mods[name] = m
-            ops.ln_modulate(self._stream_rows(pl.x_in, w, name, d), m[:, 0:d], m[:, d:2 * d], 6 * d, pl.nrm1[sl[name]], d)
+            if not pl.fold_norm:
+                ops.ln_modulate(self._stream_rows(pl.x_in, w, name, d), m[:, 0:d], m[:, d:2 * d], 6 * d, pl.nrm1[sl[name]], d,
+                                stats=part(pl.stats1, name))
         if pl.fused_qkv:
             for name, _, qkvn, nq, nk, _, _, rows, s0 in streams:
                 self._qkv_nograd(pl.nrm1[sl[name]], f"{p}.attn.{qkvn[0]}", pl.qkv[sl[name]], w, rows, s0,
@@ -538,7 +543,6 @@
                                  w.Q, w.K, w.Vt, B, H, w.S, w.Sp, rows, s0, V=pl.V, Qt=pl.Qt, Kt=pl.Kt, q_scale=self.q_scale())
         if pl.run_attn:
             self._attn(w, pl.O, pl.lse, d, w.S * d)
-        part = lambda t, name: None if t is None else t[sl[name]]
         if pl.run_out:
             for name, _, _, _, _, outn, *_ in streams:
                 ops.gemm(self._stream_rows(pl.O, w, name, d), W16(f"{p}.attn.{outn}.weight"), W16(f"{p}.attn.{outn}.bias"),
@@ -547,9 +551,10 @@
             if pl.x_mid is not None:
                 pl.x_mid.copy_(w.X)
         x_mid = w.X if pl.run_out else pl.x_mid
-        for name in ("txt", "img"):
+        for name in (() if pl.fold_norm else ("txt", "img")):
             m = mods[name]
-            ops.ln_modulate(self._stream_rows(x_mid, w, name, d), m[:, 3 * d:4 * d], m[:, 4 * d:5 * d], 6 * d, pl.nrm2[sl[name]], d)
+            ops.ln_modulate(self._stream_rows(x_mid, w, name, d), m[:, 3 * d:4 * d], m[:, 4 * d:5 * d], 6 * d, pl.nrm2[sl[name]], d,
+                            stats=part(pl.stats2, name))
         for name, _, _, _, _, _, ffn, *_ in (streams if pl.run_ff else ()):
             ops.gemm(Rows.of(pl.nrm2[sl[name]]), W16(f"{p}.{ffn}.net.0.proj.weight"), W16(f"{p}.{ffn}.net.0.proj.bias"),
                      Rows.of(w.hid[sl[name]]), 4 * d, d, EPI_BIAS_GELU, aux=part(pl.hid_pre, name))
@@ -572,7 +577,8 @@
             m = torch.empty(B, 3 * d, dtype=BF16, device=self.store.device)
             ops.skinny_linear(st, self.W(f"{p}.norm.linear.weight"), self.W(f"{p}.norm.linear.bias"), m, 3 * d, d)
         Xa = Rows(pl.x_in, M, d, S, S * d)
-        ops.ln_modulate(Xa, m[:, 0:d], m[:, d:2 * d], 3 * d, pl.nrm1, d)
+        if not pl.fold_norm:
+            ops.ln_modulate(Xa, m[:, 0:d], m[:, d:2 * d], 3 * d, pl.nrm1, d, stats=pl.stats1)
         wq, wk = self.W32(f"{p}.attn.norm_q.weight"), self.W32(f"{p}.attn.norm_k.weight")
         if pl.fused_qkv:
             self._qkv_nograd(pl.nrm1, f"{p}.attn.to_q", pl.qkv, w, S, 0, wq, wk, cos, sin)
diff --git a/mixgrpo_amd/flux_backward.py b/mixgrpo_amd/flux_backward.py
--- a/mixgrpo_amd/flux_backward.py
+++ b/mixgrpo_amd/flux_backward.py
@@ -1,3 +1,4 @@
+import bisect
 import math
 
 import torch
@@ -37,6 +38,10 @@
                 k = dict(O=e(B, S, d), lse=e(B, H, S, dtype=F32), y_attn=e(M, d))
                 if b < cfg.num_layers:
                     k.update(y_ff=e(M, d), x_mid=e(B, S, d))
+                if ops.LNMOD_T:
+                    k.update(stats1=e(M, 2, dtype=F32))
+                    if b < cfg.num_layers:
+                        k.update(stats2=e(M, 2, dtype=F32))
                 self.keep.append(k)
             self._ff_shape, self._ff_device = (M, 4 * d), device
             self._qkv_shape = (M, 3 * d)
@@ -59,6 +64,7 @@
         self.At = e(5 * d * Mp)
         self.Wt = e(7 * d * max(d, 64) + 5 * d * d)
         self.ones = torch.ones(1, 5 * d, dtype=BF16, device=device)
+        self.grad_writes = None
 
     def view(self, B):
         return self if B == self.B else _TrainView(self, B)
@@ -119,17 +125,58 @@
         self.save = {k: (v[:M] if k in rows else v[:B]) for k, v in base.save.items()}
         self.keep = None
         if base.keep is not None:
-            self.keep = [{k: (v[:M] if k in ("y_attn", "y_ff", "hid_pre", "qkv") else v[:B]) for k, v in kb.items()}
+            self.keep = [{k: (v[:M] if k in ("y_attn", "y_ff", "hid_pre", "qkv", "stats1", "stats2") else v[:B]) for k, v in kb.items()}
                          for kb in base.keep]
         self.dX, self.dO, self.dQ, self.dK, self.dV, self.dOt, self.delta = (
             t[:B] for t in (base.dX, base.dO, base.dQ, base.dK, base.dV, base.dOt, base.delta))
         self.dy, self.dbig, self.dnrm = base.dy[:M], base.dbig[:M], base.dnrm[:M]
         self.dCt, self.At, self.Wt, self.ones = base.dCt, base.At, base.Wt, base.ones
+        self.grad_writes = None
+
+
+class _GradWrites:
+
+    def __init__(self, store):
+        self.store = store
+        self.g = store.ensure_grad()
+        self.first = getattr(store, "grad_stale", False)
+        self.lo, self.hi = [], []
+
+    def beta(self, *views):
+        if not self.first:
+            return 1.0
+        betas = {self._beta(v) for v in views if v is not None}
+        assert len(betas) == 1, "one kernel call reaches a written and an unwritten gradient slice"
+        return betas.pop()
+
+    def _beta(self, v):
+        off = v.data_ptr() - self.g.data_ptr()
+        if off < 0 or off >= self.g.numel() * 4:
+            return 1.0
+        assert v.is_contiguous() and v.dtype == F32
+        lo, hi = off // 4, off // 4 + v.numel()
+        i = bisect.bisect_right(self.lo, lo)
+        if i > 0 and hi <= self.hi[i - 1]:
+            return 1.0
+        assert (i == 0 or self.hi[i - 1] <= lo) and (i == len(self.lo) or hi <= self.lo[i]), "gradient slices overlap in part"
+        self.lo.insert(i, lo)
+        self.hi.insert(i, hi)
+        return 0.0
+
+    def finish(self):
+        if not self.first:
+            return
+        pos = 0
+        for lo, hi in zip(self.lo + [self.g.numel()], self.hi + [self.g.numel()]):
+            if lo > pos:
+                self.g[pos:lo].zero_()
+            pos = hi
+        self.store.grad_stale = False
 
 
 class _BlockPlan:
 
-    def __init__(self, w, double, tr=None, blk=None, recompute=False):
+    def __init__(self, w, double, tr=None, blk=None, recompute=False, fold_norm=True):
         k = tr.keep[blk] if tr is not None and tr.keep else None
         s = tr.save if recompute else {}
         replay = recompute and k is not None
@@ -141,6 +188,9 @@
         self.run_attn = self.run_out = not replay
         self.run_ff = not (replay and has("hid_pre"))
         self.lean = not double and not self.run_ff
+        self.fold_norm = fold_norm and replay and has("stats1") and not self.run_qkv and not self.run_ff
+        self.stats1, self.stats2 = (k.get("stats1"), k.get("stats2")) if k is not None and (self.fold_norm or not recompute) \
+            else (None, None)
         self.restore = tr.block_in[blk] if recompute and not replay else None
         self.x_in = tr.block_in[blk] if replay else w.X
         self.nrm1, self.nrm2 = s.get("nrm1", w.nrm), s.get("nrm2", w.nrm)
@@ -220,7 +270,7 @@
 
 def _wgrad(model, tr, A, K, dC: Rows, N, wname, bname, rows=None):
     if model.lora is not None:
-        return _lora_wgrad(model, A, K, dC, wname, N if rows else None)
+        return _lora_wgrad(model, tr, A, K, dC, wname, N if rows else None)
     st = model.store
     g = st.ensure_grad()
     parts = A if isinstance(A, list) else [(A, K, False)]
@@ -231,17 +281,21 @@
     gb = None
     if bname is not None:
         gb = st.fused(g, bname, N) if rows else st.view(g, bname)
-    ops.transpose(dC, N, dCt, Mp, colsum_out=gb, colsum_beta=1.0)
+    fw = tr.grad_writes
+    ops.transpose(dC, N, dCt, Mp, colsum_out=gb, colsum_beta=1.0 if gb is None else fw.beta(gb))
     k0 = 0
     for a_rows, width, gelu in parts:
-        ops.transpose(a_rows, width, At[k0:k0 + width], Mp, gelu=gelu)
+        if isinstance(a_rows, ops.LnMod):
+            ops.transpose_lnmod(a_rows, width, At[k0:k0 + width], Mp)
+        else:
+            ops.transpose(a_rows, width, At[k0:k0 + width], Mp, gelu=gelu)
         k0 += width
     assert k0 == K
     gw = st.fused(g, wname, N) if rows else st.view(g, wname)
-    ops.gemm(Rows.of(dCt), At, None, Rows(gw, N, K), K, Mp, EPI_F32_ACC, beta=1.0, ldw=Mp)
-
-
-def _lora_wgrad(model, X, K, dC: Rows, wname, rows_total):
+    ops.gemm(Rows.of(dCt), At, None, Rows(gw, N, K), K, Mp, EPI_F32_ACC, beta=fw.beta(gw), ldw=Mp)
+
+
+def _lora_wgrad(model, tr, X, K, dC: Rows, wname, rows_total):
     lo = model.lora
     members = lo.members(wname, rows_total)
     if not members:
@@ -258,8 +312,9 @@
         dCm = Rows(flat[col:], M, dC.ld, dC.rpb, dC.bstride)
         ops.lora_proj(X, A16, T, K, r, lo.scale)
         ops.lora_proj(dCm, Bt16, dT, n, r, lo.scale)
-        ops.lora_wgrad(T, dCm, lo.view(g, f"{module}.lora_Bt"), n, r, beta=1.0)
-        ops.lora_wgrad(dT, X, lo.view(g, f"{module}.lora_A"), K, r, beta=1.0)
+        gBt, gA = lo.view(g, f"{module}.lora_Bt"), lo.view(g, f"{module}.lora_A")
+        ops.lora_wgrad(T, dCm, gBt, n, r, beta=tr.grad_writes.beta(gBt))
+        ops.lora_wgrad(dT, X, gA, K, r, beta=tr.grad_writes.beta(gA))
 
 
 def _dgrad(model, tr, dC: Rows, N, K, wname, out: Rows, rows=None, epi=EPI_BIAS, aux=None, ldaux=None, row_lo=0,
@@ -290,7 +345,8 @@
     st = model.store
     if model.lora is None:
         g = st.ensure_grad()
-        ops.skinny_wgrad(dmod, x, st.view(g, wname), st.view(g, bname), N, K)
+        gw, gb = st.view(g, wname), st.view(g, bname)
+        ops.skinny_wgrad(dmod, x, gw, gb, N, K, beta=tr.grad_writes.beta(gw, gb))
     if dx_acc is not None:
         ops.skinny_dgrad(dmod, st.view(st.w16, wname), dx_acc, N, K)
 
@@ -310,6 +366,7 @@
     else:
         sink = torch.zeros(cfg.attention_head_dim, dtype=F32, device=dev)
         gnorm = lambda name: sink
+    fw = tr.grad_writes = _GradWrites(store if model.lora is None else model.lora)
     dst = torch.zeros(B, d, dtype=BF16, device=dev)
 
     def srows(t, which, width):
@@ -332,11 +389,12 @@
     grad_ready = getattr(model, "_grad_ready", None) or (lambda prefix: None)
     grad_ready("tail")
     nblk = cfg.num_layers + cfg.num_single_layers
+    fold_norm = model.lora is None
     for i in reversed(range(cfg.num_single_layers)):
         blk = cfg.num_layers + i
         p = f"single_transformer_blocks.{i}"
         m = sv["mods"][blk]
-        pl = _BlockPlan(w, False, tr, blk, recompute=True)
+        pl = _BlockPlan(w, False, tr, blk, recompute=True, fold_norm=fold_norm)
         model._single_block(i, w, st_, cos, sin, pl, mod_in=m)
         dmod = torch.empty(B, 3 * d, dtype=BF16, device=dev)
         x_in = Rows(tr.block_in[blk], M, d, S, S * d)
@@ -353,11 +411,13 @@
         ops.gemm(dyr, Wt[0:d], None, Rows.of(dO.view(M, pl.ldo)), d, d, EPI_BIAS)
         ops.gemm(dyr, Wt[d:5 * d], None, Rows(dbig[0, 3 * d:], M, 7 * d), 4 * d, d, EPI_DGELU, aux=pl.hid_pre, ldaux=4 * d)
         _attn_bwd(model, w, w.Q, w.K, pl.V, pl.Qt, pl.Kt, pl.O, dO, pl.lse, tr, B, H, S, Sp, pl.ldo, S * pl.ldo, scale)
+        gq, gk = gnorm(f"{p}.attn.norm_q.weight"), gnorm(f"{p}.attn.norm_k.weight")
         ops.qk_norm_rope_bwd(pl.qkv, model.W32(f"{p}.attn.norm_q.weight"), model.W32(f"{p}.attn.norm_k.weight"), cos, sin,
-                             tr.dQ, tr.dK, tr.dV, dbig, gnorm(f"{p}.attn.norm_q.weight"),
-                             gnorm(f"{p}.attn.norm_k.weight"), B, H, S, Sp, S, 0, ld_dqkv=7 * d, q_scale=q_scale)
+                             tr.dQ, tr.dK, tr.dV, dbig, gq, gk, B, H, S, Sp, S, 0, ld_dqkv=7 * d, q_scale=q_scale,
+                             beta=fw.beta(gq, gk))
         dbr = Rows.of(dbig)
-        _wgrad(model, tr, Rows.of(pl.nrm1), d, dbr, 7 * d, f"{p}.attn.to_q.weight", f"{p}.attn.to_q.bias", rows=True)
+        n1 = [(ops.LnMod(x_in, pl.stats1, m[:, 0:d], m[:, d:2 * d], 3 * d), d, False)] if pl.fold_norm else Rows.of(pl.nrm1)
+        _wgrad(model, tr, n1, d, dbr, 7 * d, f"{p}.attn.to_q.weight", f"{p}.attn.to_q.bias", rows=True)
         _dgrad(model, tr, dbr, 7 * d, d, f"{p}.attn.to_q.weight", Rows.of(tr.dnrm), rows=True)
         ops.ln_modulate_bwd(tr.dnrm, x_in, m[:, d:2 * d], 3 * d, dXr, True, dmod[:, 0:d], dmod[:, d:2 * d], d)
         _skinny_bwd(model, tr, dmod, st_, f"{p}.norm.linear.weight", f"{p}.norm.linear.bias", 3 * d, d, dst)
@@ -370,7 +430,7 @@
     for i in reversed(range(cfg.num_layers)):
         p = f"transformer_blocks.{i}"
         mods = sv["mods"][i]
-        pl = _BlockPlan(w, True, tr, i, recompute=True)
+        pl = _BlockPlan(w, True, tr, i, recompute=True, fold_norm=fold_norm)
         model._double_block(i, w, st_, cos, sin, pl, mods_in=mods)
         dmods = {k: torch.empty(B, 6 * d, dtype=BF16, device=dev) for k in ("img", "txt")}
         for name, norm, qkvn, nq, nk, outn, ffn, rows, s0 in streams:
@@ -383,7 +443,11 @@
             _dgrad(model, tr, Rows.of(tr.dy[sl[name]]), d, 4 * d, f"{p}.{ffn}.net.2.weight", Rows.of(dh_all[sl[name]]),
                    epi=EPI_DGELU, aux=pl.hid_pre[sl[name]], ldaux=4 * d)
         for name, norm, qkvn, nq, nk, outn, ffn, rows, s0 in streams:
-            _wgrad(model, tr, Rows.of(pl.nrm2[sl[name]]), d, Rows.of(dh_all[sl[name]]), 4 * d, f"{p}.{ffn}.net.0.proj.weight",
+            m = mods[name]
+            n2 = Rows.of(pl.nrm2[sl[name]])
+            if pl.fold_norm:
+                n2 = [(ops.LnMod(srows(pl.x_mid, name, d), pl.stats2[sl[name]], m[:, 3 * d:4 * d], m[:, 4 * d:5 * d], 6 * d), d, False)]
+            _wgrad(model, tr, n2, d, Rows.of(dh_all[sl[name]]), 4 * d, f"{p}.{ffn}.net.0.proj.weight",
                    f"{p}.{ffn}.net.0.proj.bias")
         for name, norm, qkvn, nq, nk, outn, ffn, rows, s0 in streams:
             _dgrad(model, tr, Rows.of(dh_all[sl[name]]), 4 * d, d, f"{p}.{ffn}.net.0.proj.weight", Rows.of(tr.dnrm[sl[name]]))
@@ -399,10 +463,15 @@
             _dgrad(model, tr, Rows.of(tr.dy[sl[name]]), d, d, f"{p}.attn.{outn}.weight", srows(dO3, name, d))
         _attn_bwd(model, w, w.Q, w.K, pl.V, pl.Qt, pl.Kt, pl.O, dO3, pl.lse, tr, B, H, S, Sp, d, S * d, scale)
         for name, norm, qkvn, nq, nk, outn, ffn, rows, s0 in streams:
+            gq, gk = gnorm(f"{p}.attn.{nq}.weight"), gnorm(f"{p}.attn.{nk}.weight")
             ops.qk_norm_rope_bwd(pl.qkv[sl[name]], model.W32(f"{p}.attn.{nq}.weight"), model.W32(f"{p}.attn.{nk}.weight"), cos,
-                                 sin, tr.dQ, tr.dK, tr.dV, dqkv_all[sl[name]], gnorm(f"{p}.attn.{nq}.weight"),
-                                 gnorm(f"{p}.attn.{nk}.weight"), B, H, S, Sp, rows, s0, q_scale=q_scale)
-            _wgrad(model, tr, Rows.of(pl.nrm1[sl[name]]), d, Rows.of(dqkv_all[sl[name]]), 3 * d, f"{p}.attn.{qkvn[0]}.weight",
+                                 sin, tr.dQ, tr.dK, tr.dV, dqkv_all[sl[name]], gq, gk, B, H, S, Sp, rows, s0, q_scale=q_scale,
+                                 beta=fw.beta(gq, gk))
+            m = mods[name]
+            n1 = Rows.of(pl.nrm1[sl[name]])
+            if pl.fold_norm:
+                n1 = [(ops.LnMod(srows(tr.block_in[i], name, d), pl.stats1[sl[name]], m[:, 0:d], m[:, d:2 * d], 6 * d), d, False)]
+            _wgrad(model, tr, n1, d, Rows.of(dqkv_all[sl[name]]), 3 * d, f"{p}.attn.{qkvn[0]}.weight",
                    f"{p}.attn.{qkvn[0]}.bias", rows=True)
         for name, norm, qkvn, nq, nk, outn, ffn, rows, s0 in streams:
             _dgrad(model, tr, Rows.of(dqkv_all[sl[name]]), 3 * d, d, f"{p}.attn.{qkvn[0]}.weight", Rows.of(tr.dnrm[sl[name]]),
@@ -430,6 +499,7 @@
         ops.ew(h1, da1, dh1, 1)
         _skinny_bwd(model, tr, dh1, x, f"time_text_embed.{name}.linear_1.weight",
                     f"time_text_embed.{name}.linear_1.bias", d, K, None)
+    fw.finish()
     if model.lora is not None:
         if model.lora_param.grad is None:
             model.lora_param.grad = model.lora.ensure_grad()
diff --git a/mixgrpo_amd/lora.py b/mixgrpo_amd/lora.py
--- a/mixgrpo_amd/lora.py
+++ b/mixgrpo_amd/lora.py
@@ -74,6 +74,7 @@
                 off += (self.rank * width + self.ALIGN - 1) // self.ALIGN * self.ALIGN
         self.numel = off
         self.g32 = None
+        self.grad_stale = False
         self._members = {}
         self._order = [n for n, _ in self.layout]
         self._shape = dict(self.layout)
diff --git a/mixgrpo_amd/ops.py b/mixgrpo_amd/ops.py
--- a/mixgrpo_amd/ops.py
+++ b/mixgrpo_amd/ops.py
@@ -115,6 +115,28 @@
                                     D, ptr(stats), x.M, D, stream()))
 
 
+LNMOD_T = os.environ.get("MGX_LNMOD_T", "1") != "0"
+GRAD_FIRST_WRITE = os.environ.get("MGX_GRAD_FIRST_WRITE", "1") != "0"
+
+
+@dataclass
+class LnMod:
+    x: Rows
+    stats: torch.Tensor
+    shift: torch.Tensor
+    scale: torch.Tensor
+    mod_ld: int
+
+    @property
+    def M(self):
+        return self.x.M
+
+
+def transpose_lnmod(a: LnMod, D, out, ld_out):
+    check(lib().mgx_transpose_lnmod_bf16(ptr(a.x.t), a.x.ld, a.x.rpb, a.x.bstride, ptr(a.stats), a.shift.data_ptr(),
+                                         a.scale.data_ptr(), a.mod_ld, ptr(out), ld_out, a.x.M, D, stream()))
+
+
 def ln_modulate_bwd(dy, x: Rows, scale, mod_ld, dx: Rows, accumulate, dshift, dscale, D):
     ws = scratch("ln_bwd", lib().mgx_ln_modulate_bwd_workspace(x.M, min(x.rpb, x.M), D), F32, dy.device)
     check(lib().mgx_ln_modulate_bwd(ptr(dy), D, ptr(x.t), x.ld, min(x.rpb, x.M), x.bstride, scale.data_ptr(), mod_ld,
@@ -133,11 +155,12 @@
 
 
 def qk_norm_rope_bwd(qkv, wq, wk, cos, sin, dQ, dK, dV, dqkv, gwq, gwk, B, H, S, Sp, rows_per_batch, s0, ld_dqkv=None,
-                     q_scale=1.0):
+                     q_scale=1.0, beta=1.0):
     ws = scratch("qk_bwd", lib().mgx_qk_norm_rope_bwd_workspace(B, H, rows_per_batch), F32, qkv.device)
-    check(lib().mgx_qk_norm_rope_bwd_qs(ptr(qkv), qkv.shape[-1], ptr(wq), ptr(wk), ptr(cos), ptr(sin), ptr(dQ), ptr(dK),
-                                        ptr(dV), dqkv.data_ptr(), qkv.shape[-1] if ld_dqkv is None else ld_dqkv, ptr(gwq),
-                                        ptr(gwk), ptr(ws), B, H, S, Sp, rows_per_batch, s0, float(q_scale), stream()))
+    check(lib().mgx_qk_norm_rope_bwd_qs_beta(ptr(qkv), qkv.shape[-1], ptr(wq), ptr(wk), ptr(cos), ptr(sin), ptr(dQ), ptr(dK),
+                                             ptr(dV), dqkv.data_ptr(), qkv.shape[-1] if ld_dqkv is None else ld_dqkv, ptr(gwq),
+                                             ptr(gwk), ptr(ws), B, H, S, Sp, rows_per_batch, s0, float(q_scale), float(beta),
+                                             stream()))
 
 
 def linear_qk_norm_rope(X, Wqk, bias, wq, wk, cos, sin, Q, K, B, H, S, rows_per_batch, s0, Kdim, q_scale=1.0, pairs=None):
@@ -227,12 +250,12 @@
                                       out.stride(0), nb, N, K, stream()))
 
 
-def skinny_wgrad(dout, x, dW, dbias, N, K):
+def skinny_wgrad(dout, x, dW, dbias, N, K, beta=1.0):
     Bn = x.shape[0]
     for b0 in range(0, Bn, 16):
         nb = min(16, Bn - b0)
-        check(lib().mgx_skinny_wgrad(dout[b0:].data_ptr(), dout.stride(0), x[b0:].data_ptr(), x.stride(0), ptr(dW), K,
-                                     ptr(dbias), nb, N, K, stream()))
+        check(lib().mgx_skinny_wgrad_beta(dout[b0:].data_ptr(), dout.stride(0), x[b0:].data_ptr(), x.stride(0), ptr(dW), K,
+                                          ptr(dbias), nb, N, K, float(beta) if b0 == 0 else 1.0, stream()))
 
 
 def skinny_dgrad(dout, W, dx, N, K, accumulate=True):
diff --git a/mixgrpo_amd/optim.py b/mixgrpo_amd/optim.py
--- a/mixgrpo_amd/optim.py
+++ b/mixgrpo_amd/optim.py
@@ -3,6 +3,23 @@
 import torch
 
 from . import ops
+
+
+def discard_grad(store):
+    if store.g32 is None:
+        return
+    if ops.GRAD_FIRST_WRITE:
+        store.grad_stale = True
+    else:
+        store.g32.zero_()
+
+
+def settled_grad(store):
+    g = store.ensure_grad()
+    if getattr(store, "grad_stale", False):
+        g.zero_()
+        store.grad_stale = False
+    return g
 
 
 class FusedAdamW:
@@ -22,12 +39,10 @@
         self.param_groups = [{"lr": self.lr}]
 
     def zero_grad(self, set_to_none=False):
-        g = self.store.g32
-        if g is not None:
-            g.zero_()
+        discard_grad(self.store)
 
     def grad_sqnorm(self):
-        ops.sqnorm(self.store.ensure_grad(), self.gnorm_sq)
+        ops.sqnorm(settled_grad(self.store), self.gnorm_sq)
         return self.gnorm_sq
 
     def step(self, max_grad_norm=None, grad_scale=1.0, gnorm_sq=None):
@@ -36,7 +51,7 @@
         nsq = None
         if max_grad_norm is not None:
             nsq = gnorm_sq if gnorm_sq is not None else self.grad_sqnorm()
-        ops.adamw_step(self.store.w32, self.store.w16, self.store.ensure_grad(), self.m, self.v, lr, self.betas[0],
+        ops.adamw_step(self.store.w32, self.store.w16, settled_grad(self.store), self.m, self.v, lr, self.betas[0],
                        self.betas[1], self.eps, self.weight_decay, self.step_count, nsq,
                        0.0 if max_grad_norm is None else float(max_grad_norm), grad_scale)
 
diff --git a/mixgrpo_amd/train_grpo_flux.py b/mixgrpo_amd/train_grpo_flux.py
--- a/mixgrpo_amd/train_grpo_flux.py
+++ b/mixgrpo_amd/train_grpo_flux.py
@@ -9,6 +9,7 @@
 from . import sampling_utils as SU
 from ._lib import check, lib, ptr, stream
 from .dist_utils import GradReducer, allreduce_mean_vec_, gather_tensor, is_dist, main_print, rank, world_size
+from .optim import settled_grad
 from .latents import pack_latents, prepare_latent_image_ids, unpack_latents
 
 F32, BF16 = torch.float32, torch.bfloat16
@@ -164,7 +165,7 @@
 
 
 def _grad_reducer(transformer):
-    g = _trainable_store(transformer).ensure_grad()
+    g = settled_grad(_trainable_store(transformer))
     r = getattr(transformer, "_mgx_grad_reducer", None)
     if r is None or r.flat.data_ptr() != g.data_ptr():
         r = GradReducer(g, mode=getattr(transformer, "dp_grad_dtype", None), overlap=getattr(transformer, "dp_overlap", None))
```

Result: no change. 0.4492, median of 6 (+0.4%).
